# reedrosenbluth/LASS

Measured on AMD Instinct MI355X. Metric: clips/sec (10s@16kHz), higher is better.
Workload: dtype f32; 1 GPU; ResUNet30 separate() fp32, batch=16/GPU, 10s@16kHz clips, fixed precomputed condition embedding, seeded random-init weights (BASELINE configs[1]); samples_per_clip=160000, parallelism=clip-sharded x1

## Files before the change

### include/lass_hip.h

```cpp
#ifndef LASS_HIP_H
#define LASS_HIP_H

#include <stddef.h>
#include <stdint.h>

#ifdef __cplusplus
extern "C" {
#endif

typedef struct lass_ctx lass_ctx;

#define LASS_OK 0
#define LASS_ERR_ARG (-1)
#define LASS_ERR_HIP (-2)
#define LASS_ERR_STATE (-3)
#define LASS_ERR_WORKSPACE (-4)

#define LASS_F32 0
#define LASS_I64 1

#define LASS_COMPUTE_F32 0
#define LASS_COMPUTE_BF16 1
#define LASS_COMPUTE_BF16X3 2

int lass_version(void);

int lass_create(lass_ctx** out, int device_id);
int lass_create_stft(lass_ctx** out, int device_id, int n_fft, int hop);
int lass_stft_geometry(const lass_ctx* ctx, int* n_fft, int* hop);
int lass_create_multistft(lass_ctx** out, int device_id, int n_fft, int n_windows, const int* win_lengths,
                          int mask_window);
int lass_destroy(lass_ctx* ctx);

const char* lass_last_error(const lass_ctx* ctx);

int lass_set_param(lass_ctx* ctx, const char* name, const void* data, const int64_t* shape, int ndim, int dtype);

int lass_finalize(lass_ctx* ctx, int compute_mode);

int lass_workspace_bytes(const lass_ctx* ctx, int B, int L, size_t* bytes);

int lass_separate(lass_ctx* ctx, const float* mixture, const float* condition, float* out, int B, int L,
                  void* workspace, size_t workspace_bytes, void* stream);


int lass_separate_ragged(lass_ctx* ctx, const float* mixture, const int* lengths, const float* condition, float* out,
                         int B, int L, void* workspace, size_t workspace_bytes, void* stream);
int lass_ragged_bucket(const lass_ctx* ctx, int L, int* lo, int* hi);


int lass_separate_windows(lass_ctx* ctx, const float* recording, int64_t total, const int64_t* starts, const int* keep,
                          const float* condition , float* out , int B, int W,
                          void* workspace, size_t workspace_bytes, void* stream);

int lass_separate_windows_faded(lass_ctx* ctx, const float* recording, int64_t total, const int64_t* starts, const int* keep,
                                const int* fade, const float* ramp, int F, const float* condition ,
                                float* out , int B, int W, void* workspace, size_t workspace_bytes, void* stream);

int lass_graph_stats(const lass_ctx* ctx, long* captures, long* replays);
int lass_set_graph_replay(lass_ctx* ctx, int enabled);
int lass_set_wino4_splits(lass_ctx* ctx, int splits);
int lass_set_wino4_vprep(lass_ctx* ctx, int mode);
int lass_set_head_fold(lass_ctx* ctx, int enabled);
int lass_set_head_sc_fold(lass_ctx* ctx, int enabled);
int lass_set_pw_split(lass_ctx* ctx, int enabled);
int lass_set_wino4_gemm(lass_ctx* ctx, int enabled);
int lass_set_wino4_vprep_buffer(lass_ctx* ctx, float* v, size_t floats);

int lass_separate_components(lass_ctx* ctx, const float* const* mag, const float* cos_mask, const float* sin_mask,
                             const float* condition, float* out, int B, int L, void* workspace, size_t workspace_bytes,
                             void* stream);


int lass_stft_magphase(lass_ctx* ctx, const float* wav, int B, int L, float* mag, float* cos_out, float* sin_out,
                       float* real_out, float* imag_out, void* stream);

int lass_multi_stft(lass_ctx* ctx, const float* wav, int B, int L, int hop, int n_windows, const int* win_lengths,
                    float* const* mag, float* const* cos_out, float* const* sin_out, void* stream);

int lass_stft_components(lass_ctx* ctx, const float* wav, int B, int L, int n_fft, int hop, int n_windows,
                         const int* win_lengths, float* const* mag, float* const* cos_out, float* const* sin_out,
                         void* stream);

int lass_istft(lass_ctx* ctx, const float* real, const float* imag, int B, int T, int L, float* wav,
               float* frames_ws, void* stream);
int lass_istft_nfft(lass_ctx* ctx, const float* real, const float* imag, int B, int T, int L, int n_fft, int win_length,
                    float* wav, void* stream);

int lass_film(lass_ctx* ctx, const float* condition, int B, float* shift, void* stream);
int lass_film_width(const lass_ctx* ctx);
int lass_film_offset(const lass_ctx* ctx, const char* site);
int lass_film_raw(lass_ctx* ctx, const float* condition, int B, float* film, void* stream);

int lass_convblock(lass_ctx* ctx, const char* prefix, const float* x, int B, int H, int W, const float* shift,
                   float* y, float* scratch, void* stream);

int lass_encoder_block(lass_ctx* ctx, const char* name, const float* x, int B, int H, int W, const float* shift, float* y,
                       float* pool, float* scratch, void* stream);

int lass_front_end(lass_ctx* ctx, const float* wav, int B, int L, float* mag, float* cos_out, float* sin_out, float* x0,
                   void* stream);

int lass_front_end_ragged(lass_ctx* ctx, const float* wav, const int* lengths, int B, int L, float* mag, float* cos_out,
                          float* sin_out, float* x0, void* stream);
int lass_istft_ragged(lass_ctx* ctx, const float* real, const float* imag, const int* lengths, int B, int T, int L, int n_fft,
                      int win_length, float* wav, void* stream);

int lass_front_end_windows(lass_ctx* ctx, const float* recording, int64_t total, const int64_t* starts, int B, int W, float* mag,
                           float* cos_out, float* sin_out, float* x0, void* stream);
int lass_istft_windows(lass_ctx* ctx, const float* real, const float* imag, const int64_t* starts, const int* keep, int64_t total,
                       int B, int T, int W, int n_fft, int win_length, float* out, void* stream);
int lass_istft_windows_faded(lass_ctx* ctx, const float* real, const float* imag, const int64_t* starts, const int* keep,
                             const int* fade, const float* ramp, int F, int64_t total, int B, int T, int W, int n_fft,
                             int win_length, float* out, void* stream);

int lass_workspace_tensor(const lass_ctx* ctx, int B, int L, const char* name, size_t* offset, int64_t shape[4],
                          int64_t strides[4]);

int lass_upconv(lass_ctx* ctx, const char* name, const float* x, int B, int h, int w, const float* shift, float* y,
                void* stream);

int lass_mask_apply(lass_ctx* ctx, const float* x12, const float* mag, const float* cos_in, const float* sin_in,
                    int B, int T, int Tpad, float* out_real, float* out_imag, void* stream);

int lass_sdr_stats(lass_ctx* ctx, const float* ref, const float* est, int B, int L, double* stats, void* stream);

int lass_mix_at_snr(lass_ctx* ctx, float* source, const float* noise, const float* snr_db, float* mixture, int B, int L,
                    double* scratch, void* stream);

#define LASS_WAV_PCM16 0
#define LASS_WAV_PCM32 1
#define LASS_WAV_F32 2
#define LASS_RESAMPLE_MAX_TAPS 16383
#define LASS_RESAMPLE_MAX_TABLE 20480
#define LASS_RESAMPLE_MAX_RATIO 65536
int lass_decode_resample(lass_ctx* ctx, const void* raw, int64_t row_stride_bytes, int B, int frames, int channels, int encoding,
                         int up, int down, const float* taps, int n_taps, float* out, int L_out, void* stream);

int lass_decode_resample_planar(lass_ctx* ctx, const void* raw, int64_t row_stride_bytes, int B, int frames, int channels,
                                int encoding, int up, int down, const float* taps, int n_taps, float* out, int L_out, void* stream);

int lass_resample_encode(lass_ctx* ctx, const float* planes, int64_t row_stride, int64_t plane_stride, int B, int channels, int L_in,
                         int up, int down, const float* taps, int n_taps, int encoding, void* out_bytes,
                         int64_t out_row_stride_bytes, int frames_out, unsigned* clipped, void* stream);


#define LASS_LOUDNESS_MAX_HOP 38400
int lass_loudness(lass_ctx* ctx, const float* planes, int64_t row_stride, int64_t plane_stride, int B, int channels, int L,
                  const int* lengths, int hop, const double* coef, const float* weights, double* out, double* blocks, int nb_max,
                  void* scratch, size_t scratch_bytes, void* stream);

int lass_resample_peak(lass_ctx* ctx, const float* planes, int64_t row_stride, int64_t plane_stride, int B, int channels, int L_in,
                       int up, int down, const float* taps, int n_taps, int frames_out, float* peak, void* stream);

int lass_loudness_gain(lass_ctx* ctx, const double* loudness, const float* peak, int B, double target_lufs, float ceiling,
                       float* gain, int* limited, void* stream);

int lass_resample_encode_gain(lass_ctx* ctx, const float* planes, int64_t row_stride, int64_t plane_stride, int B, int channels,
                              int L_in, int up, int down, const float* taps, int n_taps, int encoding, const float* gain,
                              void* out_bytes, int64_t out_row_stride_bytes, int frames_out, unsigned* clipped, void* stream);


int lass_resample_true_peak(lass_ctx* ctx, const float* planes, int64_t row_stride, int64_t plane_stride, int B, int channels,
                            int L_in, int up, int down, const float* taps, int n_taps, int frames_out, int os, const float* os_taps,
                            int n_os_taps, float* peak, void* stream);

int lass_loudness_stats(lass_ctx* ctx, const float* planes, int64_t row_stride, int64_t plane_stride, int B, int channels, int L,
                        const int* lengths, int hop, const double* coef, const float* weights, double* out, double* blocks,
                        int nb_max, double* short_term, int ns_max, void* scratch, size_t scratch_bytes, void* stream);

int lass_segment_mix(lass_ctx* ctx, const float* waveforms, int B, int L, const int* mix_num, const float* comp_db, int max_comp,
                     const float* noise_db, float* mixture, float* segment, double* scratch, void* stream);


typedef struct lass_text_ctx lass_text_ctx;

int lass_text_create(lass_text_ctx** out, int device_id);
int lass_text_destroy(lass_text_ctx* ctx);
const char* lass_text_last_error(const lass_text_ctx* ctx);
int lass_text_set_param(lass_text_ctx* ctx, const char* name, const void* data, const int64_t* shape, int ndim);
int lass_text_finalize(lass_text_ctx* ctx);
int lass_text_layers(const lass_text_ctx* ctx);
int lass_text_workspace_bytes(const lass_text_ctx* ctx, int N, int S, size_t* bytes);
int lass_text_encode(lass_text_ctx* ctx, const int64_t* input_ids, const int64_t* attention_mask, int N, int S,
                     float* out, float* pooler_out, void* workspace, size_t workspace_bytes, void* stream);


typedef struct lass_audioq_ctx lass_audioq_ctx;

typedef struct lass_audioq_taps {
    float* wave48k;
    float* logmel;
    float* tokens;
    float* stage[4];
    float* embedding;
} lass_audioq_taps;

int lass_audioq_create(lass_audioq_ctx** out, int device_id);
int lass_audioq_destroy(lass_audioq_ctx* ctx);
const char* lass_audioq_last_error(const lass_audioq_ctx* ctx);
int lass_audioq_set_param(lass_audioq_ctx* ctx, const char* name, const void* data, const int64_t* shape, int ndim);
int lass_audioq_finalize(lass_audioq_ctx* ctx);
int lass_audioq_stages(const lass_audioq_ctx* ctx);
int lass_audioq_workspace_bytes(const lass_audioq_ctx* ctx, int B, size_t* bytes);
int lass_audioq_encode_wave48k(lass_audioq_ctx* ctx, const float* wave, const int* lengths, int B, int L, float* out,
                               const lass_audioq_taps* taps, void* workspace, size_t workspace_bytes, void* stream);
int lass_audioq_encode_wave32k(lass_audioq_ctx* ctx, const float* wave, const int* lengths, int B, int L, float* out,
                               const lass_audioq_taps* taps, void* workspace, size_t workspace_bytes, void* stream);


int lass_set_profiling(lass_ctx* ctx, int enabled);
int lass_profile_count(const lass_ctx* ctx);
int lass_profile_get(lass_ctx* ctx, int i, const char** name, double* ms, int* launches);
int lass_profile_reset(lass_ctx* ctx);

#ifdef __cplusplus
}
#endif
#endif
```

### lass_amd/_lib.py

```python
from __future__ import annotations

import ctypes
import os
from ctypes import POINTER, c_char_p, c_double, c_float, c_int, c_int64, c_long, c_size_t, c_void_p

_HERE = os.path.dirname(os.path.abspath(__file__))
LIB_PATH = os.environ.get("LASS_HIP_LIB") or os.path.join(_HERE, "csrc", "liblass_hip.so")

_lib = None

SYMBOLS = [
    ("lass_version", c_int, []),
    ("lass_create", c_int, [POINTER(c_void_p), c_int]),
    ("lass_create_stft", c_int, [POINTER(c_void_p), c_int, c_int, c_int]),
    ("lass_stft_geometry", c_int, [c_void_p, POINTER(c_int), POINTER(c_int)]),
    ("lass_create_multistft", c_int, [POINTER(c_void_p), c_int, c_int, c_int, POINTER(c_int), c_int]),
    ("lass_destroy", c_int, [c_void_p]),
    ("lass_last_error", c_char_p, [c_void_p]),
    ("lass_set_param", c_int, [c_void_p, c_char_p, c_void_p, POINTER(c_int64), c_int, c_int]),
    ("lass_finalize", c_int, [c_void_p, c_int]),
    ("lass_workspace_bytes", c_int, [c_void_p, c_int, c_int, POINTER(c_size_t)]),
    ("lass_separate", c_int, [c_void_p, c_void_p, c_void_p, c_void_p, c_int, c_int, c_void_p, c_size_t, c_void_p]),
    ("lass_separate_ragged", c_int, [c_void_p, c_void_p, c_void_p, c_void_p, c_void_p, c_int, c_int, c_void_p, c_size_t,
                                     c_void_p]),
    ("lass_ragged_bucket", c_int, [c_void_p, c_int, POINTER(c_int), POINTER(c_int)]),
    ("lass_front_end_ragged", c_int, [c_void_p, c_void_p, c_void_p, c_int, c_int, c_void_p, c_void_p, c_void_p, c_void_p,
                                      c_void_p]),
    ("lass_istft_ragged", c_int, [c_void_p, c_void_p, c_void_p, c_void_p, c_int, c_int, c_int, c_int, c_int, c_void_p,
                                  c_void_p]),
    ("lass_separate_windows", c_int, [c_void_p, c_void_p, c_int64, c_void_p, c_void_p, c_void_p, c_void_p, c_int, c_int, c_void_p,
                                      c_size_t, c_void_p]),
    ("lass_front_end_windows", c_int, [c_void_p, c_void_p, c_int64, c_void_p, c_int, c_int, c_void_p, c_void_p, c_void_p,
                                       c_void_p, c_void_p]),
    ("lass_istft_windows", c_int, [c_void_p, c_void_p, c_void_p, c_void_p, c_void_p, c_int64, c_int, c_int, c_int, c_int, c_int,
                                   c_void_p, c_void_p]),
    ("lass_separate_windows_faded", c_int, [c_void_p, c_void_p, c_int64, c_void_p, c_void_p, c_void_p, c_void_p, c_int, c_void_p,
                                            c_void_p, c_int, c_int, c_void_p, c_size_t, c_void_p]),
    ("lass_istft_windows_faded", c_int, [c_void_p, c_void_p, c_void_p, c_void_p, c_void_p, c_void_p, c_void_p, c_int, c_int64,
                                         c_int, c_int, c_int, c_int, c_int, c_void_p, c_void_p]),
    ("lass_stft_magphase", c_int, [c_void_p, c_void_p, c_int, c_int, c_void_p, c_void_p, c_void_p, c_void_p,
                                   c_void_p, c_void_p]),
    ("lass_mix_at_snr", c_int, [c_void_p, c_void_p, c_void_p, c_void_p, c_void_p, c_int, c_int, c_void_p, c_void_p]),
    ("lass_decode_resample", c_int, [c_void_p, c_void_p, c_int64, c_int, c_int, c_int, c_int, c_int, c_int, c_void_p, c_int,
                                     c_void_p, c_int, c_void_p]),
    ("lass_decode_resample_planar", c_int, [c_void_p, c_void_p, c_int64, c_int, c_int, c_int, c_int, c_int, c_int, c_void_p, c_int,
                                            c_void_p, c_int, c_void_p]),
    ("lass_resample_encode", c_int, [c_void_p, c_void_p, c_int64, c_int64, c_int, c_int, c_int, c_int, c_int, c_void_p, c_int, c_int,
                                     c_void_p, c_int64, c_int, c_void_p, c_void_p]),
    ("lass_loudness", c_int, [c_void_p, c_void_p, c_int64, c_int64, c_int, c_int, c_int, c_void_p, c_int, POINTER(c_double), c_void_p,
                              c_void_p, c_void_p, c_int, c_void_p, c_size_t, c_void_p]),
    ("lass_resample_peak", c_int, [c_void_p, c_void_p, c_int64, c_int64, c_int, c_int, c_int, c_int, c_int, c_void_p, c_int, c_int,
                                   c_void_p, c_void_p]),
    ("lass_loudness_gain", c_int, [c_void_p, c_void_p, c_void_p, c_int, c_double, c_float, c_void_p, c_void_p, c_void_p]),
    ("lass_resample_encode_gain", c_int, [c_void_p, c_void_p, c_int64, c_int64, c_int, c_int, c_int, c_int, c_int, c_void_p, c_int,
                                          c_int, c_void_p, c_void_p, c_int64, c_int, c_void_p, c_void_p]),
    ("lass_resample_true_peak", c_int, [c_void_p, c_void_p, c_int64, c_int64, c_int, c_int, c_int, c_int, c_int, c_void_p, c_int, c_int,
                                        c_int, c_void_p, c_int, c_void_p, c_void_p]),
    ("lass_loudness_stats", c_int, [c_void_p, c_void_p, c_int64, c_int64, c_int, c_int, c_int, c_void_p, c_int, POINTER(c_double),
                                    c_void_p, c_void_p, c_void_p, c_int, c_void_p, c_int, c_void_p, c_size_t, c_void_p]),
    ("lass_segment_mix", c_int, [c_void_p, c_void_p, c_int, c_int, c_void_p, c_void_p, c_int, c_void_p, c_void_p, c_void_p,
                                 c_void_p, c_void_p]),
    ("lass_multi_stft", c_int, [c_void_p, c_void_p, c_int, c_int, c_int, c_int, POINTER(c_int), POINTER(c_void_p),
                                POINTER(c_void_p), POINTER(c_void_p), c_void_p]),
    ("lass_graph_stats", c_int, [c_void_p, POINTER(c_long), POINTER(c_long)]),
    ("lass_set_graph_replay", c_int, [c_void_p, c_int]),
    ("lass_set_wino4_splits", c_int, [c_void_p, c_int]),
    ("lass_set_wino4_vprep", c_int, [c_void_p, c_int]),
    ("lass_set_wino4_vprep_buffer", c_int, [c_void_p, c_void_p, c_size_t]),
    ("lass_set_head_fold", c_int, [c_void_p, c_int]),
    ("lass_set_head_sc_fold", c_int, [c_void_p, c_int]),
    ("lass_set_pw_split", c_int, [c_void_p, c_int]),
    ("lass_set_wino4_gemm", c_int, [c_void_p, c_int]),
    ("lass_separate_components", c_int, [c_void_p, POINTER(c_void_p), c_void_p, c_void_p, c_void_p, c_void_p, c_int,
                                         c_int, c_void_p, c_size_t, c_void_p]),
    ("lass_stft_components", c_int, [c_void_p, c_void_p, c_int, c_int, c_int, c_int, c_int, POINTER(c_int),
                                     POINTER(c_void_p), POINTER(c_void_p), POINTER(c_void_p), c_void_p]),
    ("lass_istft_nfft", c_int, [c_void_p, c_void_p, c_void_p, c_int, c_int, c_int, c_int, c_int, c_void_p, c_void_p]),
    ("lass_istft", c_int, [c_void_p, c_void_p, c_void_p, c_int, c_int, c_int, c_void_p, c_void_p, c_void_p]),
    ("lass_film", c_int, [c_void_p, c_void_p, c_int, c_void_p, c_void_p]),
    ("lass_film_width", c_int, [c_void_p]),
    ("lass_film_offset", c_int, [c_void_p, c_char_p]),
    ("lass_film_raw", c_int, [c_void_p, c_void_p, c_int, c_void_p, c_void_p]),
    ("lass_convblock", c_int, [c_void_p, c_char_p, c_void_p, c_int, c_int, c_int, c_void_p, c_void_p, c_void_p,
                               c_void_p]),
    ("lass_encoder_block", c_int, [c_void_p, c_char_p, c_void_p, c_int, c_int, c_int, c_void_p, c_void_p, c_void_p,
                                   c_void_p, c_void_p]),
    ("lass_front_end", c_int, [c_void_p, c_void_p, c_int, c_int, c_void_p, c_void_p, c_void_p, c_void_p, c_void_p]),
    ("lass_workspace_tensor", c_int, [c_void_p, c_int, c_int, c_char_p, POINTER(c_size_t), POINTER(c_int64),
                                      POINTER(c_int64)]),
    ("lass_upconv", c_int, [c_void_p, c_char_p, c_void_p, c_int, c_int, c_int, c_void_p, c_void_p, c_void_p]),
    ("lass_mask_apply", c_int, [c_void_p, c_void_p, c_void_p, c_void_p, c_void_p, c_int, c_int, c_int, c_void_p,
                                c_void_p, c_void_p]),
    ("lass_sdr_stats", c_int, [c_void_p, c_void_p, c_void_p, c_int, c_int, c_void_p, c_void_p]),
    ("lass_text_create", c_int, [POINTER(c_void_p), c_int]),
    ("lass_text_destroy", c_int, [c_void_p]),
    ("lass_text_last_error", c_char_p, [c_void_p]),
    ("lass_text_set_param", c_int, [c_void_p, c_char_p, c_void_p, POINTER(c_int64), c_int]),
    ("lass_text_finalize", c_int, [c_void_p]),
    ("lass_text_layers", c_int, [c_void_p]),
    ("lass_text_workspace_bytes", c_int, [c_void_p, c_int, c_int, POINTER(c_size_t)]),
    ("lass_text_encode", c_int, [c_void_p, c_void_p, c_void_p, c_int, c_int, c_void_p, c_void_p, c_void_p, c_size_t,
                                 c_void_p]),
    ("lass_audioq_create", c_int, [POINTER(c_void_p), c_int]),
    ("lass_audioq_destroy", c_int, [c_void_p]),
    ("lass_audioq_last_error", c_char_p, [c_void_p]),
    ("lass_audioq_set_param", c_int, [c_void_p, c_char_p, c_void_p, POINTER(c_int64), c_int]),
    ("lass_audioq_finalize", c_int, [c_void_p]),
    ("lass_audioq_stages", c_int, [c_void_p]),
    ("lass_audioq_workspace_bytes", c_int, [c_void_p, c_int, POINTER(c_size_t)]),
    ("lass_audioq_encode_wave48k", c_int, [c_void_p, c_void_p, POINTER(c_int), c_int, c_int, c_void_p, c_void_p, c_void_p,
                                           c_size_t, c_void_p]),
    ("lass_audioq_encode_wave32k", c_int, [c_void_p, c_void_p, POINTER(c_int), c_int, c_int, c_void_p, c_void_p, c_void_p,
                                           c_size_t, c_void_p]),
    ("lass_set_profiling", c_int, [c_void_p, c_int]),
    ("lass_profile_count", c_int, [c_void_p]),
    ("lass_profile_get", c_int, [c_void_p, c_int, POINTER(c_char_p), POINTER(c_double), POINTER(c_int)]),
    ("lass_profile_reset", c_int, [c_void_p]),
]


class LassError(RuntimeError):
    pass


def load():
    global _lib
    if _lib is not None:
        return _lib
    import torch

    if not os.path.exists(LIB_PATH):
        raise LassError(
            f"{LIB_PATH} is missing - build it with `python -c 'import __graft_entry__ as g; g.build()'` "
            "(hipcc --offload-arch=gfx950).  lass_amd has no CPU fallback.")
    lib = ctypes.CDLL(LIB_PATH, mode=ctypes.RTLD_GLOBAL)
    for name, res, args in SYMBOLS:
        fn = getattr(lib, name)
        fn.restype = res
        fn.argtypes = args
    _lib = lib
    return lib


def check(ctx, rc: int, what: str):
    if rc < 0:
        msg = load().lass_last_error(ctx)
        raise LassError(f"{what} failed ({rc}): {msg.decode() if msg else '?'}")
    return rc


class TowerContext:

    def __init__(self, family: str, dev, tensors):
        import torch

        self.lib, self.family = load(), family
        h = c_void_p()
        rc = self.fn("create")(ctypes.byref(h), dev.index if dev.index is not None else torch.cuda.current_device())
        if rc < 0:
            raise LassError(f"{family}_create failed ({rc}): {self.fn('last_error')(None).decode()}")
        self.ctx = h
        self.key = self.key_of(dev, tensors)
        torch.cuda.current_stream(dev).synchronize()
        for name, p in tensors:
            t = p.detach().to(torch.float32).contiguous()
            shape = (c_int64 * t.dim())(*t.shape)
            self.check(self.fn("set_param")(self.ctx, name.encode(), c_void_p(t.data_ptr()), shape, t.dim()),
                       f"{family}_set_param({name})")
        self.check(self.fn("finalize")(self.ctx), f"{family}_finalize")

    @staticmethod
    def key_of(dev, tensors):
        return (dev, tuple((p.data_ptr(), p._version) for _, p in tensors))

    def fn(self, name: str):
        return getattr(self.lib, f"{self.family}_{name}")

    def check(self, rc: int, what: str) -> int:
        if rc < 0:
            raise LassError(f"{what} failed ({rc}): {self.fn('last_error')(self.ctx).decode()}")
        return rc

    def __del__(self):
        try:
            if getattr(self, "ctx", None):
                self.fn("destroy")(self.ctx)
                self.ctx = None
        except Exception:
            pass


def grow_workspace(owner, nbytes: int, dev):
    import torch

    if owner._ws is None or owner._ws.device != dev or owner._ws.numel() < nbytes:
        owner._ws = None
        owner._ws = torch.empty(nbytes, dtype=torch.uint8, device=dev)
    return owner._ws
```

### lass_amd/csrc/api.hip

```cpp
#include <hip/hip_runtime.h>

#include <algorithm>
#include <cmath>
#include <cstdio>
#include <cstdlib>
#include <cstring>
#include <map>
#include <string>
#include <vector>

#include "../../include/lass_hip.h"
#include "ctx_parts.h"
#include "graph_cache.h"
#include "head_fold.h"
#include "kernels.h"
#include "weight_plan.h"
#include "workspace_plan.h"

namespace {

constexpr float kBnEps = 1e-5f;
constexpr int kMaxBranches = LASS_MAX_STFT_WINDOWS;

struct Site {
    std::string film;
    std::string bn;
    int C = 0;
    int off = 0;
};

struct ResBlock {
    std::string prefix;
    int cin = 0, cout = 0;
    int width = 0;
    int s1 = -1, s2 = -1;
    WeightImages img;
};

struct ProfEntry {
    const char* name;
    double ms = 0;
    int launches = 0;
};

thread_local std::string g_create_err;

}

struct lass_ctx {
    int device = 0;
    std::string err;
    Geometry g;
    ModelTable m;
    std::string pre_name[kMaxBranches];
    ParamStore raw;
    bool finalized = false;
    float2* tw2k = nullptr;
    std::vector<Site> sites;
    std::map<std::string, int> site_idx;
    int n_shift = 0;
    float *film_W = nullptr, *film_b = nullptr, *bn_scale = nullptr, *bn_base = nullptr;
    float *bn0_s = nullptr, *bn0_h = nullptr;
    std::vector<ResBlock> enc, dec;
    int dec_site[6] = {0};
    WeightImages up_img[6], img;
    int head_rows = 0;
    std::vector<void*> owned;
    RouteCfg cfg;
    float* stage_v = nullptr;
    size_t stage_v_floats = 0;
    float* stage_m = nullptr;
    size_t stage_m_floats = 0;
    float* stage_v_user = nullptr;
    size_t stage_v_user_floats = 0;
    float* stage_part = nullptr;
    size_t stage_part_floats = 0;
    bool use_graph = true;
    GraphCache<hipGraphExec_t> graphs;
    std::map<std::pair<int, int>, bool> last_split;
    hipStream_t g_stream = nullptr;
    int split_batch = 1;
    hipStream_t s2 = nullptr;
    hipEvent_t ev_fork = nullptr, ev_join = nullptr;
    unsigned long gen = 0;
    long g_replays = 0, g_captures = 0;
    bool profiling = false;
    std::vector<ProfEntry> prof;
    std::vector<hipEvent_t> ev_pool;
    struct Pending { int cls; hipEvent_t a, b; };
    std::vector<Pending> pending;
    size_t ev_used = 0;
};

namespace {

bool starts_with(const std::string& s, const char* p) { return s.rfind(p, 0) == 0; }
bool ends_with(const std::string& s, const char* p) {
    const size_t n = strlen(p);
    return s.size() >= n && s.compare(s.size() - n, n, p) == 0;
}

std::string film_to_bn(const std::string& film) {
    std::string s = "base.";
    for (size_t i = 0; i < film.size(); ++i) {
        if (film[i] == '-' && i + 1 < film.size() && film[i + 1] == '>') {
            s += '.';
            ++i;
        } else {
            s += film[i];
        }
    }
    const size_t p = s.rfind("beta");
    s.replace(p, 4, "bn");
    return s;
}

int add_site(lass_ctx* c, const std::string& film, int C) {
    Site s;
    s.film = film;
    s.bn = film_to_bn(film);
    s.C = C;
    s.off = c->n_shift;
    c->n_shift += C;
    c->site_idx[film] = (int)c->sites.size();
    c->sites.push_back(s);
    return (int)c->sites.size() - 1;
}

void build_arch(lass_ctx* c) {
    const Geometry& g = c->g;
    c->sites.clear();
    c->site_idx.clear();
    c->n_shift = 0;
    c->enc.clear();
    c->dec.clear();
    c->m = model_table(g.variant == 0 ? 0 : g.nbr, g.fcrop);
    for (int k = 0; k < g.nbr; ++k) {
        ResBlock rb;
        std::string film;
        if (g.variant == 0) {
            rb.prefix = "base.encoder_block1.conv_block1";
            film = "encoder_block1->conv_block1";
            c->pre_name[k] = "base.pre_conv";
        } else {
            const std::string w = std::to_string(g.wins[k]);
            rb.prefix = "base.encoder_block1s." + w + ".conv_block1";
            film = "encoder_block1s->" + w + "->conv_block1";
            c->pre_name[k] = "base.pre_convs." + w;
        }
        rb.cin = rb.cout = kPreCh;
        rb.width = g.fcrop;
        rb.s1 = add_site(c, film + "->beta1", kPreCh);
        rb.s2 = add_site(c, film + "->beta2", kPreCh);
        c->enc.push_back(rb);
    }
    for (int i = 1; i < 7; ++i) {
        const EncSpec& e = c->m.E[i];
        ResBlock rb;
        rb.prefix = std::string("base.") + e.name + ".conv_block1";
        rb.cin = e.cin;
        rb.cout = e.cout;
        rb.width = g.fcrop >> i;
        rb.s1 = add_site(c, std::string(e.name) + "->conv_block1->beta1", e.cin);
        rb.s2 = add_site(c, std::string(e.name) + "->conv_block1->beta2", e.cout);
        c->enc.push_back(rb);
    }
    for (int i = 0; i < 6; ++i) {
        const auto& d = c->m.D[i];
        const int e = 5 - i;
        c->dec_site[i] = add_site(c, std::string(d.name) + "->beta1", d.cin);
        ResBlock rb;
        rb.prefix = std::string("base.") + d.name + ".conv_block2";
        rb.cin = c->m.dec_cat[i];
        rb.cout = d.cout;
        rb.width = g.fcrop >> e;
        rb.s1 = add_site(c, std::string(d.name) + "->conv_block2->beta1", rb.cin);
        rb.s2 = add_site(c, std::string(d.name) + "->conv_block2->beta2", d.cout);
        c->dec.push_back(rb);
    }
}

std::vector<int64_t> expected_shape(const lass_ctx* c, const std::string& name) {
    auto bn_field = [](const std::string& n) {
        return ends_with(n, ".weight") || ends_with(n, ".bias") || ends_with(n, ".running_mean") ||
               ends_with(n, ".running_var");
    };
    if (starts_with(name, "base.bn0.") && bn_field(name)) return {c->g.nbins};
    for (int k = 0; k < c->g.nbr; ++k) {
        if (name == c->pre_name[k] + ".weight") return {kPreCh, 1, 1, 1};
        if (name == c->pre_name[k] + ".bias") return {kPreCh};
    }
    if (name == "base.after_conv.weight") return {3, kPreCh, 1, 1};
    if (name == "base.after_conv.bias") return {3};
    auto res_block = [&](const ResBlock& rb) -> std::vector<int64_t> {
        const std::string& p = rb.prefix;
        if (!starts_with(name, (p + ".").c_str())) return {};
        const std::string f = name.substr(p.size() + 1);
        if (starts_with(f, "bn1.") && bn_field(f)) return {rb.cin};
        if (starts_with(f, "bn2.") && bn_field(f)) return {rb.cout};
        if (f == "conv1.weight") return {rb.cout, rb.cin, 3, 3};
        if (f == "conv2.weight") return {rb.cout, rb.cout, 3, 3};
        if (rb.cin != rb.cout && f == "shortcut.weight") return {rb.cout, rb.cin, 1, 1};
        if (rb.cin != rb.cout && f == "shortcut.bias") return {rb.cout};
        return {};
    };
    for (const auto& rb : c->enc) {
        auto s = res_block(rb);
        if (!s.empty()) return s;
    }
    for (int i = 0; i < 6; ++i) {
        auto s = res_block(c->dec[i]);
        if (!s.empty()) return s;
        const DecSpec& d = c->m.D[i];
        const std::string p = std::string("base.") + d.name;
        if (name == p + ".conv1.weight") return {d.cin, d.cout, d.uh, d.uw};
        if (starts_with(name, (p + ".bn1.").c_str()) && bn_field(name)) return {d.cin};
    }
    if (starts_with(name, "film.")) {
        for (const auto& s : c->sites) {
            if (name == "film." + s.film + ".weight") return {s.C, LASS_COND};
            if (name == "film." + s.film + ".bias") return {s.C};
        }
    }
    return {};
}

bool ignorable(const std::string& name) {
    if (starts_with(name, "base.stft.") || starts_with(name, "base.istft.")) return true;
    if (ends_with(name, "num_batches_tracked")) return true;
    for (const auto& d : kDec) {
        if (starts_with(name, (std::string("base.") + d.name + ".bn2.").c_str())) return true;
        if (starts_with(name, (std::string("film.") + d.name + "->beta2.").c_str())) return true;
    }
    return false;
}

const float* rawp(const lass_ctx* c, const std::string& name) { return c->raw.get(name); }

template <typename T>
int dev_alloc(lass_ctx* c, T** p, size_t count) {
    void* v = nullptr;
    HIP_TRY(c, hipMalloc(&v, count * sizeof(T)));
    c->owned.push_back(v);
    *p = (T*)v;
    return 0;
}

void free_owned(lass_ctx* c) {
    for (void* p : c->owned) (void)hipFree(p);
    c->owned.clear();
}

SlotSet missing_images(const lass_ctx* c, const WeightImages* blk, const WeightImages* up, SlotSet want) {
    SlotSet miss = 0;
    for (int s = 0; s < kWeightSlots; ++s) {
        const WeightImages* im = s < kBlockSlots ? blk : s < kDecoderSlotsEnd ? up : &c->img;
        if ((want >> s & 1) && !(im && im->p[s])) miss |= SlotSet(1) << s;
    }
    return miss;
}

enum ProfClass { P_STFT = 0, P_FILM, P_PRECONV, P_CONV3X3, P_TCONV, P_POOL, P_MASK, P_ISTFT, P_COUNT };
const char* kProfNames[P_COUNT] = {"stft_magphase", "film", "pre_conv", "conv3x3_mfma", "tconv_mfma",
                                   "avg_pool",      "mask_apply", "istft"};

constexpr size_t kProfPairs = 512;

struct ProfScope {
    lass_ctx* c;
    hipStream_t s;
    int cls;
    hipEvent_t b = nullptr;
    bool on = false;
    ProfScope(lass_ctx* ctx, hipStream_t st, int k) : c(ctx), s(st), cls(k) {
        if (!c->profiling || c->ev_used + 2 > c->ev_pool.size()) return;
        hipEvent_t a = c->ev_pool[c->ev_used++];
        b = c->ev_pool[c->ev_used++];
        (void)hipEventRecord(a, s);
        c->pending.push_back({cls, a, b});
        on = true;
    }
    ~ProfScope() {
        if (on) (void)hipEventRecord(b, s);
    }
};

void prof_collect(lass_ctx* c) {
    for (auto& p : c->pending) {
        float ms = 0;
        if (hipEventElapsedTime(&ms, p.a, p.b) == hipSuccess) {
            c->prof[p.cls].ms += ms;
            c->prof[p.cls].launches += 1;
        }
    }
    c->pending.clear();
    c->ev_used = 0;
}

struct CatCopies {
    void* act;
    void* raw;
    int noct;
    const float* scale;
    const float* shift;
};

struct MaskHead {
    const float* mag;
    const float* cosv;
    const float* sinv;
    float* oreal;
    float* oimag;
    int T;
    int nbins;
};

struct PreConv {
    const float* x0;
    const float* w;
    const float* b;
};

struct UpFuse {
    const void* xin;
    int cin, h, w;
    const void* w16;
    const void* wsc16;
};

struct BlockFusions {
    float* pool_out = nullptr;
    int pool_h = 2;
    long pool_bs = 0;
    int cofs = 0;
    const PreConv* pre = nullptr;
    const MaskHead* head = nullptr;
    const CatCopies* skip_out = nullptr;
    const CatCopies* cat_in = nullptr;
    const Site* act_out = nullptr;
    const CatCopies* pool_copies = nullptr;
    const UpFuse* up = nullptr;
    float* kpart = nullptr;
    float* vws = nullptr;
    size_t vws_floats = 0;
    float* mws = nullptr;
    size_t mws_floats = 0;
    const HeadScPlanes* planes = nullptr;
};

BlockIO block_io(const float* x, long x_bs, const BlockFusions& f) {
    BlockIO io;
    io.x0 = f.pre && f.pre->x0;
    io.head = f.head != nullptr;
    io.pool = f.pool_out != nullptr; io.pool_h = f.pool_h;
    io.x_aligned = x && ((uintptr_t)x & 15u) == 0 && x_bs % 4 == 0;
    io.sc_planes = f.planes != nullptr;
    io.cat_in = f.cat_in != nullptr; io.skip_out = f.skip_out != nullptr; io.pool_copies = f.pool_copies != nullptr;
    io.act_out = f.act_out != nullptr; io.up_cin = f.up ? f.up->cin : 0;
    return io;
}

bool overlaps(int B, const float* a, long a_bs, size_t a_n, const float* b, long b_bs, size_t b_n) {
    return a && b && a_n && b_n && a < b + (size_t)(B - 1) * b_bs + b_n && b < a + (size_t)(B - 1) * a_bs + a_n;
}

int run_resblock_bf16(lass_ctx* c, const ResBlock& rb, Bf16Form form, const ConvArgs& p, const ConvArgs& q, int B, hipStream_t st,
                      const BlockFusions& f) {
    if (form == BF16_TWO) {
        const bool x0 = f.pre && f.pre->x0;
        {
            ProfScope ps(c, st, P_CONV3X3);
            HIP_TRY(c, lass_launch_conv_bf16(x0 ? CONV1_ACT_PRE : CONV1_ACT, p, st));
        }
        ProfScope ps(c, st, P_CONV3X3);
        HIP_TRY(c, lass_launch_conv_bf16(rb.cin != rb.cout ? CONV2_SHORTCUT : x0 ? CONV2_IDENT_PRE : CONV2_IDENT, q, st));
        return 0;
    }
    ConvArgs uq;
    if (const UpFuse* up = f.up) {
        uq.in_bf16 = up->xin; uq.Cin = up->cin; uq.H = up->h; uq.W = up->w; uq.B = B;
        uq.w_bf16 = up->w16; uq.w2_bf16 = up->wsc16;
    }
    if (!(form == BF16_ENC1 ? lass_enc1_fused_bf16_supported(p, q) : form == BF16_DEC6 ? lass_dec6_fused_bf16_supported(p, q)
                            : form == BF16_DEC6U && f.up && lass_dec6u_fused_bf16_supported(p, q, uq)))
        return fail(c, LASS_ERR_STATE, rb.prefix + ": the launch arguments contradict the planned route");
    ProfScope ps(c, st, P_CONV3X3);
    HIP_TRY(c, form == BF16_ENC1 ? lass_launch_enc1_fused_bf16(p, q, st) : form == BF16_DEC6 ? lass_launch_dec6_fused_bf16(p, q, st)
                                 : lass_launch_dec6u_fused_bf16(p, q, uq, st));
    return 0;
}

int launch_routed(lass_ctx* c, const ResBlock& rb, const char* what, const ConvRoute& rt, const ConvArgs& a, const Wino4Split& sk,
                  float* vws, const Wino4Gemm& wg, hipStream_t st, const HeadScPlanes* planes = nullptr) {
    ProfScope ps(c, st, P_CONV3X3);
    bool ok = true;
    switch (rt.family) {
        case CONV_F4X4: {
            const Wino4Split s = rt.splits > 1 ? sk : Wino4Split();
            Wino4VPre vp;
            if (rt.v_from_memory) vp.v = vws;
            if (rt.head_sc_fold) {
                ok = planes && (rt.head_fold ? lass_wino4_headfold_planes_supported(a, *planes) : lass_wino4_sclogit_supported(a, *planes));
                if (ok) HIP_TRY(c, rt.head_fold ? lass_launch_wino4_headfold_planes(a, *planes, st) : lass_launch_wino4_sclogit(a, *planes, st));
                break;
            }
            if (rt.head_fold) {
                ok = lass_wino4_headfold_supported(a);
                if (ok) HIP_TRY(c, lass_launch_wino4_headfold(a, st));
                break;
            }
            if (rt.gemm) {
                ok = lass_wino4_gemm_supported(rt.kind, a, vp, wg);
                if (ok) HIP_TRY(c, lass_launch_wino4_gemm(rt.kind, a, vp, wg, st));
                break;
            }
            ok = rt.v_from_memory ? lass_wino4_vpre_supported(rt.kind, a, s) : lass_wino4_supported(rt.kind, a, s);
            if (ok) HIP_TRY(c, lass_launch_wino4(rt.kind, a, st, s, vp));
            break;
        }
        case CONV_F2X2:
            ok = lass_wino_supported(a);
            if (ok) HIP_TRY(c, lass_launch_wino(rt.kind, a, st));
            break;
        case CONV_DIRECT:
            HIP_TRY(c, lass_launch_conv(rt.kind, a, st));
            break;
        case CONV_NONE:
            ok = false;
            break;
    }
    return ok ? 0 : fail(c, LASS_ERR_STATE, rb.prefix + " " + what + ": the launch arguments contradict the planned route");
}

int run_resblock(lass_ctx* c, const ResBlock& rb, const float* x, long x_bs, int B, int H, int W, const float* shift,
                 float* a2, float* out, long out_bs, hipStream_t st, const BlockFusions& f = BlockFusions()) {
    const PreConv* pre = f.pre;
    const WeightImages& im = rb.img;
    const CatCopies *skip_out = f.skip_out, *cat_in = f.cat_in, *pool_copies = f.pool_copies;
    const float* x0 = pre ? pre->x0 : nullptr;
    const Site& s1 = c->sites[rb.s1];
    const Site& s2 = c->sites[rb.s2];
    const long HW = (long)H * W;
    ConvArgs p;
    p.in = x; p.in_bs = x_bs; p.Cin = rb.cin; p.w = im.f32(W1); p.Nw = rb.cout; p.N = rb.cout;
    p.pro_scale = c->bn_scale + s1.off; p.pro_shift = shift + s1.off; p.pro_shift_bs = c->n_shift;
    p.epi_scale = c->bn_scale + s2.off; p.epi_shift = shift + s2.off; p.epi_shift_bs = c->n_shift;
    p.out = a2; p.out_bs = rb.cout * HW; p.B = B; p.H = H; p.W = W;
    if (x0) {
        p.in = x0; p.in_bs = HW;
        p.pre_w = pre->w; p.pre_b = pre->b;
    }
    p.w_wino = im.f32(U1); p.w_wino4 = im.f32(U1F);
    p.w_bf16 = im.p[B1]; p.w_bf16_lo = im.p[B1L];
    const BlockIO io = block_io(x, x_bs, f);
    const BlockShape shape{rb.cin, rb.cout, rb.width};
    const Bf16Block bb = plan_bf16_block(c->cfg, shape, H, W, io);
    if (bb.cat_in != io.cat_in || bb.skip_out != io.skip_out || bb.pool_copies != io.pool_copies || bb.act_out != io.act_out ||
        (bb.form == BF16_DEC6U) != (io.up_cin != 0))
        return fail(c, LASS_ERR_STATE, rb.prefix + ": the launch arguments contradict the planned route");
    const bool bf1 = bb.form != BF16_NONE;
    void* a2_hi = a2;
    void* a2_lo = c->cfg.mode == MODE_BF16X3 ? (void*)((char*)a2 + (size_t)B * rb.cout * HW * 2) : nullptr;
    if (bf1) { p.out_bf16 = a2_hi; p.out_bf16_lo = a2_lo; }
    if (cat_in) p.in_bf16 = cat_in->act;
    const BlockRoute rt = bf1 ? BlockRoute() : plan_block(c->cfg, shape, B, H, W, io);
    if (const SlotSet miss = missing_images(c, &im, bb.form == BF16_DEC6U ? &c->up_img[5] : nullptr,
                                            bf1 ? route_images(bb, bf16_block_weights(c->cfg, rb.cin, rb.cout)) : route_images(rt)))
        return fail(c, LASS_ERR_STATE, rb.prefix + (miss == slots(WSC3) ? " shortcut: the split weights of the planned route are missing"
                                                                        : ": the launch arguments contradict the planned route"));
    const size_t xn = rb.cin * HW, on = rb.cout * HW;
    if (rt.kpart_floats) {
        if (!f.kpart) return fail(c, LASS_ERR_STATE, "split-K needs its partial workspace");
        if (overlaps(B, f.kpart, 0, rt.kpart_floats, x, x_bs, xn) || overlaps(B, f.kpart, 0, rt.kpart_floats, a2, on, on) ||
            overlaps(B, f.kpart, 0, rt.kpart_floats, out, out_bs, on))
            return fail(c, LASS_ERR_STATE, "the split-K partials must not overlap the block's input, intermediate or output");
    }
    if (rt.v_floats) {
        if (!f.vws || f.vws_floats < rt.v_floats) return fail(c, LASS_ERR_STATE, "the V-from-memory route needs its image workspace");
        if (overlaps(B, f.vws, 0, rt.v_floats, x, x_bs, xn) || overlaps(B, f.vws, 0, rt.v_floats, a2, on, on) ||
            overlaps(B, f.vws, 0, rt.v_floats, out, out_bs, on) || overlaps(B, f.vws, 0, rt.v_floats, f.kpart, 0, rt.kpart_floats))
            return fail(c, LASS_ERR_STATE, "the V image must not overlap the block's input, intermediate, output or split-K partials");
    }
    if (rt.m_floats) {
        if (!f.mws || f.mws_floats < rt.m_floats) return fail(c, LASS_ERR_STATE, "the gemm route needs its product-image workspace");
        if (overlaps(B, f.mws, 0, rt.m_floats, x, x_bs, xn) || overlaps(B, f.mws, 0, rt.m_floats, a2, on, on) ||
            overlaps(B, f.mws, 0, rt.m_floats, out, out_bs, on) || overlaps(B, f.mws, 0, rt.m_floats, f.kpart, 0, rt.kpart_floats) ||
            overlaps(B, f.mws, 0, rt.m_floats, f.vws, 0, rt.v_floats))
            return fail(c, LASS_ERR_STATE, "the product image must not overlap the block's input, intermediate, output or other workspaces");
        if (f.pool_out) {
            const size_t pn = on / ((size_t)f.pool_h * 2);
            if (overlaps(B, f.mws, 0, rt.m_floats, f.pool_out, f.pool_bs ? f.pool_bs : (long)pn, pn))
                return fail(c, LASS_ERR_STATE, "the product image must not overlap the block's pooled output");
        }
    }
    if (f.planes) {
        if (!rt.conv2.head_sc_fold) return fail(c, LASS_ERR_STATE, rb.prefix + ": the head's shortcut planes contradict the block's route");
        const size_t pn = (size_t)3 * HW;
        for (const float* pl : {(const float*)f.planes->skip, (const float*)f.planes->up})
            if (overlaps(B, pl, pn, pn, x, x_bs, xn) || overlaps(B, pl, pn, pn, a2, on, on) || overlaps(B, pl, pn, pn, out, out_bs, on) ||
                overlaps(B, pl, pn, pn, f.kpart, 0, rt.kpart_floats) || overlaps(B, pl, pn, pn, f.vws, 0, rt.v_floats))
                return fail(c, LASS_ERR_STATE, "the head's shortcut planes must not overlap the block's tensors or workspaces");
        if (overlaps(B, f.planes->skip, pn, pn, f.planes->up, pn, pn)) return fail(c, LASS_ERR_STATE, "the two sets of shortcut planes overlap");
    }
    Wino4Split sk;
    if (rt.kpart_floats) { sk.n = std::max(rt.conv1.splits, rt.conv2.splits); sk.part = f.kpart; }
    ConvArgs q;
    q.in = a2; q.in_bs = rb.cout * HW; q.Cin = rb.cout; q.w = im.f32(W2); q.Nw = rb.cout; q.N = rb.cout;
    q.out = out; q.out_bs = out_bs; q.B = B; q.H = H; q.W = W;
    q.pool_out = f.pool_out; q.pool_h = f.pool_h; q.pool_bs = f.pool_bs;
    q.w_wino = im.f32(U2); q.w2_wino = im.f32(USC); q.w_wino4 = im.f32(U2F);
    if (const MaskHead* mh = f.head) {
        q.out = nullptr;
        q.mask_w = rawp(c, "base.after_conv.weight"); q.mask_b = rawp(c, "base.after_conv.bias");
        q.mask_mag = mh->mag; q.mask_cos = mh->cosv; q.mask_sin = mh->sinv;
        q.mask_re = mh->oreal; q.mask_im = mh->oimag; q.mask_T = mh->T; q.mask_nbins = mh->nbins;
    }
    q.w_bf16 = im.p[B2]; q.w2_bf16 = im.p[BSC16]; q.w_bf16_lo = im.p[B2L]; q.w2_bf16_lo = im.p[BSCL];
    if (bf1) { q.in_bf16 = a2_hi; q.in_bf16_lo = a2_lo; }
    if (cat_in) q.in2_bf16 = cat_in->raw;
    if (pool_copies) {
        q.pool_out = nullptr;
        q.pool_bf16 = pool_copies->raw; q.pool_bf16_act = pool_copies->act;
        q.pool_oct0 = f.cofs / 8; q.pool_noct = pool_copies->noct;
        q.pool_act_scale = pool_copies->scale + f.cofs; q.pool_act_shift = pool_copies->shift + f.cofs; q.act_shift_bs = c->n_shift;
    }
    if (const Site* act_out = f.act_out) {
        q.out_bf16 = out; q.out = nullptr; q.out_oct0 = 0; q.out_noct = 0;
        q.epi_scale = c->bn_scale + act_out->off; q.epi_shift = shift + act_out->off; q.epi_shift_bs = c->n_shift;
    }
    if (skip_out) {
        q.out = nullptr;
        q.out_bf16 = skip_out->raw; q.out_bf16_act = skip_out->act;
        q.out_oct0 = (rb.cout + f.cofs) / 8; q.out_noct = skip_out->noct;
        q.act_scale = skip_out->scale + rb.cout + f.cofs; q.act_shift = skip_out->shift + rb.cout + f.cofs; q.act_shift_bs = c->n_shift;
    }
    if (rb.cin == rb.cout) {
        q.res = x; q.res_bs = x_bs;
        if (x0) {
            q.res = x0; q.res_bs = HW;
            q.pre_w = pre->w; q.pre_b = pre->b;
        }
    } else {
        q.in2 = x; q.in2_bs = x_bs; q.Cin2 = rb.cin; q.w2 = im.f32(WSC); q.bias = rawp(c, rb.prefix + ".shortcut.bias");
    }
    if (bf1) return run_resblock_bf16(c, rb, bb.form, p, q, B, st, f);
    if (rt.conv2.head_fold) {
        q.w_wino4 = im.f32(U2H); q.w2 = im.f32(WSCH); q.bias = im.f32(BH);
        q.mask_w = q.mask_b = nullptr;
    }
    if (rt.shortcut_gemm) {
        if (overlaps(B, out, out_bs, on, x, x_bs, xn) || overlaps(B, out, out_bs, on, a2, on, on))
            return fail(c, LASS_ERR_STATE, "a block's output must not overlap its input or its intermediate");
        if (rt.conv2.family == CONV_NONE) return fail(c, LASS_ERR_STATE, "conv2 with the shortcut as residual");
        if (!lass_pw_gemm_supported(CONV2_SHORTCUT, q))
            return fail(c, LASS_ERR_STATE, rb.prefix + " shortcut: the launch arguments contradict the planned route");
        PwSplitW sw;
        if (rt.pw_split) sw.w = im.p[WSC3];
        {
            ProfScope ps(c, st, P_CONV3X3);
            HIP_TRY(c, lass_launch_pw_gemm(CONV2_SHORTCUT, q, st, sw));
        }
        q.in2 = nullptr; q.in2_bs = 0; q.Cin2 = 0; q.w2 = nullptr; q.bias = nullptr;
        q.res = out; q.res_bs = out_bs;
    }
    Wino4Gemm g1, g2;
    g1.w3 = im.p[U1G]; g2.w3 = im.p[U2G];
    g1.m = g2.m = f.mws;
    if (int r = launch_routed(c, rb, "conv1", rt.conv1, p, sk, f.vws, g1, st)) return r;
    return launch_routed(c, rb, "conv2", rt.conv2, q, sk, f.vws, g2, st, f.planes);
}

int run_upconv(lass_ctx* c, int di, const float* x, int B, int h, int w, const float* shift, float* out, long out_bs,
               hipStream_t st, const CatCopies* cb = nullptr, bool x_is_act_bf16 = false, const HeadScPlanes* planes = nullptr) {
    const DecSpec& d = c->m.D[di];
    const Site& s = c->sites[c->dec_site[di]];
    ConvArgs p;
    p.in = x; p.in_bs = (long)d.cin * h * w; p.Cin = d.cin;
    p.w = rawp(c, std::string("base.") + d.name + ".conv1.weight");
    p.N = p.Nw = d.cout * d.uh * d.uw;
    p.pro_scale = c->bn_scale + s.off; p.pro_shift = shift + s.off; p.pro_shift_bs = c->n_shift;
    p.out = out; p.out_bs = out_bs; p.B = B; p.H = h; p.W = w; p.up_h = d.uh;
    p.w_bf16 = c->up_img[di].p[UP16]; p.w_bf16_lo = c->up_img[di].p[UP16L];
    UpSite site;
    site.in_act = x_is_act_bf16; site.out_copies = cb != nullptr; site.logits = planes != nullptr;
    site.aligned = p.in_bs % 4 == 0 && p.out_bs % 2 == 0 && ((uintptr_t)p.in & 15u) == 0 && ((uintptr_t)p.w & 15u) == 0 && ((uintptr_t)p.out & 7u) == 0;
    const UpRoute rt = plan_upconv(c->cfg, d, h, w, site);
    bool ok = rt.in_act == site.in_act && rt.out_copies == site.out_copies && (rt.family == UP_LOGITS) == site.logits;
    if (rt.in_act) p.in_bf16 = x;
    if (rt.out_copies) {
        p.out = nullptr;
        p.out_bf16 = cb->raw; p.out_bf16_act = cb->act; p.out_oct0 = 0; p.out_noct = cb->noct;
        p.act_scale = cb->scale; p.act_shift = cb->shift; p.act_shift_bs = c->n_shift;
    }
    ok = ok && !missing_images(c, nullptr, &c->up_img[di], route_images(rt, c->cfg));
    if (ok && rt.family == UP_LOGITS) ok = lass_tconv_logits_supported(p, *planes);
    PwSplitW sw;
    if (rt.pw_split) sw.w = c->up_img[di].p[UP3];
    if (ok && rt.family == UP_GEMM) ok = lass_pw_gemm_supported(TCONV_ACT, p);
    if (!ok || rt.family == UP_INSIDE)
        return fail(c, LASS_ERR_STATE, std::string(d.name) + " transposed conv: the launch arguments contradict the planned route");
    ProfScope ps(c, st, P_TCONV);
    switch (rt.family) {
        case UP_LOGITS:
            HIP_TRY(c, lass_launch_tconv_logits(p, *planes, st));
            break;
        case UP_BF16:
            HIP_TRY(c, lass_launch_conv_bf16(TCONV_ACT, p, st));
            break;
        case UP_GEMM:
            HIP_TRY(c, lass_launch_pw_gemm(TCONV_ACT, p, st, sw));
            break;
        default:
            HIP_TRY(c, lass_launch_conv(TCONV_ACT, p, st));
            break;
    }
    return 0;
}

PlanInputs plan_inputs(const lass_ctx* c) {
    const bool head_sc = head_sc_weights(c->cfg, c->m, c->head_rows) && !missing_images(c, nullptr, nullptr, slots(HS_WT, HS_WSKIP));
    return PlanInputs{c->g, c->m, c->cfg, c->n_shift, head_sc};
}
Plan make_plan(const lass_ctx* c, int B, int L) { return make_plan(plan_inputs(c), B, L); }
CallPlan plan_call(const lass_ctx* c, int B, int L, bool capturing, size_t workspace_bytes) {
    return plan_call(plan_inputs(c), B, L, c->split_batch, c->profiling, capturing, workspace_bytes);
}

int use_device(lass_ctx* c) {
    if (!c) return LASS_ERR_ARG;
    HIP_TRY(c, hipSetDevice(c->device));
    return 0;
}

int check_ready(lass_ctx* c) {
    if (!c) return LASS_ERR_ARG;
    if (!c->finalized) return fail(c, LASS_ERR_STATE, "lass_finalize has not been called (or a parameter changed since)");
    return use_device(c);
}

void drop_graphs(lass_ctx* c) {
    for (hipGraphExec_t x : c->graphs.take_all()) (void)hipGraphExecDestroy(x);
}

int stage_scratch(lass_ctx* c, const ResBlock& rb, int B, int H, int W, const float* x, BlockFusions* f) {
    const BlockRoute rt = plan_block(c->cfg, BlockShape{rb.cin, rb.cout, rb.width}, B, H, W, block_io(x, (long)rb.cin * H * W, *f));
    const auto grow = [&](float** buf, size_t* have, size_t need) -> int {
        if (need <= *have) return 0;
        if (*buf) HIP_TRY(c, hipFree(*buf));
        *buf = nullptr;
        *have = 0;
        HIP_TRY(c, hipMalloc((void**)buf, need * sizeof(float)));
        *have = need;
        return 0;
    };
    if (int r = grow(&c->stage_part, &c->stage_part_floats, rt.kpart_floats)) return r;
    if (rt.kpart_floats) f->kpart = c->stage_part;
    if (!c->stage_v_user)
        if (int r = grow(&c->stage_v, &c->stage_v_floats, rt.v_floats)) return r;
    if (rt.v_floats) {
        f->vws = c->stage_v_user ? c->stage_v_user : c->stage_v;
        f->vws_floats = c->stage_v_user ? c->stage_v_user_floats : c->stage_v_floats;
    }
    if (int r = grow(&c->stage_m, &c->stage_m_floats, rt.m_floats)) return r;
    if (rt.m_floats) { f->mws = c->stage_m; f->mws_floats = c->stage_m_floats; }
    return 0;
}

int stage_nfft(const lass_ctx* c) { return c->g.variant == 0 ? c->g.nfft : LASS_NFFT; }

bool istft_nfft_ok(const lass_ctx* c, int n_fft) { return n_fft == 2048 || (n_fft == 1024 && c->g.hop == LASS_HOP); }

const ResBlock* find_block(const lass_ctx* c, const std::string& prefix) {
    for (const auto& rb : c->enc) if (rb.prefix == prefix) return &rb;
    for (const auto& rb : c->dec) if (rb.prefix == prefix) return &rb;
    return nullptr;
}

hipError_t launch_bnfold(const lass_ctx* c, const std::string& bn, int C, float* scale, float* base, hipStream_t st) {
    return lass_launch_bnfold(rawp(c, bn + ".weight"), rawp(c, bn + ".bias"), rawp(c, bn + ".running_mean"), rawp(c, bn + ".running_var"), C,
                              kBnEps, scale, base, st);
}

int upload(lass_ctx* c, const std::vector<float>& v, void** slot) {
    float* d = nullptr;
    if (dev_alloc(c, &d, v.size())) return LASS_ERR_HIP;
    HIP_TRY(c, hipMemcpy(d, v.data(), v.size() * sizeof(float), hipMemcpyHostToDevice));
    *slot = d;
    return 0;
}

struct HeadHost {
    HeadFold hf;
    HeadScFold hsf;
    const std::vector<float>& of(WeightForm f) const {
        return f == WF_HEAD_U4 ? hf.u4 : f == WF_HEAD_WSC ? hf.wsc : f == WF_HEAD_BIAS ? hf.bias : f == WF_HEAD_SC_WT ? hsf.wt : hsf.wskip;
    }
};
int compose_head(lass_ctx* c, int Q, bool sc, HeadHost* h) {
    const ResBlock& rb = c->dec[5];
    const DecSpec& d6 = c->m.D[5];
    const int N = rb.cout, K = rb.cin;
    std::vector<float> w2, ws, bs, wa, ba, wt;
    const auto host = [&](std::vector<float>& v, const std::string& name, size_t n) -> int {
        v.resize(n);
        HIP_TRY(c, hipMemcpy(v.data(), rawp(c, name), n * sizeof(float), hipMemcpyDeviceToHost));
        return 0;
    };
    HIP_TRY(c, hipStreamSynchronize(nullptr));
    if (host(w2, rb.prefix + ".conv2.weight", (size_t)N * N * 9) || host(ws, rb.prefix + ".shortcut.weight", (size_t)N * K) ||
        host(bs, rb.prefix + ".shortcut.bias", N) || host(wa, "base.after_conv.weight", (size_t)Q * N) ||
        host(ba, "base.after_conv.bias", Q) ||
        (sc && host(wt, std::string("base.") + d6.name + ".conv1.weight", (size_t)d6.cin * d6.cout * d6.uh * d6.uw)))
        return LASS_ERR_HIP;
    if (sc) compose_head_sc_fold(ws.data(), wa.data(), wt.data(), N, d6.cout, kPreCh, Q, d6.cin, d6.uh, d6.uw, &h->hsf);
    if (!compose_head_fold(w2.data(), ws.data(), bs.data(), wa.data(), ba.data(), N, N, K, Q, &h->hf) || h->hf.u4.empty()) h->hf = HeadFold();
    return 0;
}

}

extern "C" {

int lass_version(void) { return 10900; }

const char* lass_last_error(const lass_ctx* ctx) { return ctx ? ctx->err.c_str() : g_create_err.c_str(); }

static int create_impl(lass_ctx** out, int device_id, const Geometry& geom) {
    if (!out) return LASS_ERR_ARG;
    *out = nullptr;
    if (int rc = open_device(device_id, g_create_err)) return rc;
    lass_ctx* c = new lass_ctx();
    c->device = device_id;
    c->g = geom;
    if (const char* e = getenv("LASS_FUSE_CATB")) c->cfg.fuse_catb = atoi(e) != 0;
    if (const char* e = getenv("LASS_FUSE_BLOCK")) c->cfg.fuse_block = atoi(e) != 0;
    if (const char* e = getenv("LASS_FUSE_UP")) c->cfg.fuse_up = atoi(e) != 0;
    if (const char* e = getenv("LASS_WINO4")) c->cfg.wino4_mincin = atoi(e);
    if (const char* e = getenv("LASS_WINO4_VPREP")) c->cfg.vprep_mode = std::max(0, std::min(2, atoi(e)));
    if (const char* e = getenv("LASS_HEAD_FOLD")) c->cfg.head_fold = atoi(e) != 0;
    if (const char* e = getenv("LASS_HEAD_SC_FOLD")) c->cfg.head_sc_fold = atoi(e) != 0;
    if (const char* e = getenv("LASS_PW_SPLIT")) c->cfg.pw_split = atoi(e) != 0;
    if (const char* e = getenv("LASS_WINO4_GEMM")) c->cfg.wino4_gemm = atoi(e) != 0;
    if (const char* e = getenv("LASS_SPLIT")) c->split_batch = std::max(0, std::min(2, atoi(e)));
    if (const char* e = getenv("LASS_GRAPH")) c->use_graph = atoi(e) != 0;
    c->prof.resize(P_COUNT);
    for (int i = 0; i < P_COUNT; ++i) c->prof[i].name = kProfNames[i];
    build_arch(c);
    if (hipSetDevice(device_id) != hipSuccess) {
        g_create_err = "hipSetDevice failed";
        delete c;
        return LASS_ERR_HIP;
    }
    std::vector<float2> tw2k(2048);
    for (int k = 0; k < 2048; ++k) {
        const double a = 2.0 * M_PI * k / 2048.0;
        tw2k[k] = make_float2((float)std::cos(a), (float)std::sin(a));
    }
    if (hipMalloc((void**)&c->tw2k, sizeof(float2) * 2048) != hipSuccess ||
        hipMemcpy(c->tw2k, tw2k.data(), sizeof(float2) * 2048, hipMemcpyHostToDevice) != hipSuccess) {
        g_create_err = "allocating FFT tables failed";
        delete c;
        return LASS_ERR_HIP;
    }
    *out = c;
    return 0;
}

int lass_create(lass_ctx** out, int device_id) { return create_impl(out, device_id, Geometry()); }

int lass_create_stft(lass_ctx** out, int device_id, int n_fft, int hop) {
    if (!out) return LASS_ERR_ARG;
    *out = nullptr;
    Geometry g;
    if (n_fft == 2048 && hop == 320) {
        g.nfft = 2048; g.nbins = 1025; g.fcrop = 1024; g.hop = 320; g.wins[0] = 2048;
    } else if (n_fft != LASS_NFFT || hop != LASS_HOP) {
        g_create_err = "lass_create_stft: (n_fft, hop) must be (1024, 160) or (2048, 320), got (" + std::to_string(n_fft) + ", " +
                       std::to_string(hop) + ")";
        return LASS_ERR_ARG;
    }
    return create_impl(out, device_id, g);
}

int lass_stft_geometry(const lass_ctx* c, int* n_fft, int* hop) {
    if (!c) return LASS_ERR_ARG;
    if (n_fft) *n_fft = c->g.nfft;
    if (hop) *hop = c->g.hop;
    return 0;
}

int lass_create_multistft(lass_ctx** out, int device_id, int n_fft, int n_windows, const int* win_lengths,
                          int mask_window) {
    if (!out) return LASS_ERR_ARG;
    *out = nullptr;
    Geometry g;
    g.variant = 1;
    g.magphase_sem = 1;
    if (n_fft != 2048 || n_windows < 1 || n_windows > kMaxBranches || !win_lengths) {
        g_create_err = "lass_create_multistft: n_fft must be 2048 and 1 <= n_windows <= 4";
        return LASS_ERR_ARG;
    }
    g.nfft = n_fft; g.nbins = n_fft / 2 + 1; g.fcrop = n_fft / 2; g.nbr = n_windows; g.mask_br = -1;
    for (int k = 0; k < n_windows; ++k) {
        const int w = win_lengths[k];
        if (w < 32 || w > n_fft || (2048 % w) != 0) {
            g_create_err = "lass_create_multistft: window lengths must be powers of two in [32, n_fft]";
            return LASS_ERR_ARG;
        }
        for (int j = 0; j < k; ++j)
            if (g.wins[j] == w) {
                g_create_err = "lass_create_multistft: duplicate window length";
                return LASS_ERR_ARG;
            }
        g.wins[k] = w;
        if (w == mask_window) g.mask_br = k;
    }
    if (g.mask_br < 0) {
        g_create_err = "lass_create_multistft: mask_window is not one of the analysis windows";
        return LASS_ERR_ARG;
    }
    return create_impl(out, device_id, g);
}

int lass_destroy(lass_ctx* c) {
    if (!c) return LASS_ERR_ARG;
    (void)hipSetDevice(c->device);
    free_owned(c);
    c->raw.free_all();
    for (auto e : c->ev_pool) (void)hipEventDestroy(e);
    (void)hipDeviceSynchronize();
    drop_graphs(c);
    if (c->g_stream) (void)hipStreamDestroy(c->g_stream);
    if (c->s2) (void)hipStreamDestroy(c->s2);
    if (c->ev_join) (void)hipEventDestroy(c->ev_join);
    if (c->ev_fork) (void)hipEventDestroy(c->ev_fork);
    (void)hipFree(c->tw2k);
    (void)hipFree(c->stage_part);
    (void)hipFree(c->stage_v);
    (void)hipFree(c->stage_m);
    delete c;
    return 0;
}

int lass_set_param(lass_ctx* c, const char* name_c, const void* data, const int64_t* shape, int ndim, int dtype) {
    if (!c || !name_c || !data || ndim < 0 || (ndim > 0 && !shape)) return fail(c, LASS_ERR_ARG, "bad argument");
    const std::string name(name_c);
    std::vector<int64_t> want = expected_shape(c, name);
    if (want.empty()) {
        if (ignorable(name)) return 1;
        return fail(c, LASS_ERR_ARG, "unknown parameter '" + name + "'");
    }
    if (dtype != LASS_F32) return fail(c, LASS_ERR_ARG, "parameter '" + name + "' must be float32");
    std::vector<int64_t> got(shape, shape + ndim);
    if (got != want) {
        std::string m = "shape mismatch for '" + name + "': got (";
        for (auto v : got) m += std::to_string(v) + ",";
        m += ") want (";
        for (auto v : want) m += std::to_string(v) + ",";
        return fail(c, LASS_ERR_ARG, m + ")");
    }
    HIP_TRY(c, hipSetDevice(c->device));
    if (int rc = c->raw.put(c, name, data, shape, ndim)) return rc;
    c->finalized = false;
    return 0;
}

int lass_finalize(lass_ctx* c, int compute_mode) {
    if (!c) return LASS_ERR_ARG;
    if (compute_mode != LASS_COMPUTE_F32 && compute_mode != LASS_COMPUTE_BF16 && compute_mode != LASS_COMPUTE_BF16X3)
        return fail(c, LASS_ERR_ARG, "unsupported compute mode");
    c->last_split.clear();
    c->cfg.mode = (ComputeMode)compute_mode;
    HIP_TRY(c, hipSetDevice(c->device));
    HIP_TRY(c, hipDeviceSynchronize());
    drop_graphs(c);
    free_owned(c);
    for (auto* blocks : {&c->enc, &c->dec})
        for (ResBlock& rb : *blocks) rb.img = WeightImages();
    for (WeightImages& u : c->up_img) u = WeightImages();
    c->img = WeightImages();
    c->head_rows = 0;
    c->finalized = false;
    c->err.clear();
    hipStream_t st = nullptr;
    const auto need = [&](const std::string& p, std::initializer_list<const char*> fields) {
        for (const char* f : fields)
            if (!rawp(c, p + f) && c->err.empty()) c->err = "missing parameter '" + p + f + "'";
    };
    const auto bn = {".weight", ".bias", ".running_mean", ".running_var"}, wb = {".weight", ".bias"};
    for (const Site& s : c->sites) { need(s.bn, bn); need("film." + s.film, wb); }
    need("base.bn0", bn);
    for (int k = 0; k < c->g.nbr; ++k) need(c->pre_name[k], wb);
    need("base.after_conv", wb);
    for (const auto* blocks : {&c->enc, &c->dec})
        for (const ResBlock& rb : *blocks) {
            need(rb.prefix, {".conv1.weight", ".conv2.weight"});
            if (rb.cin != rb.cout) need(rb.prefix, {".shortcut.weight", ".shortcut.bias"});
        }
    for (const DecSpec& d : c->m.D) need(std::string("base.") + d.name, {".conv1.weight"});
    if (!c->err.empty()) return LASS_ERR_STATE;
    if (dev_alloc(c, &c->bn_scale, c->n_shift) || dev_alloc(c, &c->bn_base, c->n_shift) ||
        dev_alloc(c, &c->film_W, (size_t)c->n_shift * LASS_COND) || dev_alloc(c, &c->film_b, c->n_shift) ||
        dev_alloc(c, &c->bn0_s, c->g.nbins) || dev_alloc(c, &c->bn0_h, c->g.nbins))
        return LASS_ERR_HIP;
    for (const Site& s : c->sites) {
        HIP_TRY(c, launch_bnfold(c, s.bn, s.C, c->bn_scale + s.off, c->bn_base + s.off, st));
        HIP_TRY(c, hipMemcpyAsync(c->film_W + (size_t)s.off * LASS_COND, rawp(c, "film." + s.film + ".weight"),
                                  (size_t)s.C * LASS_COND * sizeof(float), hipMemcpyDeviceToDevice, st));
        HIP_TRY(c, hipMemcpyAsync(c->film_b + s.off, rawp(c, "film." + s.film + ".bias"), s.C * sizeof(float), hipMemcpyDeviceToDevice, st));
    }
    HIP_TRY(c, launch_bnfold(c, "base.bn0", c->g.nbins, c->bn0_s, c->bn0_h, st));
    const Param* ra = c->raw.find("base.after_conv.weight");
    if (!ra->shape.empty() && ra->n == (size_t)ra->shape[0] * c->dec[5].cout) c->head_rows = (int)ra->shape[0];
    const ResBlock& rb6 = c->dec[5];
    const DecSpec& d6 = c->m.D[5];
    HeadHost head;
    bool composed = false;
    for (const WeightItem& it : plan_weights(c->cfg, c->m, c->head_rows)) {
        ResBlock* rb = it.owner != OWN_BLOCK ? nullptr : it.index < (int)c->enc.size() ? &c->enc[it.index] : &c->dec[it.index - c->enc.size()];
        WeightImages& im = rb ? rb->img : it.owner == OWN_DECODER ? c->up_img[it.index] : c->img;
        const std::string prefix = rb ? rb->prefix + "." : std::string("base.") + c->m.D[it.owner == OWN_DECODER ? it.index : 5].name + ".";
        const float* src = it.param ? rawp(c, prefix + it.param) : it.from >= 0 ? im.f32((WeightSlot)it.from) : nullptr;
        if (weight_form_on_host(it.form)) {
            if (!composed && compose_head(c, c->head_rows, head_sc_weights(c->cfg, c->m, c->head_rows), &head)) return LASS_ERR_HIP;
            composed = true;
            const std::vector<float>& v = head.of(it.form);
            if (v.empty()) continue;
            if (v.size() != it.count) return fail(c, LASS_ERR_STATE, "lass_finalize: a head composition contradicts the weight plan");
            if (int r = upload(c, v, &im.p[it.slot])) return r;
            continue;
        }
        char* dst = nullptr;
        if (dev_alloc(c, &dst, it.count * it.elem_bytes)) return LASS_ERR_HIP;
        float* dstf = (float*)dst;
        switch (it.form) {
            case WF_RELAYOUT: HIP_TRY(c, lass_launch_relayout_conv(src, it.rows, it.cols, it.taps, dstf, st)); break;
            case WF_F2X2: HIP_TRY(c, lass_launch_wino_weights(src, it.rows, it.cols, dstf, st)); break;
            case WF_F2X2_SC: HIP_TRY(c, lass_launch_wino_shortcut_weights(src, it.rows, it.cols, dstf, st)); break;
            case WF_F4X4: HIP_TRY(c, lass_launch_wino4_weights(src, it.rows, it.cols, dstf, st)); break;
            case WF_F4X4_SPLIT3: HIP_TRY(c, lass_launch_wino4_gemm_weights(src, it.rows, it.cols, dst, st)); break;
            case WF_PW_SPLIT3: HIP_TRY(c, lass_launch_pw_split_weights(src, it.rows, it.cols, dst, st)); break;
            case WF_UP_SC:
                HIP_TRY(c, lass_launch_compose_up_shortcut(rawp(c, rb6.prefix + ".shortcut.weight"), rawp(c, prefix + "conv1.weight"), d6.cin,
                                                           d6.cout, rb6.cin, rb6.cout, dstf, st));
                break;
            case WF_BF16: case WF_BF16_LO: case WF_BF16_T: case WF_BF16_T_LO:
                HIP_TRY(c, lass_launch_weights_bf16(src, it.rows, it.cols, it.taps, dst, it.form == WF_BF16_LO || it.form == WF_BF16_T_LO,
                                                    it.form >= WF_BF16_T, st));
                break;
            default: return fail(c, LASS_ERR_STATE, "lass_finalize: a weight form without a launcher");
        }
        im.p[it.slot] = dst;
    }
    HIP_TRY(c, hipStreamSynchronize(st));
    c->finalized = true;
    ++c->gen;
    return 0;
}

int lass_workspace_bytes(const lass_ctx* c, int B, int L, size_t* bytes) {
    if (!c || !bytes) return LASS_ERR_ARG;
    const CallPlan cp = plan_call(c, B, L, false, kNoWorkspaceLimit);
    if (!cp.whole.valid) return LASS_ERR_ARG;
    *bytes = cp.need;
    return 0;
}

int lass_film_width(const lass_ctx* c) { return c ? c->n_shift : LASS_ERR_ARG; }

int lass_film_offset(const lass_ctx* c, const char* site) {
    if (!c || !site) return -1;
    auto it = c->site_idx.find(site);
    return it == c->site_idx.end() ? -1 : c->sites[it->second].off;
}

int lass_film(lass_ctx* c, const float* cond, int B, float* shift, void* stream) {
    int r = check_ready(c);
    if (r) return r;
    if (!cond || !shift || B <= 0) return fail(c, LASS_ERR_ARG, "lass_film: bad argument");
    HIP_TRY(c, lass_launch_film(cond, B, c->film_W, c->film_b, c->bn_base, c->n_shift, shift, (hipStream_t)stream));
    return 0;
}

int lass_film_raw(lass_ctx* c, const float* cond, int B, float* film, void* stream) {
    int r = check_ready(c);
    if (r) return r;
    if (!cond || !film || B <= 0) return fail(c, LASS_ERR_ARG, "lass_film_raw: bad argument");
    HIP_TRY(c, lass_launch_film(cond, B, c->film_W, c->film_b, nullptr, c->n_shift, film, (hipStream_t)stream));
    return 0;
}

int lass_stft_magphase(lass_ctx* c, const float* wav, int B, int L, float* mag, float* cos_out, float* sin_out,
                       float* real_out, float* imag_out, void* stream) {
    if (!c) return LASS_ERR_ARG;
    const int n_fft = stage_nfft(c), hop = c->g.hop;
    if (!wav || B <= 0 || L <= n_fft / 2) return fail(c, LASS_ERR_ARG, "lass_stft_magphase: bad argument");
    if (int r = use_device(c)) return r;
    const int T = 1 + L / hop;
    StftBranch br;
    br.wlen = n_fft; br.mag = mag; br.cosv = cos_out; br.sinv = sin_out; br.real = real_out; br.imag = imag_out;
    HIP_TRY(c, lass_launch_stft2(wav, ClipForm{B, L}, n_fft, hop, T, T, 1, &br, 0, nullptr, nullptr, c->tw2k,
                                 (hipStream_t)stream));
    return 0;
}

int lass_stft_components(lass_ctx* c, const float* wav, int B, int L, int n_fft, int hop, int n_windows,
                         const int* win_lengths, float* const* mag, float* const* cos_out, float* const* sin_out,
                         void* stream) {
    if (!c || !wav || !win_lengths || !mag || !cos_out || !sin_out || B <= 0 || hop <= 0 || n_windows <= 0 ||
        n_windows > LASS_MAX_STFT_WINDOWS || (n_fft != 1024 && n_fft != 2048) || L <= n_fft / 2)
        return fail(c, LASS_ERR_ARG, "lass_stft_components: bad argument (n_fft 1024 or 2048, at most 4 windows, L > n_fft/2)");
    StftBranch br[LASS_MAX_STFT_WINDOWS];
    for (int i = 0; i < n_windows; ++i) {
        const int w = win_lengths[i];
        if (w < 32 || w > n_fft || (2048 % w) != 0)
            return fail(c, LASS_ERR_ARG, "lass_stft_components: window lengths must be powers of two in [32, n_fft]");
        if (!mag[i] || !cos_out[i] || !sin_out[i]) return fail(c, LASS_ERR_ARG, "lass_stft_components: null output");
        br[i].wlen = w; br[i].mag = mag[i]; br[i].cosv = cos_out[i]; br[i].sinv = sin_out[i];
    }
    if (int r = use_device(c)) return r;
    const int T = 1 + L / hop;
    HIP_TRY(c, lass_launch_stft2(wav, ClipForm{B, L}, n_fft, hop, T, T, n_windows, br, 1, nullptr, nullptr, c->tw2k,
                                 (hipStream_t)stream));
    return 0;
}

int lass_multi_stft(lass_ctx* c, const float* wav, int B, int L, int hop, int n_windows, const int* win_lengths,
                    float* const* mag, float* const* cos_out, float* const* sin_out, void* stream) {
    if (!c || !wav || !win_lengths || !mag || !cos_out || !sin_out || B <= 0 || hop <= 0 || n_windows <= 0 ||
        n_windows > LASS_MAX_STFT_WINDOWS)
        return fail(c, LASS_ERR_ARG, "lass_multi_stft: bad argument");
    for (int i = 0; i < n_windows; ++i) {
        const int N = win_lengths[i];
        if (N != 256 && N != 512 && N != 1024 && N != 2048)
            return fail(c, LASS_ERR_ARG, "lass_multi_stft: window lengths must be 256, 512, 1024 or 2048");
        if (L <= N / 2) return fail(c, LASS_ERR_ARG, "lass_multi_stft: waveform shorter than the reflect padding");
        if (!mag[i] || !cos_out[i] || !sin_out[i]) return fail(c, LASS_ERR_ARG, "lass_multi_stft: null output");
    }
    if (int r = use_device(c)) return r;
    HIP_TRY(c, lass_launch_multi_stft(wav, B, L, hop, n_windows, win_lengths, c->tw2k, mag, cos_out, sin_out,
                                      (hipStream_t)stream));
    return 0;
}

int lass_istft(lass_ctx* c, const float* real, const float* imag, int B, int T, int L, float* wav, float* frames_ws,
// ... 472 lines not shown
        float* x0k[kMaxBranches];
        for (int k = 0; k < nbr; ++k) x0k[k] = F(pl.x0[k]);
        HIP_TRY(c, launch_front_end(c, mixture, cf, x0k, F(pl.mag), F(pl.cosv), F(pl.sinv), st));
    } else {
        ProfScope ps(c, st, P_STFT);
        for (int k = 0; k < nbr; ++k) {
            if (!comp->mag[k]) return fail(c, LASS_ERR_ARG, std::string(who) + ": null magnitude");
            HIP_TRY(c, lass_launch_x0_from_mag(comp->mag[k], B, T, Tp, g.fcrop, c->bn0_s, c->bn0_h, F(pl.x0[k]), st));
        }
        if (!comp->cosv || !comp->sinv) return fail(c, LASS_ERR_ARG, std::string(who) + ": null phase");
        mag_m = comp->mag[g.mask_br]; cos_m = comp->cosv; sin_m = comp->sinv;
    }
    {
        ProfScope ps(c, st, P_FILM);
        HIP_TRY(c, lass_launch_film(condition, B, c->film_W, c->film_b, c->bn_base, c->n_shift, shift, st));
    }
    HeadScPlanes hs_skip, hs_up, hs_head;
    if (sp.head_sc_fold) {
        hs_skip.skip = hs_head.skip = F(pl.lg_skip); hs_skip.w = c->img.f32(HS_WSKIP);
        hs_up.up = hs_head.up = F(pl.lg_up); hs_up.w = c->img.f32(HS_WT);
        hs_skip.up = hs_head.up;
    }
    const auto copies = [&](float* store, const ResBlock& rb, int e) {
        const Site& s = c->sites[rb.s1];
        return CatCopies{store, (char*)store + (size_t)B * rb.cin * pl.lv.eh[e] * pl.lv.ew[e] * 2, rb.cin / 8, c->bn_scale + s.off, shift + s.off};
    };
    CatCopies cb[6], pc[4];
    for (int d = 1; d < 6; ++d) cb[d] = copies(F(pl.cat[d]), c->dec[d], 5 - d);
    for (int i = 0; i < 4; ++i) pc[i] = copies(F(pl.pool[i]), c->enc[nbr + i], i + 1);
    const float* x = nullptr;
    for (int i = 0; i < 7; ++i) {
        const int H = pl.lv.eh[i], W = pl.lv.ew[i];
        const long HW = (long)H * W;
        const EncSpec& e = c->m.E[i];
        const int nb = i == 0 ? nbr : 1;
        float* o = nullptr;
        long o_bs = 0;
        for (int k = 0; k < nb; ++k) {
            const ResBlock& rb = c->enc[i == 0 ? k : nbr - 1 + i];
            const BlockIO& io = sp.enc_io[i];
            BlockFusions f;
            f.cofs = k * e.cout;
            if (i < 6) {
                const int d = 5 - i;
                o = F(pl.cat[d]) + (size_t)(c->m.D[d].cout + f.cofs) * HW;
                o_bs = (long)c->m.dec_cat[d] * HW;
            } else {
                o = F(pl.center);
                o_bs = rb.cout * HW;
            }
            if (io.pool) {
                const long Ho = H / e.dh, Wo = W / e.dw;
                f.pool_out = F(pl.pool[i]) + (size_t)f.cofs * Ho * Wo;
                f.pool_h = e.dh;
                f.pool_bs = (long)e.cout * nb * Ho * Wo;
            }
            PreConv pre{};
            if (io.x0) {
                pre = PreConv{F(pl.x0[k]), rawp(c, c->pre_name[k] + ".weight"), rawp(c, c->pre_name[k] + ".bias")};
                f.pre = &pre;
            }
            if (io.sc_planes) f.planes = &hs_skip;
            if (io.skip_out) f.skip_out = &cb[5 - i];
            if (io.cat_in) f.cat_in = &pc[i - 1];
            if (io.pool_copies) f.pool_copies = &pc[i];
            scratch(f);
            r = run_resblock(c, rb, x, rb.cin * HW, B, H, W, shift, F(pl.a2), o, o_bs, st, f);
            if (r) return r;
        }
        x = i < 6 ? F(pl.pool[i]) : o;
    }
    for (int d = 0; d < 6; ++d) {
        const int e = 5 - d;
        const int H = pl.lv.eh[e], W = pl.lv.ew[e];
        const long HW = (long)H * W;
        const int h = H / c->m.D[d].uh, w = W / c->m.D[d].uw;
        const ResBlock& rb = c->dec[d];
        const BlockIO& io = sp.dec_io[d];
        BlockFusions f;
        const UpFuse upf{x, c->m.D[d].cin, h, w, c->up_img[d].p[UP16], c->img.p[UP_SC16]};
        if (io.up_cin) {
            f.up = &upf;
        } else {
            r = run_upconv(c, d, x, B, h, w, shift, F(pl.cat[d]), rb.cin * HW, st, sp.up[d].out_copies ? &cb[d] : nullptr, sp.up[d].in_act,
                           sp.up[d].family == UP_LOGITS ? &hs_up : nullptr);
            if (r) return r;
        }
        if (io.act_out) f.act_out = &c->sites[c->dec_site[d + 1]];
        if (io.cat_in) f.cat_in = &cb[d];
        const MaskHead head{mag_m, cos_m, sin_m, F(pl.oreal), F(pl.oimag), T, g.nbins};
        if (io.head) f.head = &head;
        if (io.sc_planes) f.planes = &hs_head;
        scratch(f);
        r = run_resblock(c, rb, F(pl.cat[d]), rb.cin * HW, B, H, W, shift, F(pl.a2), F(pl.decout[d]), rb.cout * HW, st, f);
        if (r) return r;
        x = F(pl.decout[d]);
    }
    {
        ProfScope ps(c, st, P_ISTFT);
        HIP_TRY(c, lass_launch_istft2(F(pl.oreal), F(pl.oimag), cf, T, g.nfft, g.wins[g.mask_br], g.hop, c->tw2k, out, st));
    }
    return 0;
}

static ClipForm upper_clips(const ClipForm& cf, int h, size_t* row) {
    ClipForm u = cf;
    u.B = cf.B - h;
    if (cf.lengths) u.lengths = cf.lengths + h;
    if (cf.starts) u.starts = cf.starts + h;
    if (cf.keep) u.keep = cf.keep + 2 * h;
    if (cf.fade) u.fade = cf.fade + 2 * h;
    *row = cf.starts ? 0 : (size_t)h * cf.L;
    return u;
}

static int separate_any(lass_ctx* c, const float* mixture, const float* condition, float* out, const ClipForm& cf, const CallPlan& cp,
                        void* workspace, size_t workspace_bytes, hipStream_t stream, const char* who) {
    const bool split = cp.split && c->finalized && mixture && condition && out && workspace;
    c->last_split[{cf.B, cf.L}] = split;
    if (!split) return separate_impl(c, mixture, nullptr, condition, out, cf, cp.whole, workspace, workspace_bytes, stream, who);
    HIP_TRY(c, hipSetDevice(c->device));
    if (!c->ev_fork) HIP_TRY(c, hipEventCreateWithFlags(&c->ev_fork, hipEventDisableTiming));
    if (!c->s2) {
        HIP_TRY(c, hipStreamCreateWithFlags(&c->s2, hipStreamNonBlocking));
        HIP_TRY(c, hipEventCreateWithFlags(&c->ev_join, hipEventDisableTiming));
    }
    const int h = cf.B / 2;
    const size_t half_ws = cp.half_bytes();
    HIP_TRY(c, hipEventRecord(c->ev_fork, stream));
    HIP_TRY(c, hipStreamWaitEvent(c->s2, c->ev_fork, 0));
    ClipForm lower = cf;
    lower.B = h;
    size_t row2;
    const ClipForm upper = upper_clips(cf, h, &row2);
    int r = separate_impl(c, mixture, nullptr, condition, out, lower, cp.half, workspace, half_ws, stream, who);
    const int r2 = separate_impl(c, mixture + row2, nullptr, condition + (size_t)h * LASS_COND, out + row2, upper, cp.half,
                                 (char*)workspace + half_ws, half_ws, c->s2, who);
    if (!r) r = r2;
    HIP_TRY(c, hipEventRecord(c->ev_join, c->s2));
    HIP_TRY(c, hipStreamWaitEvent(stream, c->ev_join, 0));
    return r;
}

static int separate_call(lass_ctx* c, const float* mixture, const float* condition, float* out, const ClipForm& cf, void* workspace,
                         size_t workspace_bytes, void* stream, const char* who) {
    const int B = cf.B, L = cf.L;
    if (!mixture) return fail(c, LASS_ERR_ARG, std::string(who) + ": null pointer");
    if (c->use_graph && !c->profiling && c->finalized) {
        GraphKey key;
        key.mix = mixture; key.cond = condition; key.out = out; key.ws = workspace; key.lens = cf.lengths; key.B = B; key.L = L;
        key.gen = c->gen;
        key.starts = cf.starts; key.keep = cf.keep; key.total = cf.total;
        key.fade = cf.fade; key.ramp = cf.ramp; key.F = cf.F;
        auto& slot = c->graphs.touch(key);
        if (c->graphs.drain_due()) {
            HIP_TRY(c, hipSetDevice(c->device));
            HIP_TRY(c, hipDeviceSynchronize());
            for (hipGraphExec_t x : c->graphs.take_retired()) (void)hipGraphExecDestroy(x);
        }
        if (slot.exec()) {
            if (workspace_bytes < slot.need)
                return fail(c, LASS_ERR_WORKSPACE, "workspace too small: need " + std::to_string(slot.need) + " bytes");
            HIP_TRY(c, hipSetDevice(c->device));
            HIP_TRY(c, hipGraphLaunch(slot.exec(), (hipStream_t)stream));
            ++c->g_replays;
            c->last_split[{B, L}] = slot.split;
            return 0;
        }
        if (c->graphs.capture_due(slot)) {
            int r0 = check_ready(c);
            if (r0) return r0;
            const CallPlan cp = plan_call(c, B, L, true, workspace_bytes);
            if (condition && out && workspace && cp.whole.valid && workspace_bytes >= cp.whole.total && ((uintptr_t)workspace & 255) == 0) {
                slot.need = cp.need;
                slot.split = cp.split;
                HIP_TRY(c, hipSetDevice(c->device));
                if (!c->g_stream) HIP_TRY(c, hipStreamCreateWithFlags(&c->g_stream, hipStreamNonBlocking));
                hipGraphExec_t exec = nullptr;
                if (hipStreamBeginCapture(c->g_stream, hipStreamCaptureModeThreadLocal) == hipSuccess) {
                    const int r = separate_any(c, mixture, condition, out, cf, cp, workspace, workspace_bytes, c->g_stream, who);
                    hipGraph_t graph = nullptr;
                    const hipError_t e = hipStreamEndCapture(c->g_stream, &graph);
                    if (!(r == 0 && e == hipSuccess && graph && hipGraphInstantiate(&exec, graph, nullptr, nullptr, 0) == hipSuccess))
                        exec = nullptr;
                    if (graph) (void)hipGraphDestroy(graph);
                }
                if (exec) {
                    c->graphs.set_exec(slot, exec);
                    ++c->g_captures;
                    HIP_TRY(c, hipGraphLaunch(exec, (hipStream_t)stream));
                    return 0;
                }
                (void)hipGetLastError();
                c->use_graph = false;
                c->err.clear();
            }
        }
    }
    const CallPlan cp = plan_call(c, B, L, false, workspace_bytes);
    return separate_any(c, mixture, condition, out, cf, cp, workspace, workspace_bytes, (hipStream_t)stream, who);
}

int lass_separate(lass_ctx* c, const float* mixture, const float* condition, float* out, int B, int L, void* workspace,
                  size_t workspace_bytes, void* stream) {
    if (!c) return LASS_ERR_ARG;
    return separate_call(c, mixture, condition, out, ClipForm{B, L}, workspace, workspace_bytes, stream, "lass_separate");
}

int lass_ragged_bucket(const lass_ctx* c, int L, int* lo, int* hi) {
    if (!c || L <= c->g.nfft / 2) return LASS_ERR_ARG;
    const int T = 1 + L / c->g.hop, Tp = (T + 31) / 32 * 32;
    if (lo) *lo = std::max(c->g.hop * (Tp - 32), c->g.nfft / 2 + 1);
    if (hi) *hi = L;
    return 0;
}

int lass_separate_ragged(lass_ctx* c, const float* mixture, const int* lengths, const float* condition, float* out, int B, int L,
                         void* workspace, size_t workspace_bytes, void* stream) {
    if (!c) return LASS_ERR_ARG;
    if (!lengths) return fail(c, LASS_ERR_ARG, "lass_separate_ragged: null lengths");
    return separate_call(c, mixture, condition, out, ClipForm{B, L, lengths}, workspace, workspace_bytes, stream, "lass_separate_ragged");
}

static int separate_windows(lass_ctx* c, const std::string& who, const float* recording, int64_t total, const int64_t* starts,
                            const int* keep, const int* fade, const float* ramp, int F, const float* condition, float* out, int B,
                            int W, void* workspace, size_t workspace_bytes, void* stream) {
    if (!recording || !starts || !keep || !condition || !out || !workspace) return fail(c, LASS_ERR_ARG, who + ": null pointer");
    if (B <= 0) return fail(c, LASS_ERR_ARG, who + ": need B >= 1");
    if (W <= c->g.nfft / 2)
        return fail(c, LASS_ERR_ARG, who + ": a window must be longer than the reflect padding (W > " + std::to_string(c->g.nfft / 2) + ")");
    if (total < W) return fail(c, LASS_ERR_ARG, who + ": the recording is shorter than one window (total < W)");
    const uintptr_t r0 = (uintptr_t)recording, o0 = (uintptr_t)out, bytes = (uintptr_t)total * sizeof(float);
    if (r0 < o0 + bytes && o0 < r0 + bytes) return fail(c, LASS_ERR_ARG, who + ": recording and out overlap");
    return separate_call(c, recording, condition, out, ClipForm{B, W, nullptr, starts, keep, total, fade, ramp, F}, workspace,
                         workspace_bytes, stream, who.c_str());
}

int lass_separate_windows(lass_ctx* c, const float* recording, int64_t total, const int64_t* starts, const int* keep,
                          const float* condition, float* out, int B, int W, void* workspace, size_t workspace_bytes, void* stream) {
    if (!c) return LASS_ERR_ARG;
    return separate_windows(c, "lass_separate_windows", recording, total, starts, keep, nullptr, nullptr, 0, condition, out, B, W,
                            workspace, workspace_bytes, stream);
}

int lass_separate_windows_faded(lass_ctx* c, const float* recording, int64_t total, const int64_t* starts, const int* keep,
                                const int* fade, const float* ramp, int F, const float* condition, float* out, int B, int W,
                                void* workspace, size_t workspace_bytes, void* stream) {
    if (!c) return LASS_ERR_ARG;
    const std::string who = "lass_separate_windows_faded";
    if (!fade || !ramp) return fail(c, LASS_ERR_ARG, who + ": null pointer");
    if (F < 1 || F > W) return fail(c, LASS_ERR_ARG, who + ": the fade length must lie in [1, W]");
    return separate_windows(c, who, recording, total, starts, keep, fade, ramp, F, condition, out, B, W, workspace, workspace_bytes,
                            stream);
}

int lass_set_graph_replay(lass_ctx* c, int enabled) {
    if (!c) return LASS_ERR_ARG;
    c->use_graph = enabled != 0;
    return 0;
}

int lass_set_wino4_splits(lass_ctx* c, int splits) {
    if (!c || (splits != 0 && splits != 1 && splits != 2 && splits != 4)) return fail(c, LASS_ERR_ARG, "lass_set_wino4_splits: 0, 1, 2 or 4");
    c->cfg.ksplit_force = splits;
    ++c->gen;
    return 0;
}

int lass_set_wino4_vprep(lass_ctx* c, int mode) {
    if (!c || mode < 0 || mode > 2) return fail(c, LASS_ERR_ARG, "lass_set_wino4_vprep: 0, 1 or 2");
    c->cfg.vprep_mode = mode;
    ++c->gen;
    return 0;
}

int lass_set_head_fold(lass_ctx* c, int enabled) {
    if (!c || (enabled != 0 && enabled != 1)) return fail(c, LASS_ERR_ARG, "lass_set_head_fold: 0 or 1");
    c->cfg.head_fold = enabled != 0;
    ++c->gen;
    return 0;
}

int lass_set_head_sc_fold(lass_ctx* c, int enabled) {
    if (!c || (enabled != 0 && enabled != 1)) return fail(c, LASS_ERR_ARG, "lass_set_head_sc_fold: 0 or 1");
    c->cfg.head_sc_fold = enabled != 0;
    ++c->gen;
    return 0;
}

int lass_set_pw_split(lass_ctx* c, int enabled) {
    if (!c || (enabled != 0 && enabled != 1)) return fail(c, LASS_ERR_ARG, "lass_set_pw_split: 0 or 1");
    c->cfg.pw_split = enabled != 0;
    ++c->gen;
    return 0;
}

int lass_set_wino4_gemm(lass_ctx* c, int enabled) {
    if (!c || (enabled != 0 && enabled != 1)) return fail(c, LASS_ERR_ARG, "lass_set_wino4_gemm: 0 or 1");
    c->cfg.wino4_gemm = enabled != 0;
    ++c->gen;
    return 0;
}

int lass_set_wino4_vprep_buffer(lass_ctx* c, float* v, size_t floats) {
    if (!c || (v && !floats)) return fail(c, LASS_ERR_ARG, "lass_set_wino4_vprep_buffer: a buffer and its size, or NULL");
    c->stage_v_user = v;
    c->stage_v_user_floats = v ? floats : 0;
    return 0;
}

int lass_graph_stats(const lass_ctx* c, long* captures, long* replays) {
    if (!c) return LASS_ERR_ARG;
    if (captures) *captures = c->g_captures;
    if (replays) *replays = c->g_replays;
    return c->use_graph ? 1 : 0;
}

int lass_separate_components(lass_ctx* c, const float* const* mag, const float* cos_mask, const float* sin_mask,
                             const float* condition, float* out, int B, int L, void* workspace, size_t workspace_bytes,
                             void* stream) {
    if (!c) return LASS_ERR_ARG;
    if (!mag || !cos_mask || !sin_mask) return fail(c, LASS_ERR_ARG, "lass_separate_components: null pointer");
    Components comp;
    for (int k = 0; k < kMaxBranches; ++k) comp.mag[k] = k < c->g.nbr ? mag[k] : nullptr;
    comp.cosv = cos_mask; comp.sinv = sin_mask;
    return separate_impl(c, nullptr, &comp, condition, out, ClipForm{B, L}, make_plan(c, B, L), workspace, workspace_bytes, stream,
                         "lass_separate_components");
}

int lass_set_profiling(lass_ctx* c, int enabled) {
    if (!c) return LASS_ERR_ARG;
    if (enabled && c->ev_pool.size() < 2 * kProfPairs) {
        HIP_TRY(c, hipSetDevice(c->device));
        c->pending.reserve(kProfPairs);
        while (c->ev_pool.size() < 2 * kProfPairs) {
            hipEvent_t e;
            HIP_TRY(c, hipEventCreate(&e));
            c->ev_pool.push_back(e);
        }
    }
    c->profiling = enabled != 0;
    return 0;
}
int lass_profile_count(const lass_ctx* c) { return c ? P_COUNT : LASS_ERR_ARG; }
int lass_profile_get(lass_ctx* c, int i, const char** name, double* ms, int* launches) {
    if (!c || i < 0 || i >= P_COUNT) return LASS_ERR_ARG;
    prof_collect(c);
    if (name) *name = c->prof[i].name;
    if (ms) *ms = c->prof[i].ms;
    if (launches) *launches = c->prof[i].launches;
    return 0;
}
int lass_profile_reset(lass_ctx* c) {
    if (!c) return LASS_ERR_ARG;
    prof_collect(c);
    for (auto& p : c->prof) { p.ms = 0; p.launches = 0; }
    return 0;
}

}
```

### lass_amd/csrc/kernels.h

```cpp
#pragma once
#include <hip/hip_runtime.h>
#include <stddef.h>
#include <stdint.h>

#include "conv_route.h"

struct ConvArgs {
    const float* in = nullptr;
    long in_bs = 0;
    int Cin = 0;
    const float* w = nullptr;
    int Nw = 0;
    const float* pro_scale = nullptr;
    const float* pro_shift = nullptr;
    int pro_shift_bs = 0;
    const float* in2 = nullptr;
    long in2_bs = 0;
    int Cin2 = 0;
    const float* w2 = nullptr;
    const float* bias = nullptr;
    const float* res = nullptr;
    long res_bs = 0;
    const float* epi_scale = nullptr;
    const float* epi_shift = nullptr;
    int epi_shift_bs = 0;
    float* out = nullptr;
    long out_bs = 0;
    int B = 0, H = 0, W = 0;
    int N = 0;
    int up_h = 1;
    const float* w_wino = nullptr;
    const float* w2_wino = nullptr;
    const float* w_wino4 = nullptr;
    const void* w_bf16 = nullptr;
    const void* w2_bf16 = nullptr;
    const void* w_bf16_lo = nullptr;
    const void* w2_bf16_lo = nullptr;
    void* out_bf16 = nullptr;
    void* out_bf16_lo = nullptr;
    const void* in_bf16 = nullptr;
    const void* in_bf16_lo = nullptr;
    void* out_bf16_act = nullptr;
    const float* act_scale = nullptr;
    const float* act_shift = nullptr;
    int act_shift_bs = 0;
    int out_oct0 = 0;
    int out_noct = 0;
    const void* in2_bf16 = nullptr;
    void* pool_bf16 = nullptr;
    void* pool_bf16_act = nullptr;
    int pool_oct0 = 0;
    int pool_noct = 0;
    const float* pool_act_scale = nullptr;
    const float* pool_act_shift = nullptr;
    const float* pre_w = nullptr;
    const float* pre_b = nullptr;
    const float* mask_w = nullptr;
    const float* mask_b = nullptr;
    const float* mask_mag = nullptr;
    const float* mask_cos = nullptr;
    const float* mask_sin = nullptr;
    float* mask_re = nullptr;
    float* mask_im = nullptr;
    int mask_T = 0;
    int mask_nbins = LASS_NBINS;
    float* pool_out = nullptr;
    long pool_bs = 0;
    int pool_h = 2;
    int gx = 0, gy = 0;
    int xcd_map = 0;
};

struct Wino4Split {
    int n = 1;
    float* part = nullptr;
};

struct Wino4VPre {
    float* v = nullptr;
};

struct HeadScPlanes {
    float* skip = nullptr;
    float* up = nullptr;
    const float* w = nullptr;
};

inline ConvShape lass_conv_shape(const ConvArgs& p) {
    ConvShape s;
    s.Cin = p.Cin; s.N = p.N; s.Nw = p.Nw; s.H = p.H; s.W = p.W;
    s.Cin2 = p.Cin2; s.pool = p.pool_out != nullptr; s.pool_h = p.pool_h; s.head = p.mask_re != nullptr;
    return s;
}

hipError_t lass_launch_conv(ConvKind kind, const ConvArgs& p, hipStream_t stream);
bool lass_tconv_logits_supported(const ConvArgs& p, const HeadScPlanes& hs);
hipError_t lass_launch_tconv_logits(const ConvArgs& p, const HeadScPlanes& hs, hipStream_t stream);

bool lass_wino_supported(const ConvArgs& p);
hipError_t lass_launch_wino(ConvKind kind, const ConvArgs& p, hipStream_t stream);
hipError_t lass_launch_wino_weights(const float* w, int Cout, int Cin, float* U, hipStream_t stream);
hipError_t lass_launch_wino_shortcut_weights(const float* w, int Cout, int Cin, float* U, hipStream_t stream);

bool lass_wino4_supported(ConvKind kind, const ConvArgs& p, const Wino4Split& sk = Wino4Split());
hipError_t lass_launch_wino4(ConvKind kind, const ConvArgs& p, hipStream_t stream, const Wino4Split& sk = Wino4Split(),
                             const Wino4VPre& vp = Wino4VPre());
bool lass_wino4_vpre_supported(ConvKind kind, const ConvArgs& p, const Wino4Split& sk = Wino4Split());
hipError_t lass_launch_wino4_weights(const float* w, int Cout, int Cin, float* U, hipStream_t stream);
bool lass_wino4_headfold_supported(const ConvArgs& p);
hipError_t lass_launch_wino4_headfold(const ConvArgs& p, hipStream_t stream);
bool lass_wino4_headfold_planes_supported(const ConvArgs& p, const HeadScPlanes& hs);
hipError_t lass_launch_wino4_headfold_planes(const ConvArgs& p, const HeadScPlanes& hs, hipStream_t stream);
bool lass_wino4_sclogit_supported(const ConvArgs& p, const HeadScPlanes& hs);
hipError_t lass_launch_wino4_sclogit(const ConvArgs& p, const HeadScPlanes& hs, hipStream_t stream);

struct Wino4Gemm {
    const void* w3 = nullptr;
    float* m = nullptr;
};
bool lass_wino4_gemm_supported(ConvKind kind, const ConvArgs& p, const Wino4VPre& vp, const Wino4Gemm& g);
hipError_t lass_launch_wino4_gemm(ConvKind kind, const ConvArgs& p, const Wino4VPre& vp, const Wino4Gemm& g, hipStream_t stream);
hipError_t lass_launch_wino4_gemm_weights(const float* U, int Cout, int Cin, void* dst, hipStream_t stream);

struct PwSplitW {
    const void* w = nullptr;
};
bool lass_pw_gemm_supported(ConvKind kind, const ConvArgs& p);
hipError_t lass_launch_pw_gemm(ConvKind kind, const ConvArgs& p, hipStream_t stream, const PwSplitW& sw = PwSplitW());
hipError_t lass_launch_pw_split_weights(const float* w, int K, int Nw, void* dst, hipStream_t stream);

bool lass_bf16_supported(const ConvArgs& p);
hipError_t lass_launch_conv_bf16(ConvKind kind, const ConvArgs& p, hipStream_t stream);
hipError_t lass_launch_weights_bf16(const float* w, int Cout, int Cin, int taps, void* dst, int lo, int transposed,
                                    hipStream_t stream);

bool lass_enc1_fused_bf16_supported(const ConvArgs& p, const ConvArgs& q);
hipError_t lass_launch_enc1_fused_bf16(const ConvArgs& p, const ConvArgs& q, hipStream_t stream);
bool lass_dec6_fused_bf16_supported(const ConvArgs& p, const ConvArgs& q);
hipError_t lass_launch_dec6_fused_bf16(const ConvArgs& p, const ConvArgs& q, hipStream_t stream);

bool lass_dec6u_fused_bf16_supported(const ConvArgs& p, const ConvArgs& q, const ConvArgs& u);
hipError_t lass_launch_dec6u_fused_bf16(const ConvArgs& p, const ConvArgs& q, const ConvArgs& u, hipStream_t stream);
hipError_t lass_launch_compose_up_shortcut(const float* wsc, const float* wt, int Cin, int Cup, int Ccat, int Nsc, float* out,
                                           hipStream_t stream);

hipError_t lass_launch_multi_stft(const float* wav, int B, int L, int hop, int nwin, const int* n_fft,
                                  const float2* tw2k, float* const* mag, float* const* cosv, float* const* sinv,
                                  hipStream_t stream);
struct StftBranch {
    int wlen = 0;
    float *mag = nullptr, *cosv = nullptr, *sinv = nullptr, *real = nullptr, *imag = nullptr, *x0 = nullptr;
};
struct ClipForm {
    int B = 0;
    int L = 0;
    const int* lengths = nullptr;
    const int64_t* starts = nullptr;
    const int* keep = nullptr;
    int64_t total = 0;
    const int* fade = nullptr;
    const float* ramp = nullptr;
    int F = 0;
};
hipError_t lass_launch_stft2(const float* wav, const ClipForm& cf, int n_fft, int hop, int T, int Tpad, int nbr,
                             const StftBranch* br, int magphase_sem, const float* s0, const float* h0,
                             const float2* tw2k, hipStream_t stream);
hipError_t lass_launch_istft2(const float* real, const float* imag, const ClipForm& cf, int T, int n_fft, int wlen, int hop,
                              const float2* tw2k, float* wav, hipStream_t stream);

hipError_t lass_launch_film(const float* cond, int B, const float* Wf, const float* bf, const float* base, int n,
                            float* out, hipStream_t stream);
hipError_t lass_launch_pool(const float* in, long in_bs, int B, int C, int H, int W, int ph, int pw, float* out,
                            hipStream_t stream);
hipError_t lass_launch_mask(const float* x12, const float* wa, const float* ba, const float* mag, const float* cosv,
                            const float* sinv, int B, int T, int Tpad, int fcrop, float* out_real, float* out_imag,
                            hipStream_t stream);
hipError_t lass_launch_x0_from_mag(const float* mag, int B, int T, int Tpad, int fcrop, const float* s0,
                                   const float* h0, float* x0, hipStream_t stream);
hipError_t lass_launch_sdr(const float* ref, const float* est, int B, int L, double* stats, hipStream_t stream);
hipError_t lass_launch_mix_at_snr(float* source, const float* noise, const float* snr_db, float* mixture, int B, int L,
                                  double* ws, hipStream_t stream);
hipError_t lass_launch_segment_mix(const float* waveforms, int B, int L, const int* mix_num, const float* comp_db, int max_comp,
                                   const float* noise_db, float* mixture, float* segment, double* ws, hipStream_t stream);
hipError_t lass_launch_relayout_conv(const float* src, int Cout, int Cin, int taps, float* dst, hipStream_t stream);
hipError_t lass_launch_bnfold(const float* g, const float* beta, const float* mean, const float* var, int C, float eps,
                              float* scale, float* base, hipStream_t stream);

size_t lass_resample_table_floats(int up, int n_taps);
hipError_t lass_launch_decode_resample(const void* raw, long long row_stride, int B, int frames, int ch, int enc, int up, int down,
                                       const float* taps, int n_taps, bool planar, float* out, int L_out, hipStream_t stream);
size_t lass_resample_span_floats(int up, int down, int n_taps, int tile);

hipError_t lass_launch_resample_encode(const float* planes, long long row_stride, long long plane_stride, int B, int ch, int L_in,
                                       int up, int down, const float* taps, int n_taps, int enc, void* out, long long out_row_stride,
                                       int frames_out, unsigned* clipped, hipStream_t stream);
hipError_t lass_launch_resample_encode_gain(const float* planes, long long row_stride, long long plane_stride, int B, int ch, int L_in,
                                            int up, int down, const float* taps, int n_taps, int enc, void* out,
                                            long long out_row_stride, int frames_out, unsigned* clipped, const float* gain,
                                            hipStream_t stream);
hipError_t lass_launch_resample_peak(const float* planes, long long row_stride, long long plane_stride, int B, int ch, int L_in, int up,
                                     int down, const float* taps, int n_taps, int frames_out, float* peak, hipStream_t stream);
hipError_t lass_launch_resample_true_peak(const float* planes, long long row_stride, long long plane_stride, int B, int ch, int L_in,
                                          int up, int down, const float* taps, int n_taps, int frames_out, int os, const float* os_taps,
                                          int n_os_taps, float* peak, hipStream_t stream);
bool lass_resample_true_peak_fits(int up, int down, int n_taps, int os);

struct LoudnessFilter {
    double coef[10];
    double lane_step[16];
    double bin_step[16];
};
int lass_loudness_lanes(int hop);
bool lass_loudness_filter(const double* coef, int hop, LoudnessFilter* f);
hipError_t lass_launch_loudness(const float* planes, long long row_stride, long long plane_stride, int B, int ch, int L,
                                const int* lengths, int hop, const LoudnessFilter& f, const float* weights, double* out,
                                double* blocks, int nb_max, double* scratch, hipStream_t stream);
hipError_t lass_launch_loudness_stats(const float* planes, long long row_stride, long long plane_stride, int B, int ch, int L,
                                      const int* lengths, int hop, const LoudnessFilter& f, const float* weights, double* out,
                                      double* blocks, int nb_max, double* short_term, int ns_max, double* scratch, hipStream_t stream);
hipError_t lass_launch_loudness_gain(const double* loudness, const float* peak, int B, double target, float ceiling, float* gain,
                                     int* limited, hipStream_t stream);
```

### lass_amd/csrc/wino4.hip

```cpp
#include <hip/hip_runtime.h>
#include "head_fold.h"
#include "kernels.h"
#include "pixel_ops.h"
#include "wino4_transform.h"
#include "wino_common.h"

namespace {

constexpr int F_PRO = 1, F_PHASEB = 2, F_BIAS = 4, F_RES = 8, F_EPIACT = 16, F_PRECONV = 64, F_RESPRE = 128, F_MASK = 1024;
constexpr int F_SPLITK = 2048;
constexpr int F_SCLOGIT = 8192;
constexpr int F_VPRE = 4096;
constexpr int NTHREADS = 256;
constexpr int KC = kWino4KC;
constexpr int NXI = kWino4NXI;
constexpr int U_F = NXI * 256;
constexpr int V_F = kWino4VFloats;

typedef float f32x2v __attribute__((ext_vector_type(2)));


template <int TC, int FLAGS>
__global__ __launch_bounds__(NTHREADS, 2) void wino4_kernel(ConvArgs p) {
    const Wino4Split sk;
    const Wino4VPre vp;
    const HeadScPlanes hs;
#include "wino4_body.h"
}
template <int TC, int FLAGS0>
__global__ __launch_bounds__(NTHREADS, 2) void wino4_splitk_kernel(ConvArgs p, Wino4Split sk) {
    constexpr int FLAGS = FLAGS0 | F_SPLITK;
    const Wino4VPre vp;
    const HeadScPlanes hs;
#include "wino4_body.h"
}
template <int TC, int FLAGS0>
__global__ __launch_bounds__(NTHREADS, 2) void wino4_vpre_kernel(ConvArgs p, Wino4Split sk, Wino4VPre vp) {
    constexpr int FLAGS = FLAGS0 | F_VPRE;
    const HeadScPlanes hs;
#include "wino4_body.h"
}
template <int TC, int FLAGS0>
__global__ __launch_bounds__(NTHREADS, 2) void wino4_sclogit_kernel(ConvArgs p, HeadScPlanes hs) {
    constexpr int FLAGS = FLAGS0 | F_SCLOGIT;
    const Wino4Split sk;
    const Wino4VPre vp;
#include "wino4_body.h"
}

template <int TC>
__global__ __launch_bounds__(NTHREADS, 3) void wino4_headfold_kernel(ConvArgs p) {
    constexpr bool PLANES = false;
    const HeadScPlanes hs;
#include "wino4_head_body.h"
}
template <int TC>
__global__ __launch_bounds__(NTHREADS, 3) void wino4_headfold_planes_kernel(ConvArgs p, HeadScPlanes hs) {
    constexpr bool PLANES = true;
#include "wino4_head_body.h"
}

template <int TC, int FLAGS>
__global__ __launch_bounds__(NTHREADS) void wino4_vprep_kernel(ConvArgs p, Wino4VPre vp) {
    constexpr bool PRO = (FLAGS & F_PRO) != 0, PRE = false;
    static_assert((FLAGS & ~F_PRO) == 0, "a prologue at most");
    constexpr int TR = 32 / TC;
    constexpr int OR_ = 4 * TR, OC = 4 * TC;
    __shared__ __attribute__((aligned(16))) float lv[V_F];
    const int tid = threadIdx.x;
    const unsigned nchunk = (unsigned)(p.Cin / KC);
    const unsigned lin = blockIdx.x;
    const int ch = (int)(lin % nchunk);
    const int bx_ = (int)(lin / nchunk % (unsigned)p.gx), b = (int)(lin / nchunk / (unsigned)p.gx);
    const int tiles_x = p.W / OC;
    const int y0 = (bx_ / tiles_x) * OR_, x0 = (bx_ % tiles_x) * OC;
    const int HW = p.H * p.W;
    const float* in_b = p.in + (size_t)b * p.in_bs;
    const float* sc = PRO ? p.pro_scale : nullptr;
    const float* sh = PRO ? p.pro_shift + (size_t)b * p.pro_shift_bs : nullptr;
#include "wino4_input.h"
    pload(ch);
    pprocess();
    __syncthreads();
    float4* dst = reinterpret_cast<float4*>(vp.v + (((size_t)b * p.gx + bx_) * nchunk + ch) * V_F);
    const float4* src = reinterpret_cast<const float4*>(lv);
#pragma unroll
    for (int i = 0; i < V_F / 4 / NTHREADS; ++i) dst[i * NTHREADS + tid] = src[i * NTHREADS + tid];
}

template <int FLAGS>
__global__ __launch_bounds__(256) void wino4_combine_kernel(ConvArgs p, Wino4Split sk) {
    constexpr bool EPI = (FLAGS & F_EPIACT) != 0, RES = (FLAGS & F_RES) != 0;
    static_assert(EPI != RES && (FLAGS & ~(F_EPIACT | F_RES)) == 0, "conv1 or the identity conv2");
    const int W4 = p.W / 4, H2 = p.H / 2, HW = p.H * p.W;
    const long idx = (long)blockIdx.x * 256 + threadIdx.x;
    if (idx >= (long)p.B * p.N * H2 * W4) return;
    const int xq = (int)(idx % W4), yh = (int)(idx / W4 % H2), n = (int)(idx / ((long)W4 * H2) % p.N), b = (int)(idx / ((long)W4 * H2 * p.N));
    const size_t pix = (size_t)(2 * yh) * p.W + 4 * xq;
    const size_t split_pitch = (size_t)p.B * p.N * HW;
    const float* pp = sk.part + ((size_t)b * p.N + n) * HW + pix;
    float4 v[2];
#pragma unroll
    for (int i = 0; i < 2; ++i) v[i] = *reinterpret_cast<const float4*>(pp + (size_t)i * p.W);
    for (int s = 1; s < sk.n; ++s)
#pragma unroll
        for (int i = 0; i < 2; ++i) {
            const float4 t = *reinterpret_cast<const float4*>(pp + (size_t)s * split_pitch + (size_t)i * p.W);
            v[i].x += t.x; v[i].y += t.y; v[i].z += t.z; v[i].w += t.w;
        }
    if (EPI) {
        const float es = p.epi_scale[n], eh = p.epi_shift[(size_t)b * p.epi_shift_bs + n];
#pragma unroll
        for (int i = 0; i < 2; ++i) {
            v[i].x = leaky(fmaf(v[i].x, es, eh)); v[i].y = leaky(fmaf(v[i].y, es, eh));
            v[i].z = leaky(fmaf(v[i].z, es, eh)); v[i].w = leaky(fmaf(v[i].w, es, eh));
        }
    }
    if (RES) {
        const float* rr = p.res + (size_t)b * p.res_bs + (size_t)n * HW + pix;
        float4 t[2];
#pragma unroll
        for (int i = 0; i < 2; ++i) t[i] = *reinterpret_cast<const float4*>(rr + (size_t)i * p.W);
#pragma unroll
        for (int i = 0; i < 2; ++i) { v[i].x += t[i].x; v[i].y += t[i].y; v[i].z += t[i].z; v[i].w += t[i].w; }
    }
    float* dst = p.out + (size_t)b * p.out_bs + (size_t)n * HW + pix;
#pragma unroll
    for (int i = 0; i < 2; ++i) *reinterpret_cast<float4*>(dst + (size_t)i * p.W) = v[i];
    if (RES && p.pool_out) {
        const int Wo = p.W / 2, Ho = p.H / p.pool_h;
        float* pd = p.pool_out + (size_t)b * (p.pool_bs ? (size_t)p.pool_bs : (size_t)p.N * Ho * Wo) + (size_t)n * Ho * Wo + 2 * xq;
        if (p.pool_h == 2) {
            float s0 = v[0].x + v[0].y, s1 = v[0].z + v[0].w;
            s0 += v[1].x; s0 += v[1].y;
            s1 += v[1].z; s1 += v[1].w;
            *reinterpret_cast<float2*>(pd + (size_t)yh * Wo) = make_float2(s0 * 0.25f, s1 * 0.25f);
        } else {
#pragma unroll
            for (int i = 0; i < 2; ++i)
                *reinterpret_cast<float2*>(pd + (size_t)(2 * yh + i) * Wo) = make_float2((v[i].x + v[i].y) * 0.5f, (v[i].z + v[i].w) * 0.5f);
        }
    }
}

__global__ __launch_bounds__(256) void wino4_weights_kernel(const float* __restrict__ w, int Cout, int Cin, float* __restrict__ U) {
    const long i = (long)blockIdx.x * 256 + threadIdx.x;
    if (i >= (long)Cout * Cin) return;
    const int co = (int)(i % Cout), ci = (int)(i / Cout);
    const float* g = w + ((size_t)co * Cin + ci) * 9;
    const double G[6][3] = {{0.25, 0, 0},           {-1.0 / 6, -1.0 / 6, -1.0 / 6}, {-1.0 / 6, 1.0 / 6, -1.0 / 6},
                            {1.0 / 24, 1.0 / 12, 1.0 / 6}, {1.0 / 24, -1.0 / 12, 1.0 / 6},  {0, 0, 1}};
    double t[6][3];
    for (int a = 0; a < 6; ++a)
        for (int c = 0; c < 3; ++c) t[a][c] = G[a][0] * (double)g[0 * 3 + c] + G[a][1] * (double)g[1 * 3 + c] + G[a][2] * (double)g[2 * 3 + c];
    float* slab = U + ((size_t)(ci / 8) * (Cout / 32) + co / 32) * U_F;
    const int e = (((co & 31) >> 4) * 4 + (ci & 3)) * 32 + (co & 15) * 2 + ((ci & 7) >> 2);
    for (int a = 0; a < 6; ++a)
        for (int c = 0; c < 6; ++c) {
            const double u = t[a][0] * G[c][0] + t[a][1] * G[c][1] + t[a][2] * G[c][2];
            slab[(a * 6 + c) * 256 + e] = (float)u;
        }
}

template <int TC, int FLAGS>
hipError_t launch_wino4_tc(const ConvArgs& p0, hipStream_t stream) {
    ConvArgs p = p0;
    constexpr int OR_ = 4 * (32 / TC), OC = 4 * TC;
    p.gx = (p.W / OC) * ((p.H + OR_ - 1) / OR_);
    p.gy = p.N / 32;
    p.xcd_map = ((long)p.gx * p.B) % 8 == 0;
    hipLaunchKernelGGL((wino4_kernel<TC, FLAGS>), dim3((unsigned)((long)p.gx * p.gy * p.B)), dim3(NTHREADS), 0, stream, p);
    return hipGetLastError();
}

template <int FLAGS>
hipError_t launch_wino4(const ConvArgs& p, hipStream_t stream) {
    const int tc = lass_wino4_block_tc(p.H, p.W);
    if (tc == 16) return launch_wino4_tc<16, FLAGS>(p, stream);
    if (tc == 8) return launch_wino4_tc<8, FLAGS>(p, stream);
    if constexpr (FLAGS == (F_PRO | F_EPIACT) || FLAGS == F_RES)
        if (tc == 4) return launch_wino4_tc<4, FLAGS>(p, stream);
    return hipErrorInvalidValue;
}

template <int TC>
hipError_t launch_wino4_headfold_tc(const ConvArgs& p0, hipStream_t stream) {
    ConvArgs p = p0;
    constexpr int OR_ = 4 * (32 / TC), OC = 4 * TC;
    p.gx = (p.W / OC) * (p.H / OR_);
    p.gy = 1;
    p.xcd_map = ((long)p.gx * p.B) % 8 == 0;
    hipLaunchKernelGGL((wino4_headfold_kernel<TC>), dim3((unsigned)((long)p.gx * p.B)), dim3(NTHREADS), 0, stream, p);
    return hipGetLastError();
}

template <int TC>
hipError_t launch_wino4_headfold_planes_tc(const ConvArgs& p0, const HeadScPlanes& hs, hipStream_t stream) {
    ConvArgs p = p0;
    constexpr int OR_ = 4 * (32 / TC), OC = 4 * TC;
    p.gx = (p.W / OC) * (p.H / OR_);
    p.gy = 1;
    p.xcd_map = ((long)p.gx * p.B) % 8 == 0;
    hipLaunchKernelGGL((wino4_headfold_planes_kernel<TC>), dim3((unsigned)((long)p.gx * p.B)), dim3(NTHREADS), 0, stream, p, hs);
    return hipGetLastError();
}

template <int TC>
hipError_t launch_wino4_sclogit_tc(const ConvArgs& p0, const HeadScPlanes& hs, hipStream_t stream) {
    ConvArgs p = p0;
    constexpr int OR_ = 4 * (32 / TC), OC = 4 * TC;
    p.gx = (p.W / OC) * (p.H / OR_);
    p.gy = p.N / 32;
    p.xcd_map = ((long)p.gx * p.B) % 8 == 0;
    hipLaunchKernelGGL((wino4_sclogit_kernel<TC, F_RES | F_RESPRE>), dim3((unsigned)((long)p.gx * p.gy * p.B)), dim3(NTHREADS), 0, stream, p, hs);
    return hipGetLastError();
}

template <int TC, int MAIN, int COMB>
hipError_t launch_wino4_vpre_tc(const ConvArgs& p0, const Wino4Split& sk, const Wino4VPre& vp, bool pro, hipStream_t stream) {
    ConvArgs p = p0;
    constexpr int OR_ = 4 * (32 / TC), OC = 4 * TC;
    constexpr bool SPLIT = (MAIN & F_SPLITK) != 0;
    const int n = SPLIT ? sk.n : 1;
    p.gx = (p.W / OC) * (p.H / OR_);
    p.gy = p.N / 32;
    p.xcd_map = ((long)p.gx * p.B * n) % 8 == 0;
    const dim3 pgrid((unsigned)((long)p.gx * (p.Cin / KC) * p.B));
    if (pro)
        hipLaunchKernelGGL((wino4_vprep_kernel<TC, F_PRO>), pgrid, dim3(NTHREADS), 0, stream, p, vp);
    else
        hipLaunchKernelGGL((wino4_vprep_kernel<TC, 0>), pgrid, dim3(NTHREADS), 0, stream, p, vp);
    if (hipError_t e = hipGetLastError()) return e;
    Wino4Split s1 = sk;
    if (!SPLIT) s1 = Wino4Split();
    hipLaunchKernelGGL((wino4_vpre_kernel<TC, MAIN>), dim3((unsigned)((long)p.gx * p.gy * p.B * n)), dim3(NTHREADS), 0, stream, p, s1, vp);
    if (hipError_t e = hipGetLastError()) return e;
    if constexpr (SPLIT) {
        const long items = (long)p.B * p.N * (p.H / 2) * (p.W / 4);
        hipLaunchKernelGGL((wino4_combine_kernel<COMB>), dim3((unsigned)((items + 255) / 256)), dim3(256), 0, stream, p, sk);
        return hipGetLastError();
    }
    return hipSuccess;
}

template <int EPI>
hipError_t launch_wino4_vpre(const ConvArgs& p, const Wino4Split& sk, const Wino4VPre& vp, hipStream_t stream) {
    constexpr bool pro = EPI == F_EPIACT;
    const int tc = lass_wino4_block_tc(p.H, p.W);
    if (tc == 16) return launch_wino4_vpre_tc<16, EPI, 0>(p, sk, vp, pro, stream);
    if (tc == 8) return launch_wino4_vpre_tc<8, EPI, 0>(p, sk, vp, pro, stream);
    if (tc == 4)
        return sk.n > 1 ? launch_wino4_vpre_tc<4, F_SPLITK, EPI>(p, sk, vp, pro, stream) : launch_wino4_vpre_tc<4, EPI, 0>(p, sk, vp, pro, stream);
    return hipErrorInvalidValue;
}

template <int MAIN, int COMB>
hipError_t launch_wino4_split(const ConvArgs& p0, const Wino4Split& sk, hipStream_t stream) {
    ConvArgs p = p0;
    p.gx = (p.W / 16) * (p.H / 32);
    p.gy = p.N / 32;
    p.xcd_map = ((long)p.gx * p.B * sk.n) % 8 == 0;
    hipLaunchKernelGGL((wino4_splitk_kernel<4, MAIN>), dim3((unsigned)((long)p.gx * p.gy * p.B * sk.n)), dim3(NTHREADS), 0, stream, p, sk);
    if (hipError_t e = hipGetLastError()) return e;
    const long items = (long)p.B * p.N * (p.H / 2) * (p.W / 4);
    hipLaunchKernelGGL((wino4_combine_kernel<COMB>), dim3((unsigned)((items + 255) / 256)), dim3(256), 0, stream, p, sk);
    return hipGetLastError();
}

}

bool lass_wino4_supported(ConvKind kind, const ConvArgs& p, const Wino4Split& sk) {
    if (!lass_wino4_shape(kind, lass_conv_shape(p), sk.n) || !p.w_wino4 || (sk.n != 1 && !sk.part)) return false;
    switch (kind) {
        case CONV1_ACT:
            return true;
        case CONV1_ACT_PRE:
            return p.pre_w && p.pre_b;
        case CONV2_IDENT_PRE:
            return p.res && p.pre_w && p.pre_b;
        case CONV2_IDENT:
            return p.res != nullptr;
        case CONV2_SHORTCUT:
            if (!(p.in2 && p.w2 && p.bias)) return false;
            return !p.mask_re || (p.W + 1 == p.mask_nbins && p.mask_w && p.mask_b && p.mask_mag && p.mask_cos && p.mask_sin && p.mask_im &&
                                  p.mask_T > 0 && p.mask_T <= p.H);
        default:
            return false;
    }
}

bool lass_wino4_vpre_supported(ConvKind kind, const ConvArgs& p, const Wino4Split& sk) {
    return lass_wino4_vpre_shape(kind, lass_conv_shape(p), sk.n) && lass_wino4_supported(kind, p, sk);
}

hipError_t lass_launch_wino4(ConvKind kind, const ConvArgs& p, hipStream_t stream, const Wino4Split& sk, const Wino4VPre& vp) {
    if (!lass_wino4_supported(kind, p, sk) || !p.in || (!p.out && !p.mask_re)) return hipErrorInvalidValue;
    if (vp.v) {
        if (!lass_wino4_vpre_supported(kind, p, sk)) return hipErrorInvalidValue;
        if (kind == CONV1_ACT) {
            if (!p.pro_scale || !p.pro_shift || !p.epi_scale || !p.epi_shift) return hipErrorInvalidValue;
            return launch_wino4_vpre<F_EPIACT>(p, sk, vp, stream);
        }
        return launch_wino4_vpre<F_RES>(p, sk, vp, stream);
    }
    switch (kind) {
        case CONV1_ACT:
        case CONV1_ACT_PRE:
            if (!p.pro_scale || !p.pro_shift || !p.epi_scale || !p.epi_shift) return hipErrorInvalidValue;
            if (sk.n > 1) return launch_wino4_split<F_PRO, F_EPIACT>(p, sk, stream);
            return kind == CONV1_ACT ? launch_wino4<F_PRO | F_EPIACT>(p, stream) : launch_wino4<F_PRO | F_EPIACT | F_PRECONV>(p, stream);
        case CONV2_IDENT:
            if (sk.n > 1) return launch_wino4_split<0, F_RES>(p, sk, stream);
            return launch_wino4<F_RES>(p, stream);
        case CONV2_IDENT_PRE:
            return launch_wino4<F_RES | F_RESPRE>(p, stream);
        case CONV2_SHORTCUT:
            return p.mask_re ? launch_wino4<F_PHASEB | F_BIAS | F_MASK>(p, stream) : launch_wino4<F_PHASEB | F_BIAS>(p, stream);
        default:
            return hipErrorInvalidValue;
    }
}

bool lass_wino4_headfold_supported(const ConvArgs& p) {
    return lass_wino4_headfold_shape(lass_conv_shape(p)) && p.in && p.w_wino4 && p.in2 && p.w2 && p.bias && p.W + 1 == p.mask_nbins &&
           p.mask_mag && p.mask_cos && p.mask_sin && p.mask_re && p.mask_im && p.mask_T > 0 && p.mask_T <= p.H;
}

hipError_t lass_launch_wino4_headfold(const ConvArgs& p, hipStream_t stream) {
    if (!lass_wino4_headfold_supported(p)) return hipErrorInvalidValue;
    return launch_wino4_headfold_tc<16>(p, stream);
}

bool lass_wino4_headfold_planes_supported(const ConvArgs& p, const HeadScPlanes& hs) {
    return lass_wino4_headfold_supported(p) && hs.skip && hs.up;
}

hipError_t lass_launch_wino4_headfold_planes(const ConvArgs& p, const HeadScPlanes& hs, hipStream_t stream) {
    if (!lass_wino4_headfold_planes_supported(p, hs)) return hipErrorInvalidValue;
    return launch_wino4_headfold_planes_tc<16>(p, hs, stream);
}

bool lass_wino4_sclogit_supported(const ConvArgs& p, const HeadScPlanes& hs) {
    return lass_wino4_supported(CONV2_IDENT_PRE, p) && lass_wino4_block_tc(p.H, p.W) == 16 && p.in && p.out && hs.skip && hs.w;
}

hipError_t lass_launch_wino4_sclogit(const ConvArgs& p, const HeadScPlanes& hs, hipStream_t stream) {
    if (!lass_wino4_sclogit_supported(p, hs)) return hipErrorInvalidValue;
    return launch_wino4_sclogit_tc<16>(p, hs, stream);
}

hipError_t lass_launch_wino4_weights(const float* w, int Cout, int Cin, float* U, hipStream_t stream) {
    const long n = (long)Cout * Cin;
    hipLaunchKernelGGL(wino4_weights_kernel, dim3((unsigned)((n + 255) / 256)), dim3(256), 0, stream, w, Cout, Cin, U);
    return hipGetLastError();
}
```

### lass_amd/csrc/wino4_body.h

```cpp
    constexpr bool PRO = (FLAGS & F_PRO) != 0, EPI = (FLAGS & F_EPIACT) != 0, SC = (FLAGS & F_PHASEB) != 0;
    constexpr bool PRE = (FLAGS & F_PRECONV) != 0;
    constexpr bool RESPRE = (FLAGS & F_RESPRE) != 0;
    constexpr bool MASK = (FLAGS & F_MASK) != 0;
    constexpr bool RES = (FLAGS & F_RES) != 0;
    static_assert(!SC || (FLAGS & F_BIAS) != 0, "the shortcut conv has a bias");
    static_assert(!PRE || PRO, "pre_conv is folded into the prologue's affine");
    static_assert(!RESPRE || ((FLAGS & F_RES) != 0 && !SC && !EPI), "conv2 with the identity residual");
    static_assert(!MASK || SC, "the output head sits behind decoder_block6's conv2 + shortcut");
    static_assert(!RES || (!SC && !EPI), "conv2 with a residual in place of the fused shortcut");
    constexpr bool SPLIT = (FLAGS & F_SPLITK) != 0;
    static_assert(!SPLIT || (FLAGS & ~(F_SPLITK | F_PRO | F_VPRE)) == 0, "a split launch has a prologue at most");
    constexpr bool VPRE = (FLAGS & F_VPRE) != 0;
    static_assert(!VPRE || (FLAGS & ~(F_VPRE | F_SPLITK | F_EPIACT | F_RES)) == 0, "conv1 / identity conv2 / split share: the prologue ran in the prep launch");
    constexpr bool SCL = (FLAGS & F_SCLOGIT) != 0;
    static_assert(!SCL || (FLAGS == (F_RES | F_RESPRE | F_SCLOGIT) && TC == 16), "the skip's logits: encoder_block1.conv2 on the 8 x 64 blocks");
    constexpr int TR = 32 / TC;
    constexpr int OR_ = 4 * TR, OC = 4 * TC;
    constexpr int NCO = 32;
    __shared__ __attribute__((aligned(16))) float lds[U_F + V_F + 2 * NCO + (MASK ? 100 : 0) + (SCL ? 96 : 0)];
    float* lu = lds;
    float* lv = lds + U_F;
    float* lds_es = lv + V_F;
    float* lds_eh = lds_es + NCO;
    float* lds_mw = lds_eh + NCO;

    const int tid = threadIdx.x;
    const int lane = tid & 63, wave = __builtin_amdgcn_readfirstlane(tid >> 6);
    const int wco = wave >> 1, wwt = wave & 1;
    int bx_, by_, b, ks = 0;
    if constexpr (SPLIT) {
        const unsigned lin = blockIdx.x, ngrp = (unsigned)(p.gx * p.B * sk.n);
        unsigned grp;
        if (p.xcd_map) {
            const unsigned j = lin >> 3;
            grp = (lin & 7u) * (ngrp >> 3) + j / (unsigned)p.gy;
            by_ = (int)(j % (unsigned)p.gy);
        } else {
            grp = lin / (unsigned)p.gy;
            by_ = (int)(lin % (unsigned)p.gy);
        }
        ks = (int)(grp % (unsigned)sk.n);
        const unsigned xz = grp / (unsigned)sk.n;
        b = (int)(xz / (unsigned)p.gx);
        bx_ = (int)(xz % (unsigned)p.gx);
    } else {
        block_coords(p, bx_, by_, b);
    }
    const int n0 = by_ * NCO;
    const int tiles_x = p.W / OC;
    const int y0 = (bx_ / tiles_x) * OR_, x0 = (bx_ % tiles_x) * OC;
    const int HW = p.H * p.W;
    const float* in_b = p.in + (size_t)b * p.in_bs;
    const float* sc = PRO ? p.pro_scale : nullptr;
    const float* sh = PRO ? p.pro_shift + (size_t)b * p.pro_shift_bs : nullptr;

    if (EPI && tid < NCO) {
        lds_es[tid] = p.epi_scale[n0 + tid];
        lds_eh[tid] = p.epi_shift[(size_t)b * p.epi_shift_bs + n0 + tid];
    }
    if (SC && tid < NCO) lds_es[tid] = p.bias[n0 + tid];
    if (RESPRE && tid < 32) {
        lds_es[tid] = p.pre_w[n0 + tid];
        lds_eh[tid] = p.pre_b[n0 + tid];
    }
    if (MASK && tid < 99) lds_mw[tid] = tid < 96 ? p.mask_w[tid] : p.mask_b[tid - 96];
    if constexpr (SCL) {
        if (tid < 96) lds_mw[tid] = hs.w[tid];
    }

    f32x4 acc[NXI];
#pragma unroll
    for (int xi = 0; xi < NXI; ++xi)
#pragma unroll
        for (int r = 0; r < 4; ++r) acc[xi][r] = 0.f;

    const int kq = lane >> 4, l15 = lane & 15;
    const float* afrag = lu + (wco >> 1) * U_F + (wco & 1) * 128 + (kq * 16 + l15) * 2;
    const float* bfrag = lv + (kq * 32 + ((wwt * 16 + l15) ^ ((kq & 1) << 4))) * 2;
    const unsigned slab_pitch = (unsigned)(p.Nw / 32) * (unsigned)(U_F * 4);
    const unsigned slab_n0 = (unsigned)(n0 / 32) * (unsigned)(U_F * 4);
    const unsigned lu_addr = (unsigned)(size_t)(__attribute__((address_space(3))) float*)lu;
    const unsigned ulane = (unsigned)lane * 16u;
    const v4i32 uw = make_rsrc_words(p.w_wino4, (unsigned)(NXI * p.Cin * p.Nw) * 4u);

#include "wino4_input.h"
    const unsigned lv_addr = (unsigned)(size_t)(__attribute__((address_space(3))) float*)lv;
    const v4i32 vw = make_rsrc_words(VPRE ? vp.v + ((size_t)b * p.gx + bx_) * (size_t)(p.Cin / KC) * V_F : nullptr,
                                     (unsigned)(p.Cin / KC) * (unsigned)(V_F * 4));

    const int ch0 = SPLIT ? ks * (p.Cin / KC) / sk.n : 0;
    const int nch = SPLIT ? (ks + 1) * (p.Cin / KC) / sk.n : p.Cin / KC;
    if constexpr (!VPRE) pload(ch0);
    lds_barrier();
    for (int ch = ch0; ch < nch; ++ch) {
        lds_barrier();
        __builtin_amdgcn_s_setprio(2);
        if constexpr (!VPRE) {
#pragma unroll
            for (int i = 0; i < 6; ++i) {
                asm volatile("" : "+v"(pc[i].x), "+v"(pc[i].y), "+v"(pc[i].z), "+v"(pc[i].w), "+v"(pl[i]), "+v"(pr[i]));
            }
            if (PRO) asm volatile("" : "+v"(ps), "+v"(ph));
        }
#pragma unroll
        for (int i = 0; i < 9; ++i) {
            const unsigned piece = (unsigned)(wave * 9 + i) * 1024u;
            lds_dma_16B(uw, ulane, (unsigned)ch * slab_pitch + slab_n0 + piece, lu_addr + piece);
        }
        if constexpr (VPRE) {
#pragma unroll
            for (int i = 0; i < 9; ++i) {
                const unsigned piece = (unsigned)(wave * 9 + i) * 1024u;
                lds_dma_16B(vw, ulane, (unsigned)ch * (unsigned)(V_F * 4) + piece, lv_addr + piece);
            }
            wait_vmcnt<0>();
        } else {
            __builtin_amdgcn_sched_barrier(0);
            pprocess();
            __builtin_amdgcn_sched_barrier(0);
            const bool pf = ch + 1 < nch;
            if (pf) pload(ch + 1);
            __builtin_amdgcn_sched_barrier(0);
            if (pf)
                wait_vmcnt<NLOAD>();
            else
                wait_vmcnt<0>();
        }
        lds_barrier();
        __builtin_amdgcn_s_setprio(0);
        constexpr int PFD = 2;
        f32x2v av[PFD + 1][2], bv[PFD + 1][2];
        auto rd = [&](int s) {
#pragma unroll
            for (int q = 0; q < 2; ++q) {
                av[s % (PFD + 1)][q] = *reinterpret_cast<const f32x2v*>(afrag + (2 * s + q) * 256);
                bv[s % (PFD + 1)][q] = *reinterpret_cast<const f32x2v*>(bfrag + (2 * s + q) * 256);
            }
        };
#pragma unroll
        for (int s = 0; s < PFD; ++s) rd(s);
#pragma unroll
        for (int s = 0; s < NXI / 2; ++s) {
            if (s + PFD < NXI / 2) rd(s + PFD);
            __builtin_amdgcn_sched_barrier(0);
            const f32x2v a0 = av[s % (PFD + 1)][0], a1 = av[s % (PFD + 1)][1];
            const f32x2v b0 = bv[s % (PFD + 1)][0], b1 = bv[s % (PFD + 1)][1];
            acc[2 * s] = __builtin_amdgcn_mfma_f32_16x16x4f32(a0.x, b0.x, acc[2 * s], 0, 0, 0);
            acc[2 * s + 1] = __builtin_amdgcn_mfma_f32_16x16x4f32(a1.x, b1.x, acc[2 * s + 1], 0, 0, 0);
            acc[2 * s] = __builtin_amdgcn_mfma_f32_16x16x4f32(a0.y, b0.y, acc[2 * s], 0, 0, 0);
            acc[2 * s + 1] = __builtin_amdgcn_mfma_f32_16x16x4f32(a1.y, b1.y, acc[2 * s + 1], 0, 0, 0);
            __builtin_amdgcn_sched_barrier(0);
        }
    }

    const int ot = wwt * 16 + l15;
    const int oy = y0 + 4 * (ot / TC), ox = x0 + 4 * (ot % TC);
    f32x4 ysp[16];
#pragma unroll
    for (int r = 0; r < 4; ++r) {
        const int nl = wco * 16 + kq * 4 + r;
        float tmp[4][6];
#pragma unroll
        for (int jx = 0; jx < 6; ++jx) {
            const float m[6] = {acc[0 + jx][r], acc[6 + jx][r], acc[12 + jx][r], acc[18 + jx][r], acc[24 + jx][r], acc[30 + jx][r]};
            float y[4];
            at6(m, y);
#pragma unroll
            for (int a = 0; a < 4; ++a) tmp[a][jx] = y[a];
        }
        const float es = (EPI || SC) ? lds_es[nl] : 0.f, eh = EPI ? lds_eh[nl] : 0.f;
#pragma unroll
        for (int a = 0; a < 4; ++a) {
            float y[4];
            at6(tmp[a], y);
#pragma unroll
            for (int c = 0; c < 4; ++c) {
                float v = y[c];
                if (EPI) v = leaky(fmaf(v, es, eh));
                if (SC) v += es;
                ysp[a * 4 + c][r] = v;
            }
        }
    }
    if constexpr (SPLIT) {
#pragma unroll
        for (int r = 0; r < 4; ++r) {
            const int n = n0 + wco * 16 + kq * 4 + r;
            float* dst = sk.part + (((size_t)ks * p.B + b) * p.N + n) * HW + (size_t)oy * p.W + ox;
#pragma unroll
            for (int a = 0; a < 4; ++a) {
                const float4 o = make_float4(ysp[a * 4 + 0][r], ysp[a * 4 + 1][r], ysp[a * 4 + 2][r], ysp[a * 4 + 3][r]);
                if (oy + a < p.H) *reinterpret_cast<float4*>(dst + (size_t)a * p.W) = o;
            }
        }
        return;
    }
    if constexpr (RESPRE) {
        const float* xr = p.res + (size_t)b * p.res_bs + (size_t)min(oy, p.H - 4) * p.W + ox;
        float4 xv[4];
#pragma unroll
        for (int a = 0; a < 4; ++a) xv[a] = *reinterpret_cast<const float4*>(xr + (size_t)a * p.W);
#pragma unroll
        for (int r = 0; r < 4; ++r) {
            const float pw = lds_es[wco * 16 + kq * 4 + r], pb = lds_eh[wco * 16 + kq * 4 + r];
#pragma unroll
            for (int a = 0; a < 4; ++a) {
                ysp[a * 4 + 0][r] += fmaf(xv[a].x, pw, pb);
                ysp[a * 4 + 1][r] += fmaf(xv[a].y, pw, pb);
                ysp[a * 4 + 2][r] += fmaf(xv[a].z, pw, pb);
                ysp[a * 4 + 3][r] += fmaf(xv[a].w, pw, pb);
            }
        }
    }
    if constexpr (SCL) {
        float* part = lds;
        lds_barrier();
#pragma unroll
        for (int q = 0; q < 3; ++q) {
            float w4[4];
#pragma unroll
            for (int r = 0; r < 4; ++r) w4[r] = lds_mw[q * 32 + wco * 16 + kq * 4 + r];
#pragma unroll
            for (int a = 0; a < 4; ++a) {
                float4 o;
                float* op = &o.x;
#pragma unroll
                for (int c = 0; c < 4; ++c) {
                    const f32x4 v = ysp[a * 4 + c];
                    op[c] = fmaf(v[3], w4[3], fmaf(v[2], w4[2], fmaf(v[1], w4[1], v[0] * w4[0])));
                }
                *reinterpret_cast<float4*>(part + ((wco * 4 + kq) * 3 + q) * 512 + ot * 16 + a * 4) = o;
            }
        }
    }
    if constexpr (RES && !RESPRE) {
        float4 rv[4][4];
#pragma unroll
        for (int r = 0; r < 4; ++r) {
            const float* rr = p.res + (size_t)b * p.res_bs + (size_t)(n0 + wco * 16 + kq * 4 + r) * HW + (size_t)min(oy, p.H - 4) * p.W + ox;
#pragma unroll
            for (int a = 0; a < 4; ++a) rv[r][a] = *reinterpret_cast<const float4*>(rr + (size_t)a * p.W);
        }
#pragma unroll
        for (int r = 0; r < 4; ++r)
#pragma unroll
            for (int a = 0; a < 4; ++a) {
                ysp[a * 4 + 0][r] += rv[r][a].x;
                ysp[a * 4 + 1][r] += rv[r][a].y;
                ysp[a * 4 + 2][r] += rv[r][a].z;
                ysp[a * 4 + 3][r] += rv[r][a].w;
            }
    }
    if constexpr (SC) {
        const float* x2 = p.in2 + (size_t)b * p.in2_bs + (size_t)min(oy, p.H - 4) * p.W + ox;
        const float* wsc = p.w2 + n0 + wco * 16 + l15;
        const int nks = p.Cin2 / 4;
        constexpr int NSB = 4;
        float4 xb[NSB][4];
        float wa[NSB];
        auto ldk = [&](int ks, int buf) {
            const float* xp = x2 + (size_t)(4 * ks + kq) * HW;
#pragma unroll
            for (int a = 0; a < 4; ++a) xb[buf][a] = *reinterpret_cast<const float4*>(xp + (size_t)a * p.W);
            wa[buf] = wsc[(size_t)(4 * ks + kq) * p.Nw];
        };
        auto mmk = [&](int buf) {
#pragma unroll
            for (int a = 0; a < 4; ++a) {
                ysp[a * 4 + 0] = __builtin_amdgcn_mfma_f32_16x16x4f32(wa[buf], xb[buf][a].x, ysp[a * 4 + 0], 0, 0, 0);
                ysp[a * 4 + 1] = __builtin_amdgcn_mfma_f32_16x16x4f32(wa[buf], xb[buf][a].y, ysp[a * 4 + 1], 0, 0, 0);
                ysp[a * 4 + 2] = __builtin_amdgcn_mfma_f32_16x16x4f32(wa[buf], xb[buf][a].z, ysp[a * 4 + 2], 0, 0, 0);
                ysp[a * 4 + 3] = __builtin_amdgcn_mfma_f32_16x16x4f32(wa[buf], xb[buf][a].w, ysp[a * 4 + 3], 0, 0, 0);
            }
        };
        ldk(0, 0);
        ldk(1, 1);
        ldk(2, 2);
        for (int ks = 0; ks < nks; ks += NSB) {
#pragma unroll
            for (int u = 0; u < NSB; ++u) {
                ldk(min(ks + u + 3, nks - 1), (u + 3) % NSB);
                __builtin_amdgcn_sched_barrier(0);
                mmk(u);
                __builtin_amdgcn_sched_barrier(0);
            }
        }
    }
    if constexpr (MASK) {
        float* part = lds;
        lds_barrier();
#pragma unroll
        for (int q = 0; q < 3; ++q) {
            float w4[4];
#pragma unroll
            for (int r = 0; r < 4; ++r) w4[r] = lds_mw[q * 32 + wco * 16 + kq * 4 + r];
#pragma unroll
            for (int a = 0; a < 4; ++a) {
                float4 o;
                float* op = &o.x;
#pragma unroll
                for (int c = 0; c < 4; ++c) {
                    const f32x4 v = ysp[a * 4 + c];
                    op[c] = v[0] * w4[0] + v[1] * w4[1] + v[2] * w4[2] + v[3] * w4[3];
                }
                *reinterpret_cast<float4*>(part + ((wco * 4 + kq) * 3 + q) * 512 + ot * 16 + a * 4) = o;
            }
        }
        lds_barrier();
        const int px = tid * 2;
        const int mt = px >> 4, ms = px & 15;
        const int my = y0 + 4 * (mt / TC) + (ms >> 2), mx = x0 + 4 * (mt % TC) + (ms & 3);
        float lg[3][2];
#pragma unroll
        for (int q = 0; q < 3; ++q) {
            float2 sum = make_float2(lds_mw[96 + q], lds_mw[96 + q]);
#pragma unroll
            for (int src = 0; src < 8; ++src) {
                const float2 v = *reinterpret_cast<const float2*>(part + (src * 3 + q) * 512 + px);
                sum.x += v.x;
                sum.y += v.y;
            }
            lg[q][0] = sum.x;
            lg[q][1] = sum.y;
        }
        if (my < p.mask_T) {
            mask_pixel(p, b, my, mx, lg[0][0], lg[1][0], lg[2][0]);
            mask_pixel(p, b, my, mx + 1, lg[0][1], lg[1][1], lg[2][1]);
        }
        return;
    }
#pragma unroll
    for (int r = 0; r < 4; ++r) {
        const int n = n0 + wco * 16 + kq * 4 + r;
        float* dst = p.out + (size_t)b * p.out_bs + (size_t)n * HW + (size_t)oy * p.W + ox;
#pragma unroll
        for (int a = 0; a < 4; ++a) {
            const float4 o = make_float4(ysp[a * 4 + 0][r], ysp[a * 4 + 1][r], ysp[a * 4 + 2][r], ysp[a * 4 + 3][r]);
            if (oy + a < p.H) *reinterpret_cast<float4*>(dst + (size_t)a * p.W) = o;
        }
        if constexpr (TC == 4 && RES) {
            if (p.pool_out && p.pool_h == 1) {
                const int Wo = p.W / 2;
                float* pd = p.pool_out + (size_t)b * (p.pool_bs ? (size_t)p.pool_bs : (size_t)p.N * p.H * Wo) + (size_t)n * p.H * Wo +
                            (size_t)oy * Wo + (ox >> 1);
#pragma unroll
                for (int a = 0; a < 4; ++a) {
                    float2 o;
                    o.x = (ysp[a * 4 + 0][r] + ysp[a * 4 + 1][r]) * 0.5f;
                    o.y = (ysp[a * 4 + 2][r] + ysp[a * 4 + 3][r]) * 0.5f;
                    if (oy + a < p.H) *reinterpret_cast<float2*>(pd + (size_t)a * Wo) = o;
                }
                continue;
            }
        }
        if ((SC || RES) && p.pool_out) {
            const int Ho = p.H / 2, Wo = p.W / 2;
            float* pd = p.pool_out + (size_t)b * (p.pool_bs ? (size_t)p.pool_bs : (size_t)p.N * Ho * Wo) + (size_t)n * Ho * Wo +
                        (size_t)(oy >> 1) * Wo + (ox >> 1);
#pragma unroll
            for (int i = 0; i < 2; ++i) {
                float2 o;
                float s0 = ysp[(2 * i) * 4 + 0][r] + ysp[(2 * i) * 4 + 1][r];
                s0 += ysp[(2 * i + 1) * 4 + 0][r];
                s0 += ysp[(2 * i + 1) * 4 + 1][r];
                float s1 = ysp[(2 * i) * 4 + 2][r] + ysp[(2 * i) * 4 + 3][r];
                s1 += ysp[(2 * i + 1) * 4 + 2][r];
                s1 += ysp[(2 * i + 1) * 4 + 3][r];
                o.x = s0 * 0.25f;
                o.y = s1 * 0.25f;
                if (oy + 2 * i + 1 < p.H) *reinterpret_cast<float2*>(pd + (size_t)i * Wo) = o;
            }
        }
    }
    if constexpr (SCL) {
        const float* part = lds;
        lds_barrier();
        const int px = tid * 2;
        const int mt = px >> 4, ms = px & 15;
        const int my = y0 + 4 * (mt / TC) + (ms >> 2), mx = x0 + 4 * (mt % TC) + (ms & 3);
#pragma unroll
        for (int q = 0; q < 3; ++q) {
            float2 sum = *reinterpret_cast<const float2*>(part + q * 512 + px);
#pragma unroll
            for (int src = 1; src < 8; ++src) {
                const float2 v = *reinterpret_cast<const float2*>(part + (src * 3 + q) * 512 + px);
                sum.x += v.x;
                sum.y += v.y;
            }
            if (my < p.H) *reinterpret_cast<float2*>(hs.skip + ((size_t)b * 3 + q) * HW + (size_t)my * p.W + mx) = sum;
        }
    }
```

### lass_amd/csrc/wino4_gemm.hip

```cpp
#include <hip/hip_runtime.h>
#include "pw_gemm_split.h"
#include "wino4_transform.h"

namespace {

constexpr int F_PRO = 1, F_RES = 8, F_EPIACT = 16;
constexpr int NXI = kWino4NXI;
constexpr int U_F = NXI * 256;
constexpr int V_F = kWino4VFloats;

__host__ __device__ inline unsigned tiles_of(const ConvArgs& p) { return (unsigned)p.B * (unsigned)p.gx * 32u; }

template <int TC, int FLAGS>
__global__ __launch_bounds__(NTHREADS) void wino4_scatter_kernel(ConvArgs p, Wino4VPre vp) {
    constexpr bool PRO = (FLAGS & F_PRO) != 0, PRE = false;
    static_assert((FLAGS & ~F_PRO) == 0, "a prologue at most");
    constexpr int KC = kWino4KC;
    constexpr int TR = 32 / TC;
    constexpr int OR_ = 4 * TR, OC = 4 * TC;
    __shared__ __attribute__((aligned(16))) float lv[V_F];
    const int tid = threadIdx.x;
    const unsigned nchunk = (unsigned)(p.Cin / KC);
    const unsigned lin = blockIdx.x;
    const int ch = (int)(lin % nchunk);
    const int bx_ = (int)(lin / nchunk % (unsigned)p.gx), b = (int)(lin / nchunk / (unsigned)p.gx);
    const int tiles_x = p.W / OC;
    const int y0 = (bx_ / tiles_x) * OR_, x0 = (bx_ % tiles_x) * OC;
    const int HW = p.H * p.W;
    const float* in_b = p.in + (size_t)b * p.in_bs;
    const float* sc = PRO ? p.pro_scale : nullptr;
    const float* sh = PRO ? p.pro_shift + (size_t)b * p.pro_shift_bs : nullptr;
#include "wino4_input.h"
    pload(ch);
    pprocess();
    __syncthreads();
    const size_t Pt = tiles_of(p);
    float* dst = vp.v + (size_t)(ch * KC) * Pt + ((size_t)b * p.gx + bx_) * 32;
#pragma unroll
    for (int it = 0; it < NXI * KC * 8 / NTHREADS; ++it) {
        const int i = it * NTHREADS + tid;
        const int q = i & 7, c = (i >> 3) & 7, xi = i >> 6;
        const float* src = lv + xi * 256 + ((c & 3) * 32 + ((4 * q) ^ ((c & 1) << 4))) * 2 + (c >> 2);
        const float4 o = make_float4(src[0], src[2], src[4], src[6]);
        *reinterpret_cast<float4*>(dst + ((size_t)xi * p.Cin + c) * Pt + 4 * q) = o;
    }
}

template <bool ACC2>
__global__ __launch_bounds__(NTHREADS, 2) void wino4_gemm_kernel(ConvArgs p, PwSplitW sw) {
    constexpr bool TCONV = false, XI = true;
#include "pw_gemm_split_body.h"
}

template <int TC, int FLAGS>
__global__ __launch_bounds__(256) void wino4_gather_kernel(ConvArgs p, const float* __restrict__ m) {
    constexpr bool EPI = (FLAGS & F_EPIACT) != 0, RES = (FLAGS & F_RES) != 0;
    static_assert(EPI != RES && (FLAGS & ~(F_EPIACT | F_RES)) == 0, "conv1 or the identity conv2");
    constexpr int OR_ = 4 * (32 / TC), OC = 4 * TC;
    const size_t Pt = tiles_of(p);
    const size_t idx = (size_t)blockIdx.x * 256 + threadIdx.x;
    if (idx >= (size_t)p.N * Pt) return;
    const unsigned pp = (unsigned)(idx % Pt);
    const int n = (int)(idx / Pt);
    const int pt = (int)(pp & 31u);
    const unsigned blk = pp >> 5;
    const int bx_ = (int)(blk % (unsigned)p.gx), b = (int)(blk / (unsigned)p.gx);
    const int tiles_x = p.W / OC;
    const int oy = (bx_ / tiles_x) * OR_ + 4 * (pt / TC), ox = (bx_ % tiles_x) * OC + 4 * (pt % TC);
    const int HW = p.H * p.W;
    float acc[NXI];
    const float* mp = m + (size_t)n * Pt + pp;
#pragma unroll
    for (int xi = 0; xi < NXI; ++xi) acc[xi] = mp[(size_t)xi * p.N * Pt];
    float tmp[4][6];
#pragma unroll
    for (int jx = 0; jx < 6; ++jx) {
        const float mm[6] = {acc[0 + jx], acc[6 + jx], acc[12 + jx], acc[18 + jx], acc[24 + jx], acc[30 + jx]};
        float y[4];
        at6(mm, y);
#pragma unroll
        for (int a = 0; a < 4; ++a) tmp[a][jx] = y[a];
    }
    float ys[4][4];
#pragma unroll
    for (int a = 0; a < 4; ++a) at6(tmp[a], ys[a]);
    if (EPI) {
        const float es = p.epi_scale[n], eh = p.epi_shift[(size_t)b * p.epi_shift_bs + n];
#pragma unroll
        for (int a = 0; a < 4; ++a)
#pragma unroll
            for (int c = 0; c < 4; ++c) ys[a][c] = leaky(fmaf(ys[a][c], es, eh));
    }
    const size_t pix = (size_t)n * HW + (size_t)oy * p.W + ox;
    if (RES) {
        const float* rr = p.res + (size_t)b * p.res_bs + pix;
        float4 t[4];
#pragma unroll
        for (int a = 0; a < 4; ++a) t[a] = *reinterpret_cast<const float4*>(rr + (size_t)a * p.W);
#pragma unroll
        for (int a = 0; a < 4; ++a) { ys[a][0] += t[a].x; ys[a][1] += t[a].y; ys[a][2] += t[a].z; ys[a][3] += t[a].w; }
    }
    float* dst = p.out + (size_t)b * p.out_bs + pix;
#pragma unroll
    for (int a = 0; a < 4; ++a) *reinterpret_cast<float4*>(dst + (size_t)a * p.W) = make_float4(ys[a][0], ys[a][1], ys[a][2], ys[a][3]);
    if (RES && p.pool_out) {
        const int Wo = p.W / 2, Ho = p.H / p.pool_h;
        float* pd = p.pool_out + (size_t)b * (p.pool_bs ? (size_t)p.pool_bs : (size_t)p.N * Ho * Wo) + (size_t)n * Ho * Wo + (ox >> 1);
        if (p.pool_h == 2) {
#pragma unroll
            for (int i = 0; i < 2; ++i) {
                float s0 = ys[2 * i][0] + ys[2 * i][1], s1 = ys[2 * i][2] + ys[2 * i][3];
                s0 += ys[2 * i + 1][0]; s0 += ys[2 * i + 1][1];
                s1 += ys[2 * i + 1][2]; s1 += ys[2 * i + 1][3];
                *reinterpret_cast<float2*>(pd + (size_t)((oy >> 1) + i) * Wo) = make_float2(s0 * 0.25f, s1 * 0.25f);
            }
        } else {
#pragma unroll
            for (int a = 0; a < 4; ++a)
                *reinterpret_cast<float2*>(pd + (size_t)(oy + a) * Wo) = make_float2((ys[a][0] + ys[a][1]) * 0.5f, (ys[a][2] + ys[a][3]) * 0.5f);
        }
    }
}

__global__ __launch_bounds__(256) void wino4_gemm_weights_kernel(const float* __restrict__ U, int Cout, int Cin, bf16x8* __restrict__ dst) {
    const size_t plane = (size_t)(Cin / 8) * Cout, u = (size_t)blockIdx.x * 256 + threadIdx.x;
    if (u >= plane * NXI) return;
    const int xi = (int)(u / plane);
    const size_t r = u - (size_t)xi * plane;
    const int o = (int)(r / Cout), co = (int)(r - (size_t)o * Cout);
    const float* slab = U + ((size_t)o * (Cout / 32) + co / 32) * U_F + xi * 256;
    float x[8];
#pragma unroll
    for (int j = 0; j < 8; ++j) x[j] = slab[(((co & 31) >> 4) * 4 + (j & 3)) * 32 + (co & 15) * 2 + (j >> 2)];
    bf16x8 h, mm, l;
    split3(x, h, mm, l);
    bf16x8* d = dst + (size_t)xi * 3 * plane + r;
    d[0] = h;
    d[plane] = mm;
    d[2 * plane] = l;
}

template <int TC, int EPI>
hipError_t launch_tc(const ConvArgs& p0, const Wino4VPre& vp, const Wino4Gemm& g, hipStream_t stream) {
    ConvArgs p = p0;
    constexpr int OR_ = 4 * (32 / TC), OC = 4 * TC;
    p.gx = (p.W / OC) * (p.H / OR_);
    p.gy = p.N / 32;
    const unsigned Pt = tiles_of(p);
    const dim3 sgrid((unsigned)((long)p.gx * (p.Cin / kWino4KC) * p.B));
    if (EPI == F_EPIACT)
        hipLaunchKernelGGL((wino4_scatter_kernel<TC, F_PRO>), sgrid, dim3(NTHREADS), 0, stream, p, vp);
    else
        hipLaunchKernelGGL((wino4_scatter_kernel<TC, 0>), sgrid, dim3(NTHREADS), 0, stream, p, vp);
    if (hipError_t e = hipGetLastError()) return e;
    ConvArgs q;
    q.in2 = vp.v; q.in2_bs = (long)p.Cin * Pt; q.Cin2 = p.Cin;
    q.N = q.Nw = p.N; q.H = 1; q.W = (int)Pt; q.B = NXI;
    q.out = g.m; q.out_bs = (long)p.N * Pt;
    q.gx = (int)((Pt + PB - 1) / PB);
    q.gy = p.N / NB;
    q.xcd_map = ((long)q.gx * q.B) % 8 == 0;
    PwSplitW sw;
    sw.w = g.w3;
    hipLaunchKernelGGL(wino4_gemm_kernel<TC == 4>, dim3((unsigned)((long)q.gx * q.gy * q.B)), dim3(NTHREADS), 0, stream, q, sw);
    if (hipError_t e = hipGetLastError()) return e;
    const size_t items = (size_t)p.N * Pt;
    hipLaunchKernelGGL((wino4_gather_kernel<TC, EPI>), dim3((unsigned)((items + 255) / 256)), dim3(256), 0, stream, p, (const float*)g.m);
    return hipGetLastError();
}

template <int EPI>
hipError_t launch_geom(const ConvArgs& p, const Wino4VPre& vp, const Wino4Gemm& g, hipStream_t stream) {
    const int tc = lass_wino4_block_tc(p.H, p.W);
    if (tc == 16) return launch_tc<16, EPI>(p, vp, g, stream);
    if (tc == 8) return launch_tc<8, EPI>(p, vp, g, stream);
    if (tc == 4) return launch_tc<4, EPI>(p, vp, g, stream);
    return hipErrorInvalidValue;
}

}

bool lass_wino4_gemm_supported(ConvKind kind, const ConvArgs& p, const Wino4VPre& vp, const Wino4Gemm& g) {
    if (!lass_wino4_gemm_shape(kind, lass_conv_shape(p)) || p.B <= 0 || !p.in || !p.out || !vp.v || !g.m || !g.w3 || ((uintptr_t)g.w3 & 15u) ||
        ((uintptr_t)vp.v & 15u) || ((uintptr_t)g.m & 15u))
        return false;
    const unsigned long long Pt = (unsigned long long)p.B * (unsigned long long)(p.H * p.W / 16);
    if (Pt >= 0x7FFFFFFFull || Pt * (unsigned long long)p.N / 256ull >= 0x7FFFFFFFull) return false;
    if (kind == CONV1_ACT) return p.pro_scale && p.pro_shift && p.epi_scale && p.epi_shift;
    return kind == CONV2_IDENT && p.res && (!p.pool_out || p.pool_h == 1 || p.pool_h == 2);
}

hipError_t lass_launch_wino4_gemm(ConvKind kind, const ConvArgs& p, const Wino4VPre& vp, const Wino4Gemm& g, hipStream_t stream) {
    if (!lass_wino4_gemm_supported(kind, p, vp, g)) return hipErrorInvalidValue;
    return kind == CONV1_ACT ? launch_geom<F_EPIACT>(p, vp, g, stream) : launch_geom<F_RES>(p, vp, g, stream);
}

hipError_t lass_launch_wino4_gemm_weights(const float* U, int Cout, int Cin, void* dst, hipStream_t stream) {
    if (!U || !dst || Cin <= 0 || Cin % 8 != 0 || Cout <= 0 || Cout % 32 != 0 || ((uintptr_t)dst & 15u)) return hipErrorInvalidValue;
    const size_t units = (size_t)(Cin / 8) * Cout * NXI;
    hipLaunchKernelGGL(wino4_gemm_weights_kernel, dim3((unsigned)((units + 255) / 256)), dim3(256), 0, stream, U, Cout, Cin,
                       reinterpret_cast<bf16x8*>(dst));
    return hipGetLastError();
}
```

### lass_amd/csrc/wino4_head_body.h

```cpp
    constexpr bool PRO = false, PRE = false;
    constexpr int TR = 32 / TC;
    constexpr int OR_ = 4 * TR, OC = 4 * TC;
    constexpr int UH_F = kHeadFoldU4Floats;
    constexpr int NQ = 3;
    constexpr int NXW = NXI / 4;
    constexpr int XQ_F = NXI * 32 + 16, XK_F = NQ * XQ_F + 48, X_F = 2 * XK_F;
    static_assert(X_F % 4 == 0 && X_F + 2 * NQ * 512 <= UH_F + V_F, "the hand-over images fit into the dead U / V region");
    __shared__ __attribute__((aligned(16))) float lds[UH_F + V_F + kHeadFoldRows];
    float* lu = lds;
    float* lv = lds + UH_F;
    float* lds_b = lv + V_F;

    const int tid = threadIdx.x;
    const int lane = tid & 63, wave = __builtin_amdgcn_readfirstlane(tid >> 6);
    const int wk = wave >> 1, wwt = wave & 1;
    int bx_, by_, b;
    block_coords(p, bx_, by_, b);
    const int tiles_x = p.W / OC;
    const int y0 = (bx_ / tiles_x) * OR_, x0 = (bx_ % tiles_x) * OC;
    if (y0 >= p.mask_T) return;
    const int HW = p.H * p.W;
    const float* in_b = p.in + (size_t)b * p.in_bs;
    const float* sc = nullptr;
    const float* sh = nullptr;
    if (tid < kHeadFoldRows) lds_b[tid] = p.bias[tid];

    f32x4 acc[NXW];
#pragma unroll
    for (int g = 0; g < NXW; ++g)
#pragma unroll
        for (int r = 0; r < 4; ++r) acc[g][r] = 0.f;

    const int kq = lane >> 4, l15 = lane & 15;
    const int l31 = lane & 31, lks = lane >> 5;
    const float* afrag = lu + ((lks * kHeadFoldRows4 + (lane & 3)) * NXI + wave * NXW) * 4;
    const float* bfrag0 = lv + wave * NXW * 256 + l31 * 2 + lks;
    const float* bfrag1 = lv + wave * NXW * 256 + (l31 ^ 16) * 2 + lks;
    const unsigned lu_addr = (unsigned)(size_t)(__attribute__((address_space(3))) float*)lu;
    const unsigned ulane = (unsigned)lane * 16u;
    const v4i32 uw = make_rsrc_words(p.w_wino4, (unsigned)(p.Cin / KC) * (unsigned)(UH_F * 4));

#include "wino4_input.h"

    const int nch = p.Cin / KC;
    pload(0);
    lds_barrier();
    for (int ch = 0; ch < nch; ++ch) {
        lds_barrier();
        __builtin_amdgcn_s_setprio(2);
#pragma unroll
        for (int i = 0; i < 6; ++i) {
            asm volatile("" : "+v"(pc[i].x), "+v"(pc[i].y), "+v"(pc[i].z), "+v"(pc[i].w), "+v"(pl[i]), "+v"(pr[i]));
        }
        static_assert(UH_F == 5 * 256, "5 pieces");
        const unsigned slab = (unsigned)ch * (unsigned)(UH_F * 4);
        {
            const unsigned piece = (unsigned)wave * 1024u;
            lds_dma_16B(uw, ulane, slab + piece, lu_addr + piece);
        }
        if (wave == 0) lds_dma_16B(uw, ulane, slab + 4096u, lu_addr + 4096u);
        __builtin_amdgcn_sched_barrier(0);
        pprocess();
        __builtin_amdgcn_sched_barrier(0);
        const bool pf = ch + 1 < nch;
        if (pf) pload(ch + 1);
        __builtin_amdgcn_sched_barrier(0);
        if (pf)
            wait_vmcnt<NLOAD>();
        else
            wait_vmcnt<0>();
        lds_barrier();
        __builtin_amdgcn_s_setprio(0);
        f32x4 av[NXW];
        float bv[2][NXW];
        auto rdb = [&](int c) {
            const float* bp = ((c & 1) ? bfrag1 : bfrag0) + c * 64;
#pragma unroll
            for (int g = 0; g < NXW; ++g) bv[c & 1][g] = bp[g * 256];
        };
#pragma unroll
        for (int g = 0; g < NXW; ++g) av[g] = *reinterpret_cast<const f32x4*>(afrag + g * 4);
        rdb(0);
#pragma unroll
        for (int c = 0; c < 4; ++c) {
            if (c + 1 < 4) rdb(c + 1);
            __builtin_amdgcn_sched_barrier(0);
#pragma unroll
            for (int g = 0; g < NXW; ++g) acc[g] = __builtin_amdgcn_mfma_f32_4x4x1f32(av[g][c], bv[c & 1][g], acc[g], 0, 0, 0);
            __builtin_amdgcn_sched_barrier(0);
        }
    }

    float2 lsk[NQ], lup[NQ];
    if constexpr (PLANES) {
        const int ppx = tid * 2, pmt = ppx >> 4, pms = ppx & 15;
        const size_t po = (size_t)b * NQ * HW + (size_t)(y0 + 4 * (pmt / TC) + (pms >> 2)) * p.W + (x0 + 4 * (pmt % TC) + (pms & 3));
#pragma unroll
        for (int q = 0; q < NQ; ++q) {
            lsk[q] = *reinterpret_cast<const float2*>(hs.skip + po + (size_t)q * HW);
            lup[q] = *reinterpret_cast<const float2*>(hs.up + po + (size_t)q * HW);
        }
    }
    float* xh = lds;
    float* part = lds + X_F;
    lds_barrier();
#pragma unroll
    for (int g = 0; g < NXW; ++g)
#pragma unroll
        for (int r = 0; r < NQ; ++r) xh[lks * XK_F + r * XQ_F + (wave * NXW + g) * 32 + l31] = acc[g][r];
    lds_barrier();
    const int ot = wwt * 16 + l15;
    const int oy = y0 + 4 * (ot / TC), ox = x0 + 4 * (ot % TC);
    {
        const float* xs = xh + wk * XK_F + min(kq, NQ - 1) * XQ_F + ot;
        float mm[NXI];
#pragma unroll
        for (int xi = 0; xi < NXI; ++xi) mm[xi] = xs[xi * 32];
        float tmp[4][6];
#pragma unroll
        for (int jx = 0; jx < 6; ++jx) {
            const float m[6] = {mm[0 + jx], mm[6 + jx], mm[12 + jx], mm[18 + jx], mm[24 + jx], mm[30 + jx]};
            float y[4];
            at6(m, y);
#pragma unroll
            for (int a = 0; a < 4; ++a) tmp[a][jx] = y[a];
        }
#pragma unroll
        for (int a = 0; a < 4; ++a) {
            float y[4];
            at6(tmp[a], y);
            if (kq < NQ) *reinterpret_cast<float4*>(part + (wk * NQ + kq) * 512 + ot * 16 + a * 4) = make_float4(y[0], y[1], y[2], y[3]);
        }
    }
    if constexpr (!PLANES) {
        lds_barrier();
        f32x4 ysp[16];
#pragma unroll
        for (int a = 0; a < 4; ++a) {
            float4 yq[NQ];
#pragma unroll
            for (int q = 0; q < NQ; ++q) yq[q] = *reinterpret_cast<const float4*>(part + (wk * NQ + q) * 512 + ot * 16 + a * 4);
#pragma unroll
            for (int q = 0; q < NQ; ++q) {
                ysp[a * 4 + 0][q] = kq == 0 ? yq[q].x : 0.f;
                ysp[a * 4 + 1][q] = kq == 0 ? yq[q].y : 0.f;
                ysp[a * 4 + 2][q] = kq == 0 ? yq[q].z : 0.f;
                ysp[a * 4 + 3][q] = kq == 0 ? yq[q].w : 0.f;
            }
#pragma unroll
            for (int c = 0; c < 4; ++c) ysp[a * 4 + c][3] = 0.f;
        }
        const float* x2 = p.in2 + (size_t)b * p.in2_bs + (size_t)min(oy, p.H - 4) * p.W + ox;
        const float* wsc = p.w2 + l15;
        const int nks = p.Cin2 / 8, k0 = wk * nks;
        constexpr int NSB = 4;
        float4 xb[NSB][4];
        float wa[NSB];
        auto ldk = [&](int ks, int buf) {
            const float* xp = x2 + (size_t)(4 * ks + kq) * HW;
#pragma unroll
            for (int a = 0; a < 4; ++a) xb[buf][a] = *reinterpret_cast<const float4*>(xp + (size_t)a * p.W);
            wa[buf] = wsc[(size_t)(4 * ks + kq) * kHeadFoldRows];
        };
        auto mmk = [&](int buf) {
#pragma unroll
            for (int a = 0; a < 4; ++a) {
                ysp[a * 4 + 0] = __builtin_amdgcn_mfma_f32_16x16x4f32(wa[buf], xb[buf][a].x, ysp[a * 4 + 0], 0, 0, 0);
                ysp[a * 4 + 1] = __builtin_amdgcn_mfma_f32_16x16x4f32(wa[buf], xb[buf][a].y, ysp[a * 4 + 1], 0, 0, 0);
                ysp[a * 4 + 2] = __builtin_amdgcn_mfma_f32_16x16x4f32(wa[buf], xb[buf][a].z, ysp[a * 4 + 2], 0, 0, 0);
                ysp[a * 4 + 3] = __builtin_amdgcn_mfma_f32_16x16x4f32(wa[buf], xb[buf][a].w, ysp[a * 4 + 3], 0, 0, 0);
            }
        };
        ldk(k0, 0);
        ldk(k0 + 1, 1);
        ldk(k0 + 2, 2);
        for (int ks = 0; ks < nks; ks += NSB) {
#pragma unroll
            for (int u = 0; u < NSB; ++u) {
                ldk(k0 + min(ks + u + 3, nks - 1), (u + 3) % NSB);
                __builtin_amdgcn_sched_barrier(0);
                mmk(u);
                __builtin_amdgcn_sched_barrier(0);
            }
        }
        if (kq == 0) {
#pragma unroll
            for (int q = 0; q < NQ; ++q)
#pragma unroll
                for (int a = 0; a < 4; ++a)
                    *reinterpret_cast<float4*>(part + (wk * NQ + q) * 512 + ot * 16 + a * 4) =
                        make_float4(ysp[a * 4 + 0][q], ysp[a * 4 + 1][q], ysp[a * 4 + 2][q], ysp[a * 4 + 3][q]);
        }
    }
    lds_barrier();
    const int px = tid * 2;
    const int mt = px >> 4, ms = px & 15;
    const int my = y0 + 4 * (mt / TC) + (ms >> 2), mx = x0 + 4 * (mt % TC) + (ms & 3);
    float lg[NQ][2];
#pragma unroll
    for (int q = 0; q < NQ; ++q) {
        const float2 v0 = *reinterpret_cast<const float2*>(part + q * 512 + px);
        const float2 v1 = *reinterpret_cast<const float2*>(part + (NQ + q) * 512 + px);
        if constexpr (PLANES) {
            lg[q][0] = ((v0.x + v1.x) + (lsk[q].x + lup[q].x)) + lds_b[q];
            lg[q][1] = ((v0.y + v1.y) + (lsk[q].y + lup[q].y)) + lds_b[q];
        } else {
            lg[q][0] = (v0.x + v1.x) + lds_b[q];
            lg[q][1] = (v0.y + v1.y) + lds_b[q];
        }
    }
    if (my < p.mask_T) {
        mask_pixel(p, b, my, mx, lg[0][0], lg[1][0], lg[2][0]);
        mask_pixel(p, b, my, mx + 1, lg[0][1], lg[1][1], lg[2][1]);
    }
```

### lass_amd/csrc/wino4_input.h

```cpp
    const int pt = tid & 31, c8 = (tid & 255) >> 5;
    const int pty = pt / TC, ptx = pt % TC;
    const int gy0 = y0 + 4 * pty - 1, gx0 = x0 + 4 * ptx - 1;
    const bool left = gx0 < 0, right = gx0 + 5 >= p.W;
    unsigned vo_c[6], vo_l[6], vo_r[6], rowok = 0;
#pragma unroll
    for (int i = 0; i < 6; ++i) {
        const int gy = gy0 + i;
        const int row = (PRE ? 0 : c8 * HW) + min(max(gy, 0), p.H - 1) * p.W;
        vo_c[i] = 4u * (unsigned)(row + gx0 + 1);
        vo_l[i] = 4u * (unsigned)(row + (left ? 0 : gx0));
        vo_r[i] = 4u * (unsigned)(row + (right ? p.W - 1 : gx0 + 5));
        rowok |= (gy >= 0 && gy < p.H ? 1u : 0u) << i;
    }
    const __amdgpu_buffer_rsrc_t in_rsrc =
        __builtin_amdgcn_make_buffer_rsrc(const_cast<float*>(in_b), 0, (int)((unsigned)(PRE ? 1 : p.Cin) * (unsigned)HW * 4u), 0x00020000);
    const bool edge = left || right || rowok != 0x3fu;
    float4 pc[6];
    float pl[6], pr[6], ps = 1.f, ph = 0.f;
    const unsigned tvo = (unsigned)c8 * 4u;
    const auto tab_rsrc = [&](const float* t, int n) {
        return __builtin_amdgcn_make_buffer_rsrc(const_cast<float*>(t), 0, n * 4, 0x00020000);
    };
    const __amdgpu_buffer_rsrc_t sc_rsrc = tab_rsrc(PRO ? sc : p.in, p.Cin), sh_rsrc = tab_rsrc(PRO ? sh : p.in, p.Cin);
    const __amdgpu_buffer_rsrc_t pw_rsrc = tab_rsrc(PRE ? p.pre_w : p.in, 32), pb_rsrc = tab_rsrc(PRE ? p.pre_b : p.in, 32);
    auto pload = [&](int ch) {
        const unsigned soff = PRE ? 0u : (unsigned)(ch * KC * HW) * 4u;
        if (!PRE || ch == 0)
#pragma unroll
        for (int i = 0; i < 6; ++i) {
            pc[i] = __builtin_bit_cast(float4, __builtin_amdgcn_raw_buffer_load_b128(in_rsrc, (int)vo_c[i], (int)soff, 0));
            pl[i] = __builtin_bit_cast(float, __builtin_amdgcn_raw_buffer_load_b32(in_rsrc, (int)vo_l[i], (int)soff, 0));
            pr[i] = __builtin_bit_cast(float, __builtin_amdgcn_raw_buffer_load_b32(in_rsrc, (int)vo_r[i], (int)soff, 0));
        }
        const unsigned toff = (unsigned)(ch * KC) * 4u;
        if (PRO) {
            ps = __builtin_bit_cast(float, __builtin_amdgcn_raw_buffer_load_b32(sc_rsrc, (int)tvo, (int)toff, 0));
            ph = __builtin_bit_cast(float, __builtin_amdgcn_raw_buffer_load_b32(sh_rsrc, (int)tvo, (int)toff, 0));
        }
        if (PRE) {
            const float pw = __builtin_bit_cast(float, __builtin_amdgcn_raw_buffer_load_b32(pw_rsrc, (int)tvo, (int)toff, 0));
            const float pb = __builtin_bit_cast(float, __builtin_amdgcn_raw_buffer_load_b32(pb_rsrc, (int)tvo, (int)toff, 0));
            ph = fmaf(pb, ps, ph);
            ps = pw * ps;
        }
    };
    constexpr int NLOAD = (PRE ? 0 : 6 * 3) + (PRO ? 2 : 0) + (PRE ? 2 : 0);
    float* vdst = lv + ((c8 & 3) * 32 + (pt ^ ((c8 & 1) << 4))) * 2 + (c8 >> 2);
    auto pprocess = [&]() {
        float d[6][6];
#pragma unroll
        for (int i = 0; i < 6; ++i) {
            const float v[6] = {pl[i], pc[i].x, pc[i].y, pc[i].z, pc[i].w, pr[i]};
#pragma unroll
            for (int jx = 0; jx < 6; ++jx) d[i][jx] = PRO ? leaky(fmaf(v[jx], ps, ph)) : v[jx];
        }
        if (__builtin_amdgcn_ballot_w64(edge) != 0) {
            const bool r0 = (rowok & 1u) != 0, r5 = (rowok & 32u) != 0;
#pragma unroll
            for (int jx = 0; jx < 6; ++jx) {
                d[0][jx] = r0 ? d[0][jx] : 0.f;
                d[5][jx] = r5 ? d[5][jx] : 0.f;
            }
#pragma unroll
            for (int i = 0; i < 6; ++i) {
                d[i][0] = left ? 0.f : d[i][0];
                d[i][5] = right ? 0.f : d[i][5];
            }
        }
        float tt[6][6];
#pragma unroll
        for (int jx = 0; jx < 6; ++jx) {
            const float col[6] = {d[0][jx], d[1][jx], d[2][jx], d[3][jx], d[4][jx], d[5][jx]};
            float r[6];
            bt6(col, r);
#pragma unroll
            for (int i = 0; i < 6; ++i) tt[i][jx] = r[i];
        }
#pragma unroll
        for (int i = 0; i < 6; ++i) {
            float r[6];
            bt6(tt[i], r);
#pragma unroll
            for (int jx = 0; jx < 6; ++jx) vdst[(i * 6 + jx) * 256] = r[jx];
        }
    };
```

Before: 1184 clips/s.

## Let Winograd F4 blocks walk several spatial tiles, prefetching the next tile's input

```diff
diff --git a/include/lass_hip.h b/include/lass_hip.h
--- a/include/lass_hip.h
+++ b/include/lass_hip.h
@@ -65,6 +65,7 @@
 int lass_set_head_sc_fold(lass_ctx* ctx, int enabled);
 int lass_set_pw_split(lass_ctx* ctx, int enabled);
 int lass_set_wino4_gemm(lass_ctx* ctx, int enabled);
+int lass_set_wino4_walk(lass_ctx* ctx, int n);
 int lass_set_wino4_vprep_buffer(lass_ctx* ctx, float* v, size_t floats);
 
 int lass_separate_components(lass_ctx* ctx, const float* const* mag, const float* cos_mask, const float* sin_mask,
diff --git a/lass_amd/_lib.py b/lass_amd/_lib.py
--- a/lass_amd/_lib.py
+++ b/lass_amd/_lib.py
@@ -71,6 +71,7 @@
     ("lass_set_head_sc_fold", c_int, [c_void_p, c_int]),
     ("lass_set_pw_split", c_int, [c_void_p, c_int]),
     ("lass_set_wino4_gemm", c_int, [c_void_p, c_int]),
+    ("lass_set_wino4_walk", c_int, [c_void_p, c_int]),
     ("lass_separate_components", c_int, [c_void_p, POINTER(c_void_p), c_void_p, c_void_p, c_void_p, c_void_p, c_int,
                                          c_int, c_void_p, c_size_t, c_void_p]),
     ("lass_stft_components", c_int, [c_void_p, c_void_p, c_int, c_int, c_int, c_int, c_int, POINTER(c_int),
diff --git a/lass_amd/csrc/api.hip b/lass_amd/csrc/api.hip
--- a/lass_amd/csrc/api.hip
+++ b/lass_amd/csrc/api.hip
@@ -12,6 +12,7 @@
 #include "../../include/lass_hip.h"
 #include "ctx_parts.h"
 #include "graph_cache.h"
+#include "wino4_walk.h"
 #include "head_fold.h"
 #include "kernels.h"
 #include "weight_plan.h"
@@ -67,6 +68,7 @@
     int head_rows = 0;
     std::vector<void*> owned;
     RouteCfg cfg;
+    int wino4_walk = kWino4WalkDefault;
     float* stage_v = nullptr;
     size_t stage_v_floats = 0;
     float* stage_m = nullptr;
@@ -401,7 +403,7 @@
             if (rt.v_from_memory) vp.v = vws;
             if (rt.head_sc_fold) {
                 ok = planes && (rt.head_fold ? lass_wino4_headfold_planes_supported(a, *planes) : lass_wino4_sclogit_supported(a, *planes));
-                if (ok) HIP_TRY(c, rt.head_fold ? lass_launch_wino4_headfold_planes(a, *planes, st) : lass_launch_wino4_sclogit(a, *planes, st));
+                if (ok) HIP_TRY(c, rt.head_fold ? lass_launch_wino4_headfold_planes(a, *planes, st) : lass_launch_wino4_sclogit(a, *planes, st, c->wino4_walk));
                 break;
             }
             if (rt.head_fold) {
@@ -415,7 +417,7 @@
                 break;
             }
             ok = rt.v_from_memory ? lass_wino4_vpre_supported(rt.kind, a, s) : lass_wino4_supported(rt.kind, a, s);
-            if (ok) HIP_TRY(c, lass_launch_wino4(rt.kind, a, st, s, vp));
+            if (ok) HIP_TRY(c, lass_launch_wino4(rt.kind, a, st, s, vp, c->wino4_walk));
             break;
         }
         case CONV_F2X2:
@@ -741,6 +743,7 @@
     if (const char* e = getenv("LASS_HEAD_SC_FOLD")) c->cfg.head_sc_fold = atoi(e) != 0;
     if (const char* e = getenv("LASS_PW_SPLIT")) c->cfg.pw_split = atoi(e) != 0;
     if (const char* e = getenv("LASS_WINO4_GEMM")) c->cfg.wino4_gemm = atoi(e) != 0;
+    if (const char* e = getenv("LASS_WINO4_WALK")) c->wino4_walk = atoi(e);
     if (const char* e = getenv("LASS_SPLIT")) c->split_batch = std::max(0, std::min(2, atoi(e)));
     if (const char* e = getenv("LASS_GRAPH")) c->use_graph = atoi(e) != 0;
     c->prof.resize(P_COUNT);
@@ -1819,6 +1822,13 @@
     return 0;
 }
 
+int lass_set_wino4_walk(lass_ctx* c, int n) {
+    if (!c || n < -64 || n > 64) return fail(c, LASS_ERR_ARG, "lass_set_wino4_walk: -64 ... 64");
+    c->wino4_walk = n;
+    ++c->gen;
+    return 0;
+}
+
 int lass_set_wino4_vprep_buffer(lass_ctx* c, float* v, size_t floats) {
     if (!c || (v && !floats)) return fail(c, LASS_ERR_ARG, "lass_set_wino4_vprep_buffer: a buffer and its size, or NULL");
     c->stage_v_user = v;
diff --git a/lass_amd/csrc/kernels.h b/lass_amd/csrc/kernels.h
--- a/lass_amd/csrc/kernels.h
+++ b/lass_amd/csrc/kernels.h
@@ -104,7 +104,7 @@
 
 bool lass_wino4_supported(ConvKind kind, const ConvArgs& p, const Wino4Split& sk = Wino4Split());
 hipError_t lass_launch_wino4(ConvKind kind, const ConvArgs& p, hipStream_t stream, const Wino4Split& sk = Wino4Split(),
-                             const Wino4VPre& vp = Wino4VPre());
+                             const Wino4VPre& vp = Wino4VPre(), int walk = 1);
 bool lass_wino4_vpre_supported(ConvKind kind, const ConvArgs& p, const Wino4Split& sk = Wino4Split());
 hipError_t lass_launch_wino4_weights(const float* w, int Cout, int Cin, float* U, hipStream_t stream);
 bool lass_wino4_headfold_supported(const ConvArgs& p);
@@ -112,7 +112,7 @@
 bool lass_wino4_headfold_planes_supported(const ConvArgs& p, const HeadScPlanes& hs);
 hipError_t lass_launch_wino4_headfold_planes(const ConvArgs& p, const HeadScPlanes& hs, hipStream_t stream);
 bool lass_wino4_sclogit_supported(const ConvArgs& p, const HeadScPlanes& hs);
-hipError_t lass_launch_wino4_sclogit(const ConvArgs& p, const HeadScPlanes& hs, hipStream_t stream);
+hipError_t lass_launch_wino4_sclogit(const ConvArgs& p, const HeadScPlanes& hs, hipStream_t stream, int walk = 1);
 
 struct Wino4Gemm {
     const void* w3 = nullptr;
diff --git a/lass_amd/csrc/wino4.hip b/lass_amd/csrc/wino4.hip
--- a/lass_amd/csrc/wino4.hip
+++ b/lass_amd/csrc/wino4.hip
@@ -3,6 +3,7 @@
 #include "kernels.h"
 #include "pixel_ops.h"
 #include "wino4_transform.h"
+#include "wino4_walk.h"
 #include "wino_common.h"
 
 namespace {
@@ -11,6 +12,7 @@
 constexpr int F_SPLITK = 2048;
 constexpr int F_SCLOGIT = 8192;
 constexpr int F_VPRE = 4096;
+constexpr int F_WALK = 16384;
 constexpr int NTHREADS = 256;
 constexpr int KC = kWino4KC;
 constexpr int NXI = kWino4NXI;
@@ -19,12 +21,26 @@
 
 typedef float f32x2v __attribute__((ext_vector_type(2)));
 
+struct Wino4Walk {
+    int w = 1;
+    int gx = 0;
+};
+
 
 template <int TC, int FLAGS>
 __global__ __launch_bounds__(NTHREADS, 2) void wino4_kernel(ConvArgs p) {
     const Wino4Split sk;
     const Wino4VPre vp;
     const HeadScPlanes hs;
+    const Wino4Walk wk;
+#include "wino4_body.h"
+}
+template <int TC, int FLAGS0>
+__global__ __launch_bounds__(NTHREADS, 2) void wino4_walk_kernel(ConvArgs p, Wino4Walk wk) {
+    constexpr int FLAGS = FLAGS0 | F_WALK;
+    const Wino4Split sk;
+    const Wino4VPre vp;
+    const HeadScPlanes hs;
 #include "wino4_body.h"
 }
 template <int TC, int FLAGS0>
@@ -32,12 +48,14 @@
     constexpr int FLAGS = FLAGS0 | F_SPLITK;
     const Wino4VPre vp;
     const HeadScPlanes hs;
+    const Wino4Walk wk;
 #include "wino4_body.h"
 }
 template <int TC, int FLAGS0>
 __global__ __launch_bounds__(NTHREADS, 2) void wino4_vpre_kernel(ConvArgs p, Wino4Split sk, Wino4VPre vp) {
     constexpr int FLAGS = FLAGS0 | F_VPRE;
     const HeadScPlanes hs;
+    const Wino4Walk wk;
 #include "wino4_body.h"
 }
 template <int TC, int FLAGS0>
@@ -45,6 +63,14 @@
     constexpr int FLAGS = FLAGS0 | F_SCLOGIT;
     const Wino4Split sk;
     const Wino4VPre vp;
+    const Wino4Walk wk;
+#include "wino4_body.h"
+}
+template <int TC, int FLAGS0>
+__global__ __launch_bounds__(NTHREADS, 2) void wino4_sclogit_walk_kernel(ConvArgs p, HeadScPlanes hs, Wino4Walk wk) {
+    constexpr int FLAGS = FLAGS0 | F_SCLOGIT | F_WALK;
+    const Wino4Split sk;
+    const Wino4VPre vp;
 #include "wino4_body.h"
 }
 
@@ -62,7 +88,7 @@
 
 template <int TC, int FLAGS>
 __global__ __launch_bounds__(NTHREADS) void wino4_vprep_kernel(ConvArgs p, Wino4VPre vp) {
-    constexpr bool PRO = (FLAGS & F_PRO) != 0, PRE = false;
+    constexpr bool PRO = (FLAGS & F_PRO) != 0, PRE = false, WALK = false;
     static_assert((FLAGS & ~F_PRO) == 0, "a prologue at most");
     constexpr int TR = 32 / TC;
     constexpr int OR_ = 4 * TR, OC = 4 * TC;
@@ -162,24 +188,40 @@
         }
 }
 
+inline Wino4Walk plan_walk(Wino4WalkKind kind, ConvArgs& p, int walk) {
+    Wino4Walk wk;
+    wk.w = lass_wino4_walk_width(kind, walk, p.gx, p.gy, p.B);
+    wk.gx = p.gx;
+    if (wk.w > 1) p.gx = (wk.gx + wk.w - 1) / wk.w;
+    return wk;
+}
+
 template <int TC, int FLAGS>
-hipError_t launch_wino4_tc(const ConvArgs& p0, hipStream_t stream) {
+hipError_t launch_wino4_tc(const ConvArgs& p0, int walk, hipStream_t stream) {
     ConvArgs p = p0;
     constexpr int OR_ = 4 * (32 / TC), OC = 4 * TC;
     p.gx = (p.W / OC) * ((p.H + OR_ - 1) / OR_);
     p.gy = p.N / 32;
+    if constexpr ((FLAGS & (F_MASK | F_RES)) == 0) {
+        const Wino4Walk wk = plan_walk((FLAGS & F_PRECONV) ? W4W_CONV1_X0 : (FLAGS & F_PHASEB) ? W4W_CONV2_SC : W4W_CONV1, p, walk);
+        if (wk.w > 1) {
+            p.xcd_map = ((long)p.gx * p.B) % 8 == 0;
+            hipLaunchKernelGGL((wino4_walk_kernel<TC, FLAGS>), dim3((unsigned)((long)p.gx * p.gy * p.B)), dim3(NTHREADS), 0, stream, p, wk);
+            return hipGetLastError();
+        }
+    }
     p.xcd_map = ((long)p.gx * p.B) % 8 == 0;
     hipLaunchKernelGGL((wino4_kernel<TC, FLAGS>), dim3((unsigned)((long)p.gx * p.gy * p.B)), dim3(NTHREADS), 0, stream, p);
     return hipGetLastError();
 }
 
 template <int FLAGS>
-hipError_t launch_wino4(const ConvArgs& p, hipStream_t stream) {
+hipError_t launch_wino4(const ConvArgs& p, int walk, hipStream_t stream) {
     const int tc = lass_wino4_block_tc(p.H, p.W);
-    if (tc == 16) return launch_wino4_tc<16, FLAGS>(p, stream);
-    if (tc == 8) return launch_wino4_tc<8, FLAGS>(p, stream);
+    if (tc == 16) return launch_wino4_tc<16, FLAGS>(p, walk, stream);
+    if (tc == 8) return launch_wino4_tc<8, FLAGS>(p, walk, stream);
     if constexpr (FLAGS == (F_PRO | F_EPIACT) || FLAGS == F_RES)
-        if (tc == 4) return launch_wino4_tc<4, FLAGS>(p, stream);
+        if (tc == 4) return launch_wino4_tc<4, FLAGS>(p, walk, stream);
     return hipErrorInvalidValue;
 }
 
@@ -206,12 +248,17 @@
 }
 
 template <int TC>
-hipError_t launch_wino4_sclogit_tc(const ConvArgs& p0, const HeadScPlanes& hs, hipStream_t stream) {
+hipError_t launch_wino4_sclogit_tc(const ConvArgs& p0, const HeadScPlanes& hs, int walk, hipStream_t stream) {
     ConvArgs p = p0;
     constexpr int OR_ = 4 * (32 / TC), OC = 4 * TC;
     p.gx = (p.W / OC) * (p.H / OR_);
     p.gy = p.N / 32;
+    const Wino4Walk wk = plan_walk(W4W_CONV2_SKIP, p, walk);
     p.xcd_map = ((long)p.gx * p.B) % 8 == 0;
+    if (wk.w > 1) {
+        hipLaunchKernelGGL((wino4_sclogit_walk_kernel<TC, F_RES | F_RESPRE>), dim3((unsigned)((long)p.gx * p.gy * p.B)), dim3(NTHREADS), 0, stream, p, hs, wk);
+        return hipGetLastError();
+    }
     hipLaunchKernelGGL((wino4_sclogit_kernel<TC, F_RES | F_RESPRE>), dim3((unsigned)((long)p.gx * p.gy * p.B)), dim3(NTHREADS), 0, stream, p, hs);
     return hipGetLastError();
 }
@@ -293,7 +340,7 @@
     return lass_wino4_vpre_shape(kind, lass_conv_shape(p), sk.n) && lass_wino4_supported(kind, p, sk);
 }
 
-hipError_t lass_launch_wino4(ConvKind kind, const ConvArgs& p, hipStream_t stream, const Wino4Split& sk, const Wino4VPre& vp) {
+hipError_t lass_launch_wino4(ConvKind kind, const ConvArgs& p, hipStream_t stream, const Wino4Split& sk, const Wino4VPre& vp, int walk) {
     if (!lass_wino4_supported(kind, p, sk) || !p.in || (!p.out && !p.mask_re)) return hipErrorInvalidValue;
     if (vp.v) {
         if (!lass_wino4_vpre_supported(kind, p, sk)) return hipErrorInvalidValue;
@@ -308,14 +355,14 @@
         case CONV1_ACT_PRE:
             if (!p.pro_scale || !p.pro_shift || !p.epi_scale || !p.epi_shift) return hipErrorInvalidValue;
             if (sk.n > 1) return launch_wino4_split<F_PRO, F_EPIACT>(p, sk, stream);
-            return kind == CONV1_ACT ? launch_wino4<F_PRO | F_EPIACT>(p, stream) : launch_wino4<F_PRO | F_EPIACT | F_PRECONV>(p, stream);
+            return kind == CONV1_ACT ? launch_wino4<F_PRO | F_EPIACT>(p, walk, stream) : launch_wino4<F_PRO | F_EPIACT | F_PRECONV>(p, walk, stream);
         case CONV2_IDENT:
             if (sk.n > 1) return launch_wino4_split<0, F_RES>(p, sk, stream);
-            return launch_wino4<F_RES>(p, stream);
+            return launch_wino4<F_RES>(p, walk, stream);
         case CONV2_IDENT_PRE:
-            return launch_wino4<F_RES | F_RESPRE>(p, stream);
+            return launch_wino4<F_RES | F_RESPRE>(p, walk, stream);
         case CONV2_SHORTCUT:
-            return p.mask_re ? launch_wino4<F_PHASEB | F_BIAS | F_MASK>(p, stream) : launch_wino4<F_PHASEB | F_BIAS>(p, stream);
+            return p.mask_re ? launch_wino4<F_PHASEB | F_BIAS | F_MASK>(p, walk, stream) : launch_wino4<F_PHASEB | F_BIAS>(p, walk, stream);
         default:
             return hipErrorInvalidValue;
     }
@@ -344,9 +391,9 @@
     return lass_wino4_supported(CONV2_IDENT_PRE, p) && lass_wino4_block_tc(p.H, p.W) == 16 && p.in && p.out && hs.skip && hs.w;
 }
 
-hipError_t lass_launch_wino4_sclogit(const ConvArgs& p, const HeadScPlanes& hs, hipStream_t stream) {
+hipError_t lass_launch_wino4_sclogit(const ConvArgs& p, const HeadScPlanes& hs, hipStream_t stream, int walk) {
     if (!lass_wino4_sclogit_supported(p, hs)) return hipErrorInvalidValue;
-    return launch_wino4_sclogit_tc<16>(p, hs, stream);
+    return launch_wino4_sclogit_tc<16>(p, hs, walk, stream);
 }
 
 hipError_t lass_launch_wino4_weights(const float* w, int Cout, int Cin, float* U, hipStream_t stream) {
diff --git a/lass_amd/csrc/wino4_body.h b/lass_amd/csrc/wino4_body.h
--- a/lass_amd/csrc/wino4_body.h
+++ b/lass_amd/csrc/wino4_body.h
@@ -13,7 +13,9 @@
     constexpr bool VPRE = (FLAGS & F_VPRE) != 0;
     static_assert(!VPRE || (FLAGS & ~(F_VPRE | F_SPLITK | F_EPIACT | F_RES)) == 0, "conv1 / identity conv2 / split share: the prologue ran in the prep launch");
     constexpr bool SCL = (FLAGS & F_SCLOGIT) != 0;
-    static_assert(!SCL || (FLAGS == (F_RES | F_RESPRE | F_SCLOGIT) && TC == 16), "the skip's logits: encoder_block1.conv2 on the 8 x 64 blocks");
+    constexpr bool WALK = (FLAGS & F_WALK) != 0;
+    static_assert(!WALK || (!SPLIT && !VPRE && !MASK), "the unsplit kernels that form their own V and store their block");
+    static_assert(!SCL || ((FLAGS & ~F_WALK) == (F_RES | F_RESPRE | F_SCLOGIT) && TC == 16), "the skip's logits: encoder_block1.conv2 on the 8 x 64 blocks");
     constexpr int TR = 32 / TC;
     constexpr int OR_ = 4 * TR, OC = 4 * TC;
     constexpr int NCO = 32;
@@ -46,9 +48,14 @@
     } else {
         block_coords(p, bx_, by_, b);
     }
+    int bend = 0;
+    if constexpr (WALK) {
+        bend = min((bx_ + 1) * wk.w, wk.gx);
+        bx_ *= wk.w;
+    }
     const int n0 = by_ * NCO;
     const int tiles_x = p.W / OC;
-    const int y0 = (bx_ / tiles_x) * OR_, x0 = (bx_ % tiles_x) * OC;
+    int y0 = (bx_ / tiles_x) * OR_, x0 = (bx_ % tiles_x) * OC;
     const int HW = p.H * p.W;
     const float* in_b = p.in + (size_t)b * p.in_bs;
     const float* sc = PRO ? p.pro_scale : nullptr;
@@ -74,7 +81,7 @@
 #pragma unroll
         for (int r = 0; r < 4; ++r) acc[xi][r] = 0.f;
 
-    const int kq = lane >> 4, l15 = lane & 15;
+    int kq = lane >> 4, l15 = lane & 15;
     const float* afrag = lu + (wco >> 1) * U_F + (wco & 1) * 128 + (kq * 16 + l15) * 2;
     const float* bfrag = lv + (kq * 32 + ((wwt * 16 + l15) ^ ((kq & 1) << 4))) * 2;
     const unsigned slab_pitch = (unsigned)(p.Nw / 32) * (unsigned)(U_F * 4);
@@ -92,6 +99,7 @@
     const int nch = SPLIT ? (ks + 1) * (p.Cin / KC) / sk.n : p.Cin / KC;
     if constexpr (!VPRE) pload(ch0);
     lds_barrier();
+    do {
     for (int ch = ch0; ch < nch; ++ch) {
         lds_barrier();
         __builtin_amdgcn_s_setprio(2);
@@ -101,6 +109,10 @@
                 asm volatile("" : "+v"(pc[i].x), "+v"(pc[i].y), "+v"(pc[i].z), "+v"(pc[i].w), "+v"(pl[i]), "+v"(pr[i]));
             }
             if (PRO) asm volatile("" : "+v"(ps), "+v"(ph));
+            if constexpr (WALK && PRE) {
+                asm volatile("" : "+v"(ppw), "+v"(ppb));
+                pfold();
+            }
         }
 #pragma unroll
         for (int i = 0; i < 9; ++i) {
@@ -153,6 +165,7 @@
         }
     }
 
+    if constexpr (WALK) asm volatile("" : "+v"(kq), "+v"(l15));
     const int ot = wwt * 16 + l15;
     const int oy = y0 + 4 * (ot / TC), ox = x0 + 4 * (ot % TC);
     f32x4 ysp[16];
@@ -250,6 +263,12 @@
                 ysp[a * 4 + 2][r] += rv[r][a].z;
                 ysp[a * 4 + 3][r] += rv[r][a].w;
             }
+    }
+    if constexpr (WALK) {
+        if (bx_ + 1 < bend) {
+            WINO4_ITEM(((bx_ + 1) / tiles_x) * OR_, ((bx_ + 1) % tiles_x) * OC)
+            pload(0);
+        }
     }
     if constexpr (SC) {
         const float* x2 = p.in2 + (size_t)b * p.in2_bs + (size_t)min(oy, p.H - 4) * p.W + ox;
@@ -390,3 +409,13 @@
             if (my < p.H) *reinterpret_cast<float2*>(hs.skip + ((size_t)b * 3 + q) * HW + (size_t)my * p.W + mx) = sum;
         }
     }
+    if constexpr (WALK) {
+        if (++bx_ >= bend) break;
+        y0 = (bx_ / tiles_x) * OR_;
+        x0 = (bx_ % tiles_x) * OC;
+#pragma unroll
+        for (int xi = 0; xi < NXI; ++xi)
+#pragma unroll
+            for (int r = 0; r < 4; ++r) acc[xi][r] = 0.f;
+    }
+    } while (WALK);
diff --git a/lass_amd/csrc/wino4_gemm.hip b/lass_amd/csrc/wino4_gemm.hip
--- a/lass_amd/csrc/wino4_gemm.hip
+++ b/lass_amd/csrc/wino4_gemm.hip
@@ -13,7 +13,7 @@
 
 template <int TC, int FLAGS>
 __global__ __launch_bounds__(NTHREADS) void wino4_scatter_kernel(ConvArgs p, Wino4VPre vp) {
-    constexpr bool PRO = (FLAGS & F_PRO) != 0, PRE = false;
+    constexpr bool PRO = (FLAGS & F_PRO) != 0, PRE = false, WALK = false;
     static_assert((FLAGS & ~F_PRO) == 0, "a prologue at most");
     constexpr int KC = kWino4KC;
     constexpr int TR = 32 / TC;
diff --git a/lass_amd/csrc/wino4_head_body.h b/lass_amd/csrc/wino4_head_body.h
--- a/lass_amd/csrc/wino4_head_body.h
+++ b/lass_amd/csrc/wino4_head_body.h
@@ -1,4 +1,5 @@
     constexpr bool PRO = false, PRE = false;
+    constexpr bool WALK = false;
     constexpr int TR = 32 / TC;
     constexpr int OR_ = 4 * TR, OC = 4 * TC;
     constexpr int UH_F = kHeadFoldU4Floats;
diff --git a/lass_amd/csrc/wino4_input.h b/lass_amd/csrc/wino4_input.h
--- a/lass_amd/csrc/wino4_input.h
+++ b/lass_amd/csrc/wino4_input.h
@@ -1,20 +1,26 @@
     const int pt = tid & 31, c8 = (tid & 255) >> 5;
     const int pty = pt / TC, ptx = pt % TC;
-    const int gy0 = y0 + 4 * pty - 1, gx0 = x0 + 4 * ptx - 1;
-    const bool left = gx0 < 0, right = gx0 + 5 >= p.W;
-    unsigned vo_c[6], vo_l[6], vo_r[6], rowok = 0;
-#pragma unroll
-    for (int i = 0; i < 6; ++i) {
-        const int gy = gy0 + i;
-        const int row = (PRE ? 0 : c8 * HW) + min(max(gy, 0), p.H - 1) * p.W;
-        vo_c[i] = 4u * (unsigned)(row + gx0 + 1);
-        vo_l[i] = 4u * (unsigned)(row + (left ? 0 : gx0));
-        vo_r[i] = 4u * (unsigned)(row + (right ? p.W - 1 : gx0 + 5));
-        rowok |= (gy >= 0 && gy < p.H ? 1u : 0u) << i;
+#define WINO4_ITEM(Y0, X0)                                                                                                          \
+    {                                                                                                                               \
+        const int gy0 = (Y0) + 4 * pty - 1, gx0 = (X0) + 4 * ptx - 1;                                                               \
+        left = gx0 < 0;                                                                                                             \
+        right = gx0 + 5 >= p.W;                                                                                                     \
+        rowok = 0;                                                                                                                  \
+        _Pragma("unroll") for (int i = 0; i < 6; ++i) {                                                                             \
+            const int gy = gy0 + i;                                                                                                 \
+            const int row = (PRE ? 0 : c8 * HW) + min(max(gy, 0), p.H - 1) * p.W;                                                   \
+            vo_c[i] = 4u * (unsigned)(row + gx0 + 1);                   \
+            vo_l[i] = 4u * (unsigned)(row + (left ? 0 : gx0));                           \
+            vo_r[i] = 4u * (unsigned)(row + (right ? p.W - 1 : gx0 + 5));                                                           \
+            rowok |= (gy >= 0 && gy < p.H ? 1u : 0u) << i;                                                                          \
+        }                                                                                                                           \
+        edge = left || right || rowok != 0x3fu;                                \
     }
+    bool left, right, edge;
+    unsigned vo_c[6], vo_l[6], vo_r[6], rowok;
+    WINO4_ITEM(y0, x0)
     const __amdgpu_buffer_rsrc_t in_rsrc =
         __builtin_amdgcn_make_buffer_rsrc(const_cast<float*>(in_b), 0, (int)((unsigned)(PRE ? 1 : p.Cin) * (unsigned)HW * 4u), 0x00020000);
-    const bool edge = left || right || rowok != 0x3fu;
     float4 pc[6];
     float pl[6], pr[6], ps = 1.f, ph = 0.f;
     const unsigned tvo = (unsigned)c8 * 4u;
@@ -23,6 +29,11 @@
     };
     const __amdgpu_buffer_rsrc_t sc_rsrc = tab_rsrc(PRO ? sc : p.in, p.Cin), sh_rsrc = tab_rsrc(PRO ? sh : p.in, p.Cin);
     const __amdgpu_buffer_rsrc_t pw_rsrc = tab_rsrc(PRE ? p.pre_w : p.in, 32), pb_rsrc = tab_rsrc(PRE ? p.pre_b : p.in, 32);
+    float ppw = 0.f, ppb = 0.f;
+    auto pfold = [&]() {
+        ph = fmaf(ppb, ps, ph);
+        ps = ppw * ps;
+    };
     auto pload = [&](int ch) {
         const unsigned soff = PRE ? 0u : (unsigned)(ch * KC * HW) * 4u;
         if (!PRE || ch == 0)
@@ -38,10 +49,9 @@
             ph = __builtin_bit_cast(float, __builtin_amdgcn_raw_buffer_load_b32(sh_rsrc, (int)tvo, (int)toff, 0));
         }
         if (PRE) {
-            const float pw = __builtin_bit_cast(float, __builtin_amdgcn_raw_buffer_load_b32(pw_rsrc, (int)tvo, (int)toff, 0));
-            const float pb = __builtin_bit_cast(float, __builtin_amdgcn_raw_buffer_load_b32(pb_rsrc, (int)tvo, (int)toff, 0));
-            ph = fmaf(pb, ps, ph);
-            ps = pw * ps;
+            ppw = __builtin_bit_cast(float, __builtin_amdgcn_raw_buffer_load_b32(pw_rsrc, (int)tvo, (int)toff, 0));
+            ppb = __builtin_bit_cast(float, __builtin_amdgcn_raw_buffer_load_b32(pb_rsrc, (int)tvo, (int)toff, 0));
+            if (!WALK) pfold();
         }
     };
     constexpr int NLOAD = (PRE ? 0 : 6 * 3) + (PRO ? 2 : 0) + (PRE ? 2 : 0);
diff --git a/lass_amd/csrc/wino4_walk.h b/lass_amd/csrc/wino4_walk.h
--- /dev/null
+++ b/lass_amd/csrc/wino4_walk.h
@@ -0,0 +1,24 @@
+#pragma once
+
+constexpr int kWino4WalkSlots = 512;
+constexpr int kWino4WalkDefault = 2;
+
+enum Wino4WalkKind {
+    W4W_CONV1 = 0,
+    W4W_CONV1_X0 = 1,
+    W4W_CONV2_SC = 2,
+    W4W_CONV2_SKIP = 3
+};
+
+inline bool lass_wino4_walk_default(Wino4WalkKind kind) { return kind == W4W_CONV1_X0; }
+
+inline int lass_wino4_walk_width(Wino4WalkKind kind, int cap, int gx, int gy, int B) {
+    const bool forced = cap < -1;
+    if (!forced && !lass_wino4_walk_default(kind)) return 1;
+    int w = forced ? -cap : cap;
+    if (w > gx) w = gx;
+    if (w < 1) w = 1;
+    if (!forced)
+        while (w > 1 && (long)((gx + w - 1) / w) * gy * B < 2L * kWino4WalkSlots) --w;
+    return w;
+}
```

Result: no change. 1189 clips/s (median of 6 runs) (+0.4%).
